# baaivision/Painter

Hardware: AMD Instinct MI355X
Metric: images/sec (896x448 pairs) ViT-L fwd+bwd (higher is better)
Workload: dtype bf16; 1 GPU; painter_vit_large_patch16_input896x448 bf16 batch=8/GPU fwd+bwd on 1xMI355X (BASELINE configs[1]); global_batch=8, image=896x448x3 stitched pair, mode=train (DropPath 0.1), parallelism=dp1, rccl_ranks=0, backend=n/a, grad_allreduce=n/a

## Files before the change

### include/painter_hip.h

```cpp
#ifndef PAINTER_HIP_H
#define PAINTER_HIP_H

#include <stdint.h>

#ifdef __cplusplus
extern "C" {
#endif

#ifndef __HIP__
typedef struct ihipStream_t* hipStream_t;
#endif

enum { PA_F32 = 0, PA_BF16 = 1 };
enum {
    PA_EPI_BIAS = 0,
    PA_EPI_BIAS_F32 = 1,
    PA_EPI_BIAS_GELU = 2,
    PA_EPI_BIAS_RESID = 3
};

#define PA_ABI_VERSION 6
int pa_abi_version(void);
int pa_debug_set(int which, int value);
int pa_debug_get(int which);

int pa_linear_fwd(int dtype, int epilogue, const void* x , int64_t ldx, const void* w ,
                  const float* bias , void* out, void* out2, int64_t ldo, const float* resid ,
                  const float* rowscale , int rows_per_sample, int M, int N, int K,
                  hipStream_t stream);
int pa_linear_pixshuf(int dtype, const void* x, int64_t ldx, const void* w , const float* bias,
                      void* out_nhwc, int batch, int Hp, int Wp, int P, int C, int K, hipStream_t stream);
int64_t pa_linear_dgrad_workspace_bytes(int M, int K);
int pa_linear_dgrad(int dtype, const void* dy , int64_t lddy, const void* w ,
                    const void* gelu_aux , void* dx , int64_t lddx, float* dx_colsum,
                    void* workspace, int M, int N, int K, hipStream_t stream);
int64_t pa_linear_wgrad_workspace_bytes(int dtype, int M, int N, int K);
int pa_linear_wgrad(int dtype, const void* dy , int64_t lddy, const void* x , int64_t ldx,
                    float* dw , void* workspace, int M, int N, int K, hipStream_t stream);
int64_t pa_colsum_workspace_bytes(int M, int N);
int pa_colsum(int dtype, const void* x , int64_t ld, int M, int N, float* out , void* workspace,
              hipStream_t stream);
int pa_slab_reduce(const float* in, float* out, int64_t n, int nz, int64_t stride, int accumulate, hipStream_t stream);

int pa_layernorm_fwd(int dtype, const float* x, int64_t ldx, const float* gamma, const float* beta, float eps,
                     void* y , int64_t ldy, float* mean, float* rstd,
                     int R, int D, hipStream_t stream);
int64_t pa_layernorm_bwd_workspace_bytes(int R, int D);
int pa_layernorm_bwd(int dtype, const void* dy, int64_t lddy, const float* x, int64_t ldx, const float* mean,
                     const float* rstd, const float* gamma, const float* dres, float* dx, int64_t lddx, void* dxT,
                     int64_t lddxT, const float* rowscale, int rows_per_sample, float* dgamma_dbeta, float* dxT_colsum,
                     void* workspace, int R, int D, hipStream_t stream);
int pa_layernorm_bwd_reduce(const void* workspace, float* dgamma_dbeta, float* dxT_colsum, int with_colsum, int R, int D,
                            hipStream_t stream);

int pa_relpos_rows_padded(int Hp, int Wp);
int pa_relpos_pack(int dtype, const float* rel_pos_h, const float* rel_pos_w, void* rcat, int Hp, int Wp, int head_dim,
                   hipStream_t stream);
int pa_relpos_pack_batch(int dtype, const void* tabs, void* rcat, void* rcatT, int nblocks, int Hp, int Wp, int head_dim, hipStream_t stream);
int64_t pa_attn_tables_bytes(int dtype, int batch, int L, int heads, int Hp, int Wp, int head_dim);
int pa_attn_set_generation(int generation);
int pa_attn_launch_counts(long long* out6);
int pa_attn_trace(int enable, unsigned long long* host_out);
int pa_attn_fwd(int dtype, const void* qkv, int64_t ldq, const void* rcat, void* out, int64_t ldo, float* lse,
                void* tables, int batch, int L, int heads, int Hp, int Wp, int head_dim, float scale, hipStream_t stream);

int pa_relpos_pack_t(int dtype, const float* rel_pos_h, const float* rel_pos_w, void* rcatT, int Hp, int Wp, int head_dim,
                     hipStream_t stream);
int pa_attn_bwd_delta(int dtype, const void* out, int64_t ldo, const void* dout, int64_t lddo, float* delta, int batch,
                      int L, int heads, int head_dim, hipStream_t stream);
int pa_attn_bwd_prep_ok(int dtype, int L, int Hp, int Wp, int head_dim);
int pa_attn_bwd_prep(int dtype, const void* out, int64_t ldo, const void* dout, int64_t lddo, const float* lse, void* tables,
                     int batch, int L, int heads, int Hp, int Wp, int head_dim, float scale, hipStream_t stream);
int64_t pa_attn_bwd_aux_bytes(int batch, int L, int heads, int Hp, int Wp);
int64_t pa_attn_bwd_relpos_partials_bytes(int dtype, int batch, int L, int heads, int Hp, int Wp, int head_dim);
int pa_attn_bwd(int dtype, const void* qkv, int64_t ldq, const void* rcat, const void* rcatT, const void* dout,
                int64_t lddo, const float* lse, const float* delta, void* dqkv, void* dG, void* relpos_part, void* aux,
                void* tables, const void* out, int64_t ldo, int batch, int L, int heads, int Hp, int Wp, int head_dim, float scale,
                hipStream_t stream);
int64_t pa_attn_bwd_relpos_workspace_bytes(int dtype, int batch, int L, int heads, int Hp, int Wp, int head_dim);
int pa_attn_bwd_relpos_reduce(const void* relpos_part, float* drcat, void* workspace, int batch, int L, int heads, int Hp, int Wp,
                              int head_dim, hipStream_t stream);
int pa_attn_bwd_relpos(int dtype, const void* dG, const void* qkv, int64_t ldq, float* drcat, void* workspace,
                       int batch, int L, int heads, int Hp, int Wp, int head_dim, hipStream_t stream);

int pa_patch_weight_pack(int dtype, const float* w , void* out , int D, int P, hipStream_t stream);
int pa_patch_embed_fwd(int dtype, const float* imgs, const float* tgts, const void* w, int64_t ldw, const float* bias,
                       const float* mask_token, const float* seg_x, const float* seg_y, const float* pos,
                       const unsigned char* mask, int mask_batch_stride, const float* type_cls, const float* type_ins,
                       const float* seg_type, float* tokens, int batch, int Hp, int Wp, int P, int D, hipStream_t stream);
int pa_patch_cols_ok(int batch, int L, int P, int D);
int pa_patch_im2col(const float* imgs, const float* tgts, void* cols, int batch, int Hp, int Wp, int P, hipStream_t stream);
int pa_patch_embed_fwd_cols(const void* cols, const void* w , int64_t ldw, const float* bias, const float* mask_token,
                            const float* seg_x, const float* seg_y, const float* pos, const unsigned char* mask, int mask_batch_stride,
                            const float* type_cls, const float* type_ins, const float* seg_type, float* tokens, int batch, int L, int K,
                            int D, hipStream_t stream);
int64_t pa_patch_embed_wgrad_workspace_bytes(int D, int P);
int pa_patch_embed_wgrad(int dtype, const void* dpe , const float* imgs, const float* tgts,
                         float* dw , void* workspace, int batch, int Hp, int Wp, int P, int D,
                         hipStream_t stream);
int pa_patch_embed_dgrad(int dtype, const void* dpe, const void* w, int64_t ldw, float* dimgs, float* dtgts, const float* addend,
                         float alpha, int batch, int Hp, int Wp, int P, int D, hipStream_t stream);
int pa_pos_fwd(const int* idx , const float* val , int K, const float* pe , float* pos , int L, int D,
               hipStream_t stream);
int pa_pos_bwd(const int* idxT , const float* valT , int KT, const float* gx , const float* gy ,
               float* dpe , int S, int D, hipStream_t stream);
int pa_tokens_bwd(int dtype, const float* dx0, const unsigned char* mask, int mask_batch_stride, void* dpe, float* sums,
                  int batch, int L, int D, hipStream_t stream);

int pa_merge_fwd(const float* x, float* out, int64_t n_out, hipStream_t stream);
int pa_merge_bwd(int dtype, const float* dmerged, float* dx, void* dxT, const float* rowscale, int rows_per_sample,
                 int64_t rows_half, int D, hipStream_t stream);
int pa_scale_cast(int dtype, const float* in, void* out, const float* rowscale, int rows_per_sample, int64_t rows, int D,
                  hipStream_t stream);
int pa_cast_bf16(const float* in, void* out, int64_t n, hipStream_t stream);
int pa_debug_rmw(const float* src, float* scratch, int64_t n, int passes, int nblocks, hipStream_t stream);
int pa_ensemble_resid(const float* x0, const float* a, float* x1, int batch, int group, int L, int D, hipStream_t stream);

int pa_conv3x3_pack(int dtype, const float* w3 , void* w3r , void* wf ,
                    hipStream_t stream);
int pa_decoder_tail_fwd(int dtype, const void* x_nhwc, const void* w3r, const float* b3, const float* ln_gamma,
                        const float* ln_beta, const float* w1 , const float* b1, void* y3 ,
                        float* pred , int batch, int Hi, int Wi, float eps, hipStream_t stream);
int64_t pa_decoder_tail_bwd_workspace_bytes(int batch, int Hi, int Wi);
int pa_decoder_tail_bwd_pointwise(int dtype, const float* dpred, const void* y3, const float* ln_gamma,
                                  const float* ln_beta, const float* w1, void* dy3, float* grads, void* workspace,
                                  int batch, int Hi, int Wi, float eps, hipStream_t stream);
int pa_conv3x3_dgrad_unshuffle(int dtype, const void* dy3, const void* wf, void* dE, int batch, int Hp, int Wp, int P,
                               hipStream_t stream);
int64_t pa_conv3x3_wgrad_workspace_bytes(int batch, int Hi, int Wi);
int pa_conv3x3_wgrad(int dtype, const void* dy3, const void* x_nhwc, float* dw , void* workspace,
                     int batch, int Hi, int Wi, hipStream_t stream);
// ... 78 lines not shown
```

### painter_amd/csrc/attn3.h

```cpp
#pragma once
#include "common.h"
bool attn3_ok(int L, int Hp, int Wp);
int64_t attn3_table_bytes(int Bn, int L, int H, int Hp, int Wp);
int attn3_fwd(const bf16* qkv, int64_t ldq, const bf16* rcat, bf16* out, int64_t ldo, float* lse, void* tables, int Bn, int L, int H,
              int Hp, int Wp, float scale, hipStream_t st);
int attn3_bwd(const bf16* qkv, int64_t ldq, const bf16* rcatT, const bf16* dout, int64_t lddo, const float* lse, const float* delta,
              void* tables, bf16* dqkv, bf16* dG, float* part, int Bn, int L, int H, int Hp, int Wp, float scale, const bf16* out, int64_t ldo,
              hipStream_t st);
int attn3_bwd_prep(const bf16* out, int64_t ldo, const bf16* dout, int64_t lddo, const float* lse, void* tables, int Bn, int L, int H, int Hp,
                   float scale, hipStream_t st);
int64_t attn3_relpos_partials_bytes(int Bn, int L, int H, int Hp, int Wp);
int attn3_relpos_reduce(const float* part, float* drcat, float* tmp, int Bn, int L, int H, int Hp, int Wp, hipStream_t st);
```

### painter_amd/csrc/attn3.hip

```cpp
#include "attn3_common.h"
#include "../../include/painter_hip.h"
#include "attn3.h"
#include <cstdlib>

#ifndef A3_PRIO
#define A3_PRIO 0
#endif
#ifndef A3_HOIST
#define A3_HOIST 1
#endif
#ifndef A3_NDL
#define A3_NDL true
#endif
#define A3_PRIO_UP() do { if (A3_PRIO) __builtin_amdgcn_s_setprio(1); } while (0)
#define A3_PRIO_DOWN() do { if (A3_PRIO) __builtin_amdgcn_s_setprio(0); } while (0)

namespace a3 {

template <int STAGES>
__global__ __launch_bounds__(NT, STAGES == 1 ? 4 : 2) void fwd_kernel(const bf16* __restrict__ qkv, size_t ldq, const bf16* __restrict__ rcat,
                                                                      bf16* __restrict__ out, size_t ldo, float* __restrict__ lse,
                                                                      unsigned char* __restrict__ tables, int L, int H, int Hp, int NRP,
                                                                      float scale, int nblk, int xcd_map, int abl) {
    extern __shared__ __attribute__((aligned(16))) unsigned char smem[];
    const int tid = threadIdx.x, lane = tid & 63, wave = tid >> 6, g = lane >> 5, ql = lane & 31;
    int blk, bh;
    wg_coords(nblk, xcd_map, blk, bh, (L / 32) / NW);
    const int b = bh / H, h = bh % H, D = H * ATT_HD;
    const bf16* base = qkv + (size_t)b * L * ldq + h * ATT_HD;
    const bf16* kbase = base + D;
    const bf16* vbase = base + 2 * D;
    const int qt = blk * NW + wave;
    const bool valid = qt * 32 < L;
    const int q = qt * 32 + ql;
    unsigned char* thT = smem + STAGES * STAGE_QK + wave * Hp * 64;
    unsigned char* eimg = smem + STAGES * STAGE_QK + NW * Hp * 64;
    unsigned char* twimg = eimg + wave * 2048;
    LaneAddr la;
    la.init(lane);
    EAddr ea;
    ea.init(lane);
    const int ntile = L / 32;
    Stager ks, vs;
    ks.load(kbase, ldq, tid);
    vs.load(vbase, ldq, tid);

    bf16x8 qf[4];
    uint4 T0 = zero4(), T1 = zero4();
    if (valid) {
#pragma unroll
        for (int s = 0; s < 4; ++s) qf[s] = gfrag(base + (size_t)q * ldq, s, g);
        if (!(abl & 32)) build_tables3(twimg, thT, rcat, NRP, qf, q / WP, q % WP, Hp, 1.f / scale, lane, smem + tid * 2);
        T0 = *reinterpret_cast<const uint4*>(twimg + ql * 64 + 16 * g);
        T1 = *reinterpret_cast<const uint4*>(twimg + ql * 64 + 32 + 16 * g);
        if (tables != nullptr) {
            unsigned char* tt = tables + ((size_t)bh * ntile + qt) * ttile_bytes(Hp);
#pragma unroll
            for (int i = 0; i < 2; ++i) *reinterpret_cast<uint4*>(tt + (lane + 64 * i) * 16) = *reinterpret_cast<const uint4*>(twimg + (lane + 64 * i) * 16);
            for (int c = lane; c < Hp * 4; c += 64) *reinterpret_cast<uint4*>(tt + 2048 + c * 16) = *reinterpret_cast<const uint4*>(thT + c * 16);
        }
    }
    __syncthreads();
    build_eimg(eimg, tid);
    ks.store(smem, tid);
    vs.store(smem + IMG, tid);
    __syncthreads();

    f32x16 oacc[2];
    oacc[0] = zero16();
    oacc[1] = zero16();
    float m = 0.f, l = 0.f;
    const float sl = scale * LOG2E_F;
    const unsigned char* thw = thT + ql * 2;

    auto body = [&](auto pc, int a) {
        constexpr int P = decltype(pc)::value;
        const int j = a * PH + P;
        {
            const int jn = min(j + 1, ntile - 1);
            ks.load(kbase + (size_t)jn * 32 * ldq, ldq, tid);
            vs.load(vbase + (size_t)jn * 32 * ldq, ldq, tid);
        }
        const unsigned char* kimg = smem + (STAGES == 2 ? (j & 1) * STAGE_QK : 0);
        const unsigned char* vimg = kimg + IMG;
        if (valid) {
            const unsigned char* thr = thw + a * (RPP * 64);
            if constexpr (P == 0) win_set<0>(T1.w, thr);
            win_set<(P + 1) & 1>(T1.w, thr + (P + 1) * 64);
            const unsigned char* ei = eimg + P * EIMG;
            const bf16x8 ef0 = efrag(ei, ea, 0), ef1 = efrag(ei, ea, 1);
            bf16x8 kfr[4];
#pragma unroll
            for (int s = 0; s < 4; ++s) kfr[s] = rowfrag(kimg, la, s);
            __builtin_amdgcn_sched_barrier(0);
            f32x16 sacc = zero16();
            A3_PRIO_UP();
            sacc = mfma(ef0, as_frag(T0), sacc);
            sacc = mfma(ef1, as_frag(T1), sacc);
#pragma unroll
            for (int s = 0; s < 4; ++s) sacc = mfma(kfr[s], qf[s], sacc);
            A3_PRIO_DOWN();
            bf16x8 vtr[2][2];
            vtr[0][0] = trfrag(vimg, la, 0, 0);
            vtr[0][1] = trfrag(vimg, la, 0, 1);
            if constexpr (STAGES == 2) { vtr[1][0] = trfrag(vimg, la, 1, 0); vtr[1][1] = trfrag(vimg, la, 1, 1); }
            __builtin_amdgcn_sched_barrier(0);
            float p[16];
            const float nm = -m;
#pragma unroll
            for (int r = 0; r < 16; ++r) p[r] = fmaf(sacc[r], sl, nm);
            float tmax = max16(p);
            tmax = fmaxf(tmax, xor32(tmax));
            if (j == 0 || __any(tmax > THR)) {
                const float delta = (j == 0) ? tmax : fmaxf(tmax, 0.f);
                const float alpha = __builtin_amdgcn_exp2f(-delta);
                m += delta;
                l *= alpha;
#pragma unroll
                for (int r = 0; r < 16; ++r) { oacc[0][r] *= alpha; oacc[1][r] *= alpha; p[r] -= delta; }
            }
#pragma unroll
            for (int r = 0; r < 16; ++r) p[r] = __builtin_amdgcn_exp2f(p[r]);
            l += sum16(p);
            const bf16x8 pf0 = packfrag(p), pf1 = packfrag(p + 8);
            if constexpr (STAGES == 1) { vtr[1][0] = trfrag(vimg, la, 1, 0); vtr[1][1] = trfrag(vimg, la, 1, 1); }
            A3_PRIO_UP();
#pragma unroll
            for (int db = 0; db < 2; ++db) {
                oacc[db] = mfma(vtr[db][0], pf0, oacc[db]);
                oacc[db] = mfma(vtr[db][1], pf1, oacc[db]);
            }
            A3_PRIO_DOWN();
        }
        if constexpr (STAGES == 1) __syncthreads();
        if (j + 1 < ntile) {
            ks.store(smem + (STAGES == 2 ? ((j + 1) & 1) * STAGE_QK : 0), tid);
            vs.store(smem + (STAGES == 2 ? ((j + 1) & 1) * STAGE_QK : 0) + IMG, tid);
        }
        __syncthreads();
    };
    for (int a = 0; a < ((abl & 16) ? 0 : Hp / RPP); ++a) {
        body(std::integral_constant<int, 0>{}, a);
        body(std::integral_constant<int, 1>{}, a);
        body(std::integral_constant<int, 2>{}, a);
        body(std::integral_constant<int, 3>{}, a);
        body(std::integral_constant<int, 4>{}, a);
        body(std::integral_constant<int, 5>{}, a);
        body(std::integral_constant<int, 6>{}, a);
    }
    unsigned char* stg = smem + wave * IMG;
    if constexpr (STAGES == 1) { if (wave >= 2) stg = eimg + (wave - 2) * IMG; }
    if (valid) {
        const float lt = l + xor32(l);
        if (g == 0) {
            const float lse_q = (m + __builtin_amdgcn_logf(lt)) * LN2_F;
            lse[(size_t)bh * L + q] = lse_q;
            if (tables != nullptr) {
                unsigned char* tt = tables + ((size_t)bh * ntile + qt) * ttile_bytes(Hp);
                const float x = -lse_q * (1.f / scale);
                const bf16 hi = (bf16)x;
                *reinterpret_cast<bf16*>(tt + 2048 + Hp * 64 + ql * 2) = hi;
                *reinterpret_cast<bf16*>(tt + 2048 + (Hp + 1) * 64 + ql * 2) = (bf16)(x - (float)hi);
            }
        }
        stage_rows(stg, oacc, 1.f / lt, lane);
        write_rows(stg, out + (size_t)(b * L + qt * 32) * ldo + h * ATT_HD, ldo, lane);
    }
}

__device__ unsigned long long g_trace[2 * 2 * 64 * 8];
constexpr int NSMAX = 12;
template <int MINW, bool NDL, bool TR = false, bool FUSE = false>
__global__ __launch_bounds__(NT, MINW) void bwd_dq_kernel(const bf16* __restrict__ qkv, size_t ldq, const bf16* __restrict__ rcatT,
                                                          const bf16* __restrict__ dout, size_t lddo, const float* __restrict__ lse,
                                                          unsigned char* __restrict__ tables, bf16* __restrict__ dqkv,
                                                          bf16* __restrict__ dG, float* __restrict__ part, int L, int H, int Hp, int NRP,
                                                          float scale, int nblk, int xcd_map, int abl, int tile0, int pslot0,
                                                          const bf16* __restrict__ oatt, size_t ldo) {
    extern __shared__ __attribute__((aligned(16))) unsigned char smem[];
    const int tid = threadIdx.x, lane = tid & 63, wave = tid >> 6, g = lane >> 5, ql = lane & 31;
    const int trwg = blockIdx.x == 0 ? 0 : (blockIdx.x == gridDim.x / 2 ? 1 : -1);
    auto coarse = [&](int pt) {
        if constexpr (TR) {
            if constexpr (MINW < 3 && A3_HOIST) __builtin_amdgcn_sched_barrier(0);
            const unsigned long long t = __builtin_amdgcn_s_memtime();
            if (trwg >= 0 && wave < 2 && lane == 0) g_trace[((trwg * 2 + wave) * 64 + pt) * 8] = t;
            if constexpr (MINW < 3 && A3_HOIST) __builtin_amdgcn_sched_barrier(0);
        }
    };
    coarse(60);
    int blk, bh;
    wg_coords(nblk, xcd_map, blk, bh, (L / 32 - tile0) / NW);
    const int b = bh / H, h = bh % H, D = H * ATT_HD;
    const bf16* base = qkv + (size_t)b * L * ldq + h * ATT_HD;
    const bf16* kbase = base + D;
    const bf16* vbase = base + 2 * D;
    const int qt = tile0 + blk * NW + wave;
    const bool valid = qt * 32 < L;
    const int q = qt * 32 + ql;
    const int qh = q / WP, qw = q % WP;
    unsigned char* thT = smem + 2 * STAGE_QK + wave * Hp * 64;
    unsigned char* eimg = smem + 2 * STAGE_QK + NW * Hp * 64;
    unsigned char* rimg = eimg + PH * EIMG;
    const int rpitch = NRP * 2 + 16;
    LaneAddr la;
    la.init(lane);
    EAddr ea;
    ea.init(lane);
    const int ntile = L / 32;
    const float sl = scale * LOG2E_F;
    Stager ks, vs;
    ks.load(kbase, ldq, tid);
    vs.load(vbase, ldq, tid);
    const int rchunks = ATT_HD * (NRP / 8);

    bf16x8 qf[4], dof[4];
    uint4 T0 = zero4(), T1 = zero4();
    uint4 tch[4] = {zero4(), zero4(), zero4(), zero4()};
    float nlse2 = 0.f, ndlt = 0.f;
    unsigned char* tt = tables + ((size_t)bh * ntile + qt) * ttile_bytes(Hp);
    if (valid) {
#pragma unroll
        for (int s = 0; s < 4; ++s) {
            qf[s] = gfrag(base + (size_t)q * ldq, s, g);
            dof[s] = gfrag(dout + (size_t)(b * L + q) * lddo + h * ATT_HD, s, g);
        }
        if (oatt != nullptr) {
            float dl = 0.f;
#pragma unroll
            for (int s = 0; s < 4; ++s) {
                const bf16x8 of = gfrag(oatt + (size_t)(b * L + q) * ldo + h * ATT_HD, s, g);
#pragma unroll
                for (int t = 0; t < 8; ++t) dl = fmaf((float)of[t], (float)dof[s][t], dl);
            }
            dl += xor32(dl);
            ndlt = -dl;
            if (g == 0) *reinterpret_cast<float*>(tt + 2048 + (Hp + 2) * 64 + ql * 4) = ndlt;
        }
        T0 = *reinterpret_cast<const uint4*>(tt + ql * 64 + 16 * g);
        T1 = *reinterpret_cast<const uint4*>(tt + ql * 64 + 32 + 16 * g);
#pragma unroll
        for (int i = 0; i < 4; ++i)
            if (lane + 64 * i < Hp * 4) tch[i] = *reinterpret_cast<const uint4*>(tt + 2048 + (lane + 64 * i) * 16);
        nlse2 = -lse[(size_t)bh * L + q] * LOG2E_F;
        if (oatt == nullptr) ndlt = *reinterpret_cast<const float*>(tt + 2048 + (Hp + 2) * 64 + ql * 4);
    }
    build_eimg(eimg, tid);
    {
        const int per_row = NRP / 8;
        for (int c = tid; c < rchunks; c += 2 * NT) {
            const int c2 = c + NT;
            const uint4 v0 = *reinterpret_cast<const uint4*>(rcatT + (size_t)c * 8);
            const uint4 v1 = c2 < rchunks ? *reinterpret_cast<const uint4*>(rcatT + (size_t)c2 * 8) : zero4();
// ... 165 lines not shown
        };
        const int nstep = NRP / 16;
        const unsigned char* r0 = rimg + ql * rpitch + 16 * g, *r1 = r0 + 32 * rpitch;
        auto rfrag = [&](const unsigned char* rp, int s) { return __builtin_bit_cast(bf16x8, *reinterpret_cast<const uint4*>(rp + 32 * s)); };
        bf16x8 rf[2] = {rfrag(r0, 0), rfrag(r1, 0)};
        float gcur[8];
        gather(0, gcur);
        auto rstep = [&](int s, uint4& keep) {
            const int sn = min(s + 1, nstep - 1);
            const bf16x8 rn[2] = {rfrag(r0, sn), rfrag(r1, sn)};
            float gnext[8];
            if (abl & 32) {
#pragma unroll
                for (int t = 0; t < 8; ++t) gnext[t] = gcur[t] + 1.f;
            } else {
                gather(sn, gnext);
            }
            const bf16x8 gf = packfrag(gcur);
            if constexpr (FUSE) keep = __builtin_bit_cast(uint4, gf);
            else if (!(abl & 2)) *reinterpret_cast<uint4*>(dgrow + 16 * s + 8 * g) = __builtin_bit_cast(uint4, gf);
#pragma unroll
            for (int db = 0; db < 2; ++db) {
                if (!(abl & 64)) dq[db] = mfma(rf[db], gf, dq[db]);
                rf[db] = rn[db];
            }
#pragma unroll
            for (int t = 0; t < 8; ++t) gcur[t] = gnext[t];
        };
        if constexpr (FUSE) {
#pragma unroll
            for (int s = 0; s < NSMAX; ++s)
                if (s < ((abl & 1) ? 0 : nstep)) rstep(s, gfs[s]);
        } else {
            uint4 none;
            for (int s = 0; s < ((abl & 1) ? 0 : nstep); ++s) rstep(s, none);
        }
        stage_rows(stg, dq, 1.f, lane);
        if (!(abl & 4)) write_rows(stg, dqkv + (size_t)(b * L + qt * 32) * ldq + h * ATT_HD, ldq, lane);
    }
    if constexpr (FUSE) {
        __syncthreads();
        const int nimg = (NRP + 63) >> 6;
        unsigned char* wimg = smem + wave * (nimg + 1) * IMG;
        if (valid) {
            const int rsw = vsw(ql);
#pragma unroll
            for (int s = 0; s < NSMAX; ++s)
                if (s < NRP / 16) *reinterpret_cast<uint4*>(wimg + (s >> 2) * IMG + ql * 128 + ((((2 * s + g) & 7) ^ rsw) << 4)) = gfs[s];
#pragma unroll
            for (int s = 0; s < 4; ++s)
                *reinterpret_cast<uint4*>(wimg + nimg * IMG + ql * 128 + (((2 * s + g) ^ rsw) << 4)) = __builtin_bit_cast(uint4, qf[s]);
        }
        __syncthreads();
        float* pw = part + (size_t)(pslot0 + blockIdx.x) * NRP * ATT_HD;
        for (int u = wave; u < 2 * (NRP / 32); u += NW) {
            const int rb = u >> 1, db = u & 1;
            f32x16 acc = zero16();
            for (int w2 = 0; w2 < NW; ++w2) {
                if ((tile0 + blk * NW + w2) * 32 >= L) break;
                const unsigned char* im = smem + w2 * (nimg + 1) * IMG;
#pragma unroll
                for (int ks = 0; ks < 2; ++ks)
                    acc = mfma(trfrag(im + (rb >> 1) * IMG, la, rb & 1, ks), trfrag(im + nimg * IMG, la, db, ks), acc);
            }
            float* pcol = pw + (size_t)(rb * 32 + 4 * g) * ATT_HD + db * 32 + ql;
#pragma unroll
            for (int reg = 0; reg < 16; ++reg) pcol[((reg & 3) + 8 * (reg >> 2)) * ATT_HD] = acc[reg];
        }
    }
    if constexpr (TR) { asm volatile("s_waitcnt vmcnt(0)" ::: "memory"); }
    coarse(63);
}

constexpr int DKV_TW = 2 * IMG, DKV_TH = DKV_TW + 2048, DKV_ND = DKV_TH + 512, DKV_STAGE = DKV_ND + 128;
template <int MINW>
__global__ __launch_bounds__(NT, MINW) void bwd_dkv_kernel(const bf16* __restrict__ qkv, size_t ldq, const bf16* __restrict__ dout,
                                                           size_t lddo, const unsigned char* __restrict__ tables, bf16* __restrict__ dqkv,
                                                           int L, int H, int Hp, float scale, int nblk, int xcd_map, int abl, int tile0) {
    extern __shared__ __attribute__((aligned(16))) unsigned char smem[];
    const int tid = threadIdx.x, lane = tid & 63, wave = tid >> 6, g = lane >> 5, ql = lane & 31;
    int blk, bh;
    wg_coords(nblk, xcd_map, blk, bh, (L / 32 - tile0) / NW);
    const int b = bh / H, h = bh % H, D = H * ATT_HD;
    const bf16* qbase = qkv + (size_t)b * L * ldq + h * ATT_HD;
    const bf16* dobase = dout + (size_t)b * L * lddo + h * ATT_HD;
    const int kt = tile0 + blk * NW + wave;
    const bool valid = kt * 32 < L;
    const int key = kt * 32 + ql;
    const int kh = key / WP, kw = key % WP;
    const int khlo = ((tile0 + blk * NW) * 32) / WP;
    const int kha = (kt * 32) / WP;
    const int ntile = L / 32;
    const int TB = ttile_bytes(Hp);
    const unsigned char* tbase = tables + (size_t)bh * ntile * TB;
    LaneAddr la;
    la.init(lane);
    EAddr ea;
    ea.init(lane);
    const float sl = scale * LOG2E_F;
    const int sa = kha & 3, sb = (kha + 1) & 3;

    bf16x8 kf[4], vf[4], eb0, eb1;
    int woff[2];
    {
        uint32_t e0[4] = {0, 0, 0, 0}, e1[4] = {0, 0, 0, 0};
#pragma unroll
        for (int t = 0; t < 8; ++t) {
            const uint32_t bit = 0x3F80u << (16 * (t & 1));
            if (kw == 8 * g + t) e0[t >> 1] |= bit;
            if (t < 6) {
                if (kw == 16 + 6 * g + t) e1[t >> 1] |= bit;
            } else {
                const int slot = 2 * g + (t - 6);
                if (slot == (kh & 3) || (slot != sa && slot != sb)) e1[t >> 1] |= bit;
            }
        }
        eb0 = __builtin_bit_cast(bf16x8, make_uint4(e0[0], e0[1], e0[2], e0[3]));
        eb1 = __builtin_bit_cast(bf16x8, make_uint4(e1[0], e1[1], e1[2], e1[3]));
#pragma unroll
        for (int hs = 0; hs < 2; ++hs) {
            const int slot = 2 * g + hs;
            int row;
            if (slot == sa) row = kha - khlo;
            else if (slot == sb) row = kha + 1 - khlo;
            else {
                int rank = 0;
                for (int s2 = 0; s2 < slot; ++s2) rank += (s2 != sa && s2 != sb) ? 1 : 0;
                row = 6 + rank;
            }
            woff[hs] = DKV_TH + row * 64 + ql * 2;
        }
    }
    if (valid) {
#pragma unroll
        for (int s = 0; s < 4; ++s) {
            kf[s] = gfrag(qbase + D + (size_t)key * ldq, s, g);
            vf[s] = gfrag(qbase + 2 * D + (size_t)key * ldq, s, g);
        }
    }
    Stager qs, dos;
// ... 135 lines not shown
            unsigned char* tt = tables + ((size_t)bh * (L / 32) + qt) * TB;
            const float x = -lse[(size_t)bh * L + l] * inv_scale;
            const bf16 hi = (bf16)x;
            const bf16 lo = (bf16)(x - (float)hi);
            *reinterpret_cast<bf16*>(tt + 2048 + Hp * 64 + qi * 2) = hi;
            *reinterpret_cast<bf16*>(tt + 2048 + (Hp + 1) * 64 + qi * 2) = lo;
            *reinterpret_cast<float*>(tt + 2048 + (Hp + 2) * 64 + qi * 4) = -s;
        }
    }
}

}

int attn3_bwd_prep(const bf16* out, int64_t ldo, const bf16* dout, int64_t lddo, const float* lse, void* tables, int Bn, int L, int H, int Hp,
                   float scale, hipStream_t st) {
    const int R = Bn * L;
    PA_LAUNCH(a3::prep_delta_kernel, dim3((R + 3) / 4), dim3(256), 0, st, out, (size_t)ldo, dout, (size_t)lddo, lse,
              reinterpret_cast<unsigned char*>(tables), R, L, H, Hp, 1.f / scale);
    return (int)hipGetLastError();
}

static int g_attn_generation = 0;
extern "C" int pa_attn_set_generation(int generation) {
    if (generation != 0 && generation != 2 && generation != 3) return (int)hipErrorInvalidValue;
    g_attn_generation = generation;
    return 0;
}
static int g_attn_trace = 0;
extern "C" int pa_attn_trace(int enable, unsigned long long* host_out) {
    g_attn_trace = enable;
    if (host_out != nullptr) return (int)hipMemcpyFromSymbol(host_out, HIP_SYMBOL(a3::g_trace), sizeof(a3::g_trace));
    return 0;
}
bool attn3_ok(int L, int Hp, int Wp) {
    static const int on = [] { const char* e = getenv("PA_ATTN3"); return e ? atoi(e) : 1; }();
    return on && g_attn_generation != 2 && Wp == a3::WP && Hp % a3::RPP == 0 && Hp >= a3::RPP && L == Hp * Wp;
}
int64_t attn3_table_bytes(int Bn, int L, int H, int Hp, int Wp) {
    if (!attn3_ok(L, Hp, Wp)) return 0;
    return (int64_t)Bn * H * (L / 32) * a3::ttile_bytes(Hp);
}
static int a3_xcd_map_on() {
    static const int v = [] {
        const char* e = getenv("PA_ATTN_XCD");
        const char* l = getenv("PA_ATTN_LIGHT_LAST");
        return ((e ? atoi(e) : 1) ? 1 : 0) | ((l ? atoi(l) : 0) ? 2 : 0);
    }();
    if (g_attn_light_last == 1) return v & 1;
    if (g_attn_light_last == 2) return v | 2;
    return v;
}

int attn3_fwd(const bf16* qkv, int64_t ldq, const bf16* rcat, bf16* out, int64_t ldo, float* lse, void* tables, int Bn, int L, int H,
              int Hp, int Wp, float scale, hipStream_t st) {
    using namespace a3;
    const int NRP = pa_relpos_rows_padded(Hp, Wp);
    static const int stages = [] { const char* v = getenv("PA_ATTN3_FWD_STAGES"); return v ? atoi(v) : 1; }();
    const size_t smem = (size_t)(stages == 2 ? 2 : 1) * STAGE_QK + (size_t)NW * Hp * 64 + PH * EIMG;
    static bool done1 = false, done2 = false;
    auto kern = stages == 2 ? fwd_kernel<2> : fwd_kernel<1>;
    if (int e = set_smem(reinterpret_cast<const void*>(kern), stages == 2 ? done2 : done1)) return e;
    const int nblk = (L / 32 + NW - 1) / NW;
    PA_LAUNCH(kern, dim3(nblk * Bn * H), dim3(NT), smem, st, qkv, (size_t)ldq, rcat, out, (size_t)ldo, lse,
              reinterpret_cast<unsigned char*>(tables), L, H, Hp, NRP, scale, nblk, a3_xcd_map_on(), [] { const char* v = getenv("PA_ATTN3_FWD_ABL"); return v ? atoi(v) : 0; }());
    return (int)hipGetLastError();
}

namespace a3 {
constexpr int RED_ZC = 32;
__global__ __launch_bounds__(256) void relpos_part_reduce_kernel(const float4* __restrict__ part, float4* __restrict__ tmp, int n4, int nz) {
    __shared__ float4 sh[4][64];
    const int c = blockIdx.x * 64 + (threadIdx.x & 63), zl = threadIdx.x >> 6;
    const int z0 = (int)((int64_t)nz * blockIdx.y / gridDim.y), z1 = (int)((int64_t)nz * (blockIdx.y + 1) / gridDim.y);
    float4 s = make_float4(0, 0, 0, 0);
    if (c < n4) {
#pragma unroll 4
        for (int z = z0 + zl; z < z1; z += 4) {
            const float4 v = part[(size_t)z * n4 + c];
            s.x += v.x; s.y += v.y; s.z += v.z; s.w += v.w;
        }
    }
    sh[zl][threadIdx.x & 63] = s;
    __syncthreads();
    if (zl == 0 && c < n4) {
        float4 t = sh[0][threadIdx.x];
#pragma unroll
        for (int k = 1; k < 4; ++k) { const float4 v = sh[k][threadIdx.x]; t.x += v.x; t.y += v.y; t.z += v.z; t.w += v.w; }
        tmp[(size_t)blockIdx.y * n4 + c] = t;
    }
}
}
extern "C" int pa_slab_reduce(const float* in, float* out, int64_t n, int nz, int64_t stride, int accumulate, hipStream_t st);
static int a3_fuse_on() {
    static const int v = [] { const char* e = getenv("PA_ATTN3_FUSE_RELPOS"); return e ? atoi(e) : 1; }();
    return g_attn3_fuse == 1 ? 0 : (g_attn3_fuse == 2 ? 1 : v);
}
static int a3_blocks(int L) { return (L / 32 + a3::NW - 1) / a3::NW; }
static int64_t a3_num_partials(int Bn, int L, int H, int, int) { return (int64_t)a3_blocks(L) * Bn * H; }
int64_t attn3_relpos_partials_bytes(int Bn, int L, int H, int Hp, int Wp) {
    if (!a3_fuse_on() || !attn3_ok(L, Hp, Wp)) return 0;
    const int NRP = pa_relpos_rows_padded(Hp, Wp);
    if (NRP > 16 * a3::NSMAX) return 0;
    return a3_num_partials(Bn, L, H, Hp, Wp) * NRP * ATT_HD * sizeof(float);
}
int attn3_relpos_reduce(const float* part, float* drcat, float* tmp, int Bn, int L, int H, int Hp, int Wp, hipStream_t st) {
    using namespace a3;
    const int NRP = pa_relpos_rows_padded(Hp, Wp);
    const int nz = (int)a3_num_partials(Bn, L, H, Hp, Wp), n4 = NRP * ATT_HD / 4;
    const int zc = nz < RED_ZC ? nz : RED_ZC;
    PA_LAUNCH(relpos_part_reduce_kernel, dim3((n4 + 63) / 64, zc), dim3(256), 0, st, reinterpret_cast<const float4*>(part),
              reinterpret_cast<float4*>(tmp), n4, nz);
    if (int e = (int)hipGetLastError()) return e;
    return pa_slab_reduce(tmp, drcat, (int64_t)n4 * 4, zc, (int64_t)n4 * 4, 0, st);
}

int attn3_bwd(const bf16* qkv, int64_t ldq, const bf16* rcatT, const bf16* dout, int64_t lddo, const float* lse, const float* delta,
              void* tables, bf16* dqkv, bf16* dG, float* part, int Bn, int L, int H, int Hp, int Wp, float scale, const bf16* out, int64_t ldo,
              hipStream_t st) {
    using namespace a3;
    const int NRP = pa_relpos_rows_padded(Hp, Wp);
    if (part != nullptr && NRP > 16 * NSMAX) return (int)hipErrorInvalidValue;
    if (part == nullptr && dG == nullptr) return (int)hipErrorInvalidValue;
    unsigned char* tb = reinterpret_cast<unsigned char*>(tables);
    int e;
    if (delta != nullptr) {
        const int total = Bn * H * L;
        PA_LAUNCH(prep_kernel, dim3((total + 255) / 256), dim3(256), 0, st, lse, delta, tb, L, Hp, 1.f / scale, total);
        if ((e = (int)hipGetLastError())) return e;
    }
    const int tile0 = 0;
    const int nblk = a3_blocks(L);
    static const int dq_w = [] { const char* v = getenv("PA_ATTN3_DQ_WAVES"); return v ? atoi(v) : 2; }();
    static const int dkv_w = [] { const char* v = getenv("PA_ATTN3_DKV_WAVES"); return v ? atoi(v) : 2; }();
    if (nblk > 0) {
        static const size_t pad = [] { const char* v = getenv("PA_ATTN3_LDS_PAD"); return v ? (size_t)atoi(v) : (size_t)0; }();
        size_t smem = 2 * (size_t)STAGE_QK + (size_t)NW * Hp * 64 + PH * EIMG + (size_t)ATT_HD * (NRP * 2 + 16) + pad;
        const bool fuse = part != nullptr;
        if (fuse) {
            const size_t need = (size_t)NW * ((NRP + 63) / 64 + 1) * IMG;
            if (smem < need) smem = need;
        }
        auto kern = fuse ? bwd_dq_kernel<2, A3_NDL, false, true>
                         : (g_attn_trace ? bwd_dq_kernel<2, true, true> : (dq_w == 3 ? bwd_dq_kernel<3, false> : bwd_dq_kernel<2, A3_NDL>));
        static bool done2 = false, done3 = false, donet = false, donef = false;
        if ((e = set_smem(reinterpret_cast<const void*>(kern), fuse ? donef : (g_attn_trace ? donet : (dq_w == 3 ? done3 : done2))))) return e;
        const char* ablv = getenv("PA_ATTN3_DQ_ABL");
        PA_LAUNCH(kern, dim3(nblk * Bn * H), dim3(NT), smem, st, qkv, (size_t)ldq, rcatT, dout, (size_t)lddo, lse, tb, dqkv, dG, part, L, H,
                  Hp, NRP, scale, nblk, a3_xcd_map_on(), ablv ? atoi(ablv) : 0, tile0, 0, delta == nullptr ? out : nullptr, (size_t)ldo);
        if ((e = (int)hipGetLastError())) return e;
    }
    const int tile0_kv = 0, nblk_kv = a3_blocks(L);
    if (nblk_kv > 0) {
        size_t smem = 2 * (size_t)DKV_STAGE;
        if (smem < (size_t)NW * 2 * IMG) smem = (size_t)NW * 2 * IMG;
        static const size_t pad = [] { const char* v = getenv("PA_ATTN3_LDS_PAD"); return v ? (size_t)atoi(v) : (size_t)0; }();
        smem += pad;
        auto kern = dkv_w == 3 ? bwd_dkv_kernel<3> : bwd_dkv_kernel<2>;
        static bool done2 = false, done3 = false;
        if ((e = set_smem(reinterpret_cast<const void*>(kern), dkv_w == 3 ? done3 : done2))) return e;
        PA_LAUNCH(kern, dim3(nblk_kv * Bn * H), dim3(NT), smem, st, qkv, (size_t)ldq, dout, (size_t)lddo, tb, dqkv, L, H, Hp, scale, nblk_kv,
                  a3_xcd_map_on(), [] { const char* v = getenv("PA_ATTN3_DKV_ABL"); return v ? atoi(v) : 0; }(), tile0_kv);
        if ((e = (int)hipGetLastError())) return e;
    }
    return 0;
}
```

### painter_amd/csrc/attn_bwd.hip

```cpp
#include "attn_common.h"
#include <cstdlib>
#include "gemm_engine.h"
#include "../../include/painter_hip.h"
#include "attn2.h"
#include "attn3.h"

template <typename T> DEVI void load16(const T* p, float* v);
template <> DEVI void load16<bf16>(const bf16* p, float* v) {
    const uint4 a = *reinterpret_cast<const uint4*>(p), b = *reinterpret_cast<const uint4*>(p + 8);
    v[0] = bf16_lo(a.x); v[1] = bf16_hi(a.x); v[2] = bf16_lo(a.y); v[3] = bf16_hi(a.y);
    v[4] = bf16_lo(a.z); v[5] = bf16_hi(a.z); v[6] = bf16_lo(a.w); v[7] = bf16_hi(a.w);
    v[8] = bf16_lo(b.x); v[9] = bf16_hi(b.x); v[10] = bf16_lo(b.y); v[11] = bf16_hi(b.y);
    v[12] = bf16_lo(b.z); v[13] = bf16_hi(b.z); v[14] = bf16_lo(b.w); v[15] = bf16_hi(b.w);
}
template <> DEVI void load16<float>(const float* p, float* v) {
#pragma unroll
    for (int i = 0; i < 4; ++i) {
        const float4 a = *reinterpret_cast<const float4*>(p + 4 * i);
        v[4 * i] = a.x; v[4 * i + 1] = a.y; v[4 * i + 2] = a.z; v[4 * i + 3] = a.w;
    }
}
template <typename T, bool VEC>
__global__ __launch_bounds__(256) void attn_delta_kernel(const T* o, size_t ldo, const T* d_o, size_t lddo, float* delta, int R, int L, int H, int hd) {
    __shared__ float part[4][128];
// ... 471 lines not shown
template <typename T, int HD>
static int attn_bwd_t(const T* qkv, int64_t ldq, const T* rcat, const T* rcatT, const T* dout, int64_t lddo, const float* lse,
                      const float* delta, T* dqkv, T* dG, float* aux, int Bn, int L, int H, int Hp, int Wp, float scale, hipStream_t st) {
    typedef KvTile<T, HD> KV;
    const int TS = Hp + Wp;
    const int qtiles = L / 32;
    {
        int ts = 2 * 32 * TS * 4;
        const int stg = 32 * HD * (int)sizeof(T);
        if (ts < stg) ts = stg;
        ts = (ts + 15) / 16 * 16;
        const size_t stages = 2 * (size_t)(2 * KV::KB + KV::VB);
        int e = (int)hipErrorInvalidValue;
        if (stages + 4 * (size_t)ts <= 160 * 1024) {
            e = attn_bwd_dq_launch<T, 4, HD>(qkv, ldq, rcat, rcatT, dout, lddo, lse, delta, dqkv, dG, aux, Bn, L, H, Hp, Wp, scale, stages + 4 * (size_t)ts, ts, st);
        } else if constexpr (HD != 64) {
            if (stages + 3 * (size_t)ts <= 160 * 1024)
                e = attn_bwd_dq_launch<T, 3, HD>(qkv, ldq, rcat, rcatT, dout, lddo, lse, delta, dqkv, dG, aux, Bn, L, H, Hp, Wp, scale, stages + 3 * (size_t)ts, ts, st);
        }
        if (e) return e;
    }
    {
        constexpr int NW = 4;
        const int AUXB = (TS + 2) * AUX_LD * 4;
        size_t smem = 2 * (size_t)(2 * KV::KB + 2 * KV::VB + AUXB);
        const size_t stg = (size_t)NW * 2 * 32 * HD * sizeof(T);
        if (smem < stg) smem = stg;
        if (smem > 160 * 1024 || (TS + 2) * 8 > (HD == 64 ? 3 : 4) * NW * 64) return (int)hipErrorInvalidValue;
        auto kern = attn_bwd_dkv_kernel<T, NW, HD>;
        static bool done = false;
        if (!done) {
            hipError_t e = hipFuncSetAttribute(reinterpret_cast<const void*>(kern), hipFuncAttributeMaxDynamicSharedMemorySize, 160 * 1024);
            if (e != hipSuccess) return (int)e;
            done = true;
        }
        PA_LAUNCH(kern, dim3((qtiles + NW - 1) / NW, Bn * H), dim3(NW * 64), smem, st, qkv, (size_t)ldq, dout, (size_t)lddo,
                           aux, dqkv, L, H, Hp, Wp, scale);
        return (int)hipGetLastError();
    }
}

extern "C" int pa_attn_bwd_prep_ok(int dtype, int L, int Hp, int Wp, int head_dim) {
    return (dtype == PA_BF16 && head_dim == ATT_HD && L == Hp * Wp && attn3_ok(L, Hp, Wp)) ? 1 : 0;
}
extern "C" int pa_attn_bwd_prep(int dtype, const void* out, int64_t ldo, const void* dout, int64_t lddo, const float* lse, void* tables,
                                int batch, int L, int heads, int Hp, int Wp, int head_dim, float scale, hipStream_t st) {
    if (!pa_attn_bwd_prep_ok(dtype, L, Hp, Wp, head_dim) || tables == nullptr || ldo % 8 || lddo % 8) return (int)hipErrorInvalidValue;
    return attn3_bwd_prep((const bf16*)out, ldo, (const bf16*)dout, lddo, lse, tables, batch, L, heads, Hp, scale, st);
}
extern "C" int64_t pa_attn_bwd_relpos_partials_bytes(int dtype, int batch, int L, int heads, int Hp, int Wp, int head_dim) {
    if (dtype != PA_BF16 || head_dim != ATT_HD || L != Hp * Wp) return 0;
    return attn3_relpos_partials_bytes(batch, L, heads, Hp, Wp);
}
extern "C" int pa_attn_bwd(int dtype, const void* qkv, int64_t ldq, const void* rcat, const void* rcatT, const void* dout, int64_t lddo,
                           const float* lse, const float* delta, void* dqkv, void* dG, void* relpos_part, void* aux, void* tables,
                           const void* out, int64_t ldo, int batch, int L, int heads, int Hp, int Wp, int head_dim, float scale, hipStream_t st) {
    if (L != Hp * Wp || L % 32 || Hp % 4 || Wp % 4 || (head_dim != 64 && head_dim != 80)) return (int)hipErrorInvalidValue;
    if (dtype == PA_BF16 && head_dim == ATT_HD && tables != nullptr && attn3_ok(L, Hp, Wp)) {
        if (relpos_part != nullptr && attn3_relpos_partials_bytes(batch, L, heads, Hp, Wp) == 0) return (int)hipErrorInvalidValue;
        ++g_attn_counts[5];
        if (out != nullptr && ldo % 8) return (int)hipErrorInvalidValue;
        return attn3_bwd((const bf16*)qkv, ldq, (const bf16*)rcatT, (const bf16*)dout, lddo, lse, delta, tables, (bf16*)dqkv, (bf16*)dG,
                         (float*)relpos_part, batch, L, heads, Hp, Wp, scale, (const bf16*)out, ldo, st);
    }
    if (relpos_part != nullptr || dG == nullptr || delta == nullptr) return (int)hipErrorInvalidValue;
    if (dtype == PA_BF16 && attn2_ok(L, Hp, Wp, head_dim)) {
        ++g_attn_counts[4];
        return attn2_bwd((const bf16*)qkv, ldq, (const bf16*)rcat, (const bf16*)rcatT, (const bf16*)dout, lddo, lse, delta, (bf16*)dqkv,
                         (bf16*)dG, aux, batch, L, heads, Hp, Wp, head_dim, scale, st);
    }
    ++g_attn_counts[3];
#define PA_ATTN_BWD(TT_, HD_) attn_bwd_t<TT_, HD_>((const TT_*)qkv, ldq, (const TT_*)rcat, (const TT_*)rcatT, (const TT_*)dout, lddo, lse, delta, \
                                                   (TT_*)dqkv, (TT_*)dG, (float*)aux, batch, L, heads, Hp, Wp, scale, st)
    if (dtype == PA_BF16) return head_dim == 80 ? PA_ATTN_BWD(bf16, 80) : PA_ATTN_BWD(bf16, 64);
    return head_dim == 80 ? PA_ATTN_BWD(float, 80) : PA_ATTN_BWD(float, 64);
#undef PA_ATTN_BWD
}

extern "C" int64_t pa_attn_bwd_relpos_workspace_bytes(int dtype, int batch, int L, int heads, int Hp, int Wp, int head_dim) {
    const int NRP = pa_relpos_rows_padded(Hp, Wp);
    return (int64_t)heads * 32 * NRP * head_dim * sizeof(float);
}
template <typename T>
static int relpos_grad_t(const T* dG, const T* qkv, int64_t ldq, float* drcat, float* ws, int Bn, int L, int H, int NRP, int hd, hipStream_t st) {
    const int R = Bn * L;
    OpT<T> A{dG, (size_t)H * NRP, NRP, (size_t)NRP};
    OpT<T> B{qkv, (size_t)ldq, hd, (size_t)hd};
    const int nku = (R + TT<T>::BK - 1) / TT<T>::BK;
    static const int want = [] { const char* v = getenv("PA_RELPOS_SPLITS"); return v ? atoi(v) : 16; }();
    static const bool from_env = getenv("PA_RELPOS_SPLITS") != nullptr;
    int splits = (!from_env && g_relpos_splits > 0) ? g_relpos_splits : want;
    if (splits > 32) splits = 32;
    if (splits < 1) splits = 1;
    if (splits > nku) splits = nku;
    struct Epi {
        float* out; size_t slab; int M, N;
        DEVI void operator()(const f32x16 (&acc)[2][2], int ib, int jb, int lane, int z) const {
            float* o = out + (size_t)z * slab;
            foreach_acc(acc, ib, jb, lane, [&](int i, int j, float v) {
                if (i < M && j < N) o[(size_t)i * N + j] = v;
            });
        }
    };
    int e = launch_gemm<T, 2, 2>(A, B, Epi{ws, (size_t)NRP * hd, NRP, hd}, NRP, hd, R, splits, H, st);
    if (e) return e;
    return pa_slab_reduce(ws, drcat, (int64_t)NRP * hd, splits * H, (int64_t)NRP * hd, 0, st);
}
extern "C" int pa_attn_bwd_relpos_reduce(const void* relpos_part, float* drcat, void* workspace, int batch, int L, int heads, int Hp, int Wp,
                                         int head_dim, hipStream_t st) {
    if (head_dim != ATT_HD || relpos_part == nullptr || attn3_relpos_partials_bytes(batch, L, heads, Hp, Wp) == 0) return (int)hipErrorInvalidValue;
    return attn3_relpos_reduce((const float*)relpos_part, drcat, (float*)workspace, batch, L, heads, Hp, Wp, st);
}
extern "C" int pa_attn_bwd_relpos(int dtype, const void* dG, const void* qkv, int64_t ldq, float* drcat, void* workspace, int batch, int L,
                                  int heads, int Hp, int Wp, int head_dim, hipStream_t st) {
    if (head_dim <= 0 || head_dim % 16) return (int)hipErrorInvalidValue;
    const int NRP = pa_relpos_rows_padded(Hp, Wp);
    if (dtype == PA_BF16) return relpos_grad_t<bf16>((const bf16*)dG, (const bf16*)qkv, ldq, drcat, (float*)workspace, batch, L, heads, NRP, head_dim, st);
    return relpos_grad_t<float>((const float*)dG, (const float*)qkv, ldq, drcat, (float*)workspace, batch, L, heads, NRP, head_dim, st);
}
```

### painter_amd/csrc/attn_fwd.hip

```cpp
#include "attn_common.h"
#include "../../include/painter_hip.h"
#include "attn2.h"
#include "attn3.h"

template <typename T, int NW, int HD>
__global__ __launch_bounds__(NW * 64) void attn_fwd_kernel(const T* __restrict__ qkv, size_t ldq, const T* __restrict__ rcat,
                                                           T* __restrict__ out, size_t ldo, float* __restrict__ lse, int L, int H,
                                                           int Hp, int Wp, int NRP, float scale, int tab_stride) {
    typedef KvTile<T, HD> KV;
    constexpr int NT = NW * 64;
    constexpr int KB = KV::KB, VB = KV::VB, KS = KV::KS, DB = KV::DB;
    extern __shared__ __attribute__((aligned(16))) unsigned char smem[];
    const int tid = threadIdx.x, lane = tid & 63, wave = tid >> 6, g = lane >> 5;
    const int bh = blockIdx.y, b = bh / H, h = bh % H;
    const int D = H * HD, TS = Hp + Wp;
    const T* base = qkv + (size_t)b * L * ldq + h * HD;
    const T* kbase = base + D;
    const T* vbase = base + 2 * D;
    const int qt = blockIdx.x * NW + wave;
    const bool valid = qt * 32 < L;
    const int q = qt * 32 + (lane & 31);
    unsigned char* const kimg = smem;
    unsigned char* const vimg = smem + 2 * KB;
    unsigned char* const wreg = smem + 2 * KB + 2 * VB + (size_t)wave * tab_stride;
// ... 169 lines not shown
    if (r < nh) v = rh[r * hd + d];
    else if (r - nh < nw) v = rw[(r - nh) * hd + d];
    (tr ? rcatT : rcat)[(size_t)blk * NRP * hd + i] = from_f<T>(v);
}
extern "C" int pa_relpos_pack_batch(int dtype, const void* tabs, void* rcat, void* rcatT, int nblocks, int Hp, int Wp, int head_dim, hipStream_t st) {
    if (head_dim <= 0 || head_dim % 16 || nblocks <= 0 || nblocks > 65535) return (int)hipErrorInvalidValue;
    const int NRP = pa_relpos_rows_padded(Hp, Wp);
    const int n = NRP * head_dim;
    const float* const* t = reinterpret_cast<const float* const*>(tabs);
    if (dtype == PA_BF16)
        PA_LAUNCH(relpos_pack_batch_kernel<bf16>, dim3((n + 255) / 256, nblocks, 2), dim3(256), 0, st, t, nblocks, 2 * Hp - 1, 2 * Wp - 1, (bf16*)rcat, (bf16*)rcatT, NRP, head_dim);
    else
        PA_LAUNCH(relpos_pack_batch_kernel<float>, dim3((n + 255) / 256, nblocks, 2), dim3(256), 0, st, t, nblocks, 2 * Hp - 1, 2 * Wp - 1, (float*)rcat, (float*)rcatT, NRP, head_dim);
    LAUNCH_CHECK();
}

static int attn_tab_stride(int Hp, int Wp, int hd, int elem) {
    int a = 32 * (Hp + Wp) * 4, b = 32 * hd * elem;
    int s = a > b ? a : b;
    return (s + 15) / 16 * 16;
}
template <typename T, int NW, int HD>
static int attn_fwd_launch(const T* qkv, int64_t ldq, const T* rcat, T* out, int64_t ldo, float* lse, int Bn, int L, int H, int Hp,
                           int Wp, float scale, hipStream_t st) {
    const int NRP = pa_relpos_rows_padded(Hp, Wp);
    const int ts = attn_tab_stride(Hp, Wp, HD, sizeof(T));
    const size_t smem = 2 * KvTile<T, HD>::KB + 2 * KvTile<T, HD>::VB + (size_t)NW * ts;
    auto kern = attn_fwd_kernel<T, NW, HD>;
    static bool done = false;
    if (!done) {
        hipError_t e = hipFuncSetAttribute(reinterpret_cast<const void*>(kern), hipFuncAttributeMaxDynamicSharedMemorySize, 160 * 1024);
        if (e != hipSuccess) return (int)e;
        done = true;
    }
    if (smem > 160 * 1024) return (int)hipErrorInvalidValue;
    const int qtiles = L / 32;
    dim3 grid((qtiles + NW - 1) / NW, Bn * H);
    PA_LAUNCH(kern, grid, dim3(NW * 64), smem, st, qkv, (size_t)ldq, rcat, out, (size_t)ldo, lse, L, H, Hp, Wp, NRP, scale, ts);
    return (int)hipGetLastError();
}
template <typename T>
static int attn_fwd_t(const void* qkv, int64_t ldq, const void* rcat, void* out, int64_t ldo, float* lse, int Bn, int L, int H, int Hp,
                      int Wp, int hd, float scale, hipStream_t st) {
    const T *q = (const T*)qkv, *r = (const T*)rcat;
    T* o = (T*)out;
    if (hd == 80) return attn_fwd_launch<T, 4, 80>(q, ldq, r, o, ldo, lse, Bn, L, H, Hp, Wp, scale, st);
    if ((L / 32) % 7 == 0) return attn_fwd_launch<T, 7, 64>(q, ldq, r, o, ldo, lse, Bn, L, H, Hp, Wp, scale, st);
    return attn_fwd_launch<T, 4, 64>(q, ldq, r, o, ldo, lse, Bn, L, H, Hp, Wp, scale, st);
}

extern "C" int64_t pa_attn_tables_bytes(int dtype, int batch, int L, int heads, int Hp, int Wp, int head_dim) {
    return dtype == PA_BF16 && head_dim == ATT_HD ? attn3_table_bytes(batch, L, heads, Hp, Wp) : 0;
}
extern "C" int pa_attn_fwd(int dtype, const void* qkv, int64_t ldq, const void* rcat, void* out, int64_t ldo, float* lse, void* tables,
                           int batch, int L, int heads, int Hp, int Wp, int head_dim, float scale, hipStream_t st) {
    if (L != Hp * Wp || L % 32 || Hp % 4 || Wp % 4 || !head_dim_ok(head_dim)) return (int)hipErrorInvalidValue;
    if (dtype == PA_BF16 && head_dim == ATT_HD && attn3_ok(L, Hp, Wp)) {
        ++g_attn_counts[2];
        return attn3_fwd((const bf16*)qkv, ldq, (const bf16*)rcat, (bf16*)out, ldo, lse, tables, batch, L, heads, Hp, Wp, scale, st);
    }
    if (dtype == PA_BF16 && attn2_ok(L, Hp, Wp, head_dim)) {
        ++g_attn_counts[1];
        return attn2_fwd((const bf16*)qkv, ldq, (const bf16*)rcat, (bf16*)out, ldo, lse, batch, L, heads, Hp, Wp, head_dim, scale, st);
    }
    ++g_attn_counts[0];
    if (dtype == PA_BF16) return attn_fwd_t<bf16>(qkv, ldq, rcat, out, ldo, lse, batch, L, heads, Hp, Wp, head_dim, scale, st);
    return attn_fwd_t<float>(qkv, ldq, rcat, out, ldo, lse, batch, L, heads, Hp, Wp, head_dim, scale, st);
}

extern "C" int pa_attn_launch_counts(long long* out6) {
    if (out6 == nullptr) return (int)hipErrorInvalidValue;
    for (int i = 0; i < 6; ++i) out6[i] = g_attn_counts[i];
    return 0;
}
```

### painter_amd/csrc/attn_tile.h

```cpp
#pragma once
#include "attn_common.h"

namespace atile {

constexpr int NW = 4, NT = 256, ROWS = 128, IMG = 4096, STAGE_QK = 2 * IMG;
typedef __attribute__((ext_vector_type(4))) short s16x4;
typedef __attribute__((address_space(3))) s16x4 lds_s16x4;
typedef __attribute__((ext_vector_type(2))) uint32_t u32x2;
typedef __attribute__((ext_vector_type(8))) float f32x8;

DEVI int xcd_run(int n, int total) {
    const int xq = total >> 3, xr = total & 7, xcd = n & 7;
    return (xcd < xr ? xcd * (xq + 1) : xr * (xq + 1) + (xcd - xr) * xq) + (n >> 3);
}
DEVI void wg_coords(int nblk, int xcd_map, int& blk, int& bh, int nfull = 0) {
    const int n = blockIdx.x, total = gridDim.x;
    if ((xcd_map & 2) && nfull > 0 && nfull < nblk) {
        const int nbh = total / nblk, heavy = nfull * nbh;
        if (n < heavy) {
            const int v = (xcd_map & 1) ? xcd_run(n, heavy) : n;
            bh = v / nfull;
            blk = v - bh * nfull;
        } else {
            const int m = n - heavy, per = nblk - nfull, lt = nbh * per;
            const int v = (xcd_map & 1) ? xcd_run(m, lt) : m;
            bh = v / per;
            blk = nfull + (v - bh * per);
        }
        return;
    }
    const int v = (xcd_map & 1) ? xcd_run(n, total) : n;
    bh = v / nblk;
    blk = v - bh * nblk;
}

DEVI int vsw(int row) { return (((row >> 1) & 1) << 2) | (((row >> 2) & 1) << 1) | ((row >> 3) & 1); }

struct Stager {
    uint4 r;
    DEVI void load(const bf16* src, size_t ld, int tid) { r = *reinterpret_cast<const uint4*>(src + (size_t)(tid >> 3) * ld + (tid & 7) * 8); }
    DEVI void store(unsigned char* img, int tid) const {
        const int row = tid >> 3, c = tid & 7;
        *reinterpret_cast<uint4*>(img + row * 128 + ((c ^ vsw(row)) << 4)) = r;
    }
};

struct LaneAddr {
    int rowbase, t;
    int tr[2][2];
    DEVI void init(int lane) {
        const int row = lane & 31, g = lane >> 5;
        rowbase = row * 128;
        t = vsw(row) ^ g;
        const int i = lane & 15, half = (lane >> 4) & 1;
#pragma unroll
        for (int db = 0; db < 2; ++db)
#pragma unroll
            for (int hi = 0; hi < 2; ++hi) {
                const int r = 4 * g + (i >> 2) + 8 * hi;
                const int chunk = 4 * db + 2 * half + ((i & 3) >> 1);
                tr[db][hi] = r * 128 + ((chunk ^ vsw(r)) << 4) + (i & 1) * 8;
            }
    }
};
DEVI bf16x8 rowfrag(const unsigned char* img, const LaneAddr& a, int s) {
    return __builtin_bit_cast(bf16x8, *reinterpret_cast<const uint4*>(img + a.rowbase + (((2 * s) ^ a.t) << 4)));
}
DEVI u32x2 ldtr(const unsigned char* p) {
    return __builtin_bit_cast(u32x2, __builtin_amdgcn_ds_read_tr16_b64_v4i16((lds_s16x4*)p));
}
DEVI bf16x8 trfrag(const unsigned char* img, const LaneAddr& a, int db, int s) {
    const u32x2 l = ldtr(img + a.tr[db][0] + s * 2048), h = ldtr(img + a.tr[db][1] + s * 2048);
    return __builtin_bit_cast(bf16x8, __builtin_shufflevector(l, h, 0, 1, 2, 3));
}
DEVI bf16x8 gfrag(const bf16* p, int s, int g) { return __builtin_bit_cast(bf16x8, *reinterpret_cast<const uint4*>(p + 16 * s + 8 * g)); }
DEVI bf16x8 packfrag(const float* v) {
    const f32x8 f = {v[0], v[1], v[2], v[3], v[4], v[5], v[6], v[7]};
    return __builtin_convertvector(f, bf16x8);
}
DEVI float xor32(float v) {
    const uint32_t u = __builtin_bit_cast(uint32_t, v);
    const auto r = __builtin_amdgcn_permlane32_swap(u, u, false, false);
    return __builtin_bit_cast(float, (threadIdx.x & 32) ? r[0] : r[1]);
}
DEVI float max3f(float a, float b, float c) { return fmaxf(fmaxf(a, b), c); }
DEVI float max16(const float* p) {
    const float a = max3f(p[0], p[1], p[2]), b = max3f(p[3], p[4], p[5]), c = max3f(p[6], p[7], p[8]), d = max3f(p[9], p[10], p[11]),
                e = max3f(p[12], p[13], p[14]);
    return max3f(max3f(a, b, c), max3f(d, e, p[15]), -INFINITY);
}
DEVI float sum16(const float* p) {
    float a = p[0] + p[4], b = p[1] + p[5], c = p[2] + p[6], d = p[3] + p[7];
    a += p[8]; b += p[9]; c += p[10]; d += p[11];
    a += p[12]; b += p[13]; c += p[14]; d += p[15];
    return (a + b) + (c + d);
}
DEVI f32x16 mfma(bf16x8 a, bf16x8 b, f32x16 c) { return __builtin_amdgcn_mfma_f32_32x32x16_bf16(a, b, c, 0, 0, 0); }

DEVI void stage_rows(unsigned char* stg, const f32x16 (&acc)[2], float mul, int lane) {
    const int g = lane >> 5;
#pragma unroll
    for (int db = 0; db < 2; ++db)
#pragma unroll
        for (int rg = 0; rg < 4; ++rg) {
            const int d0 = db * 32 + 8 * rg + 4 * g;
            *reinterpret_cast<uint2*>(stg + (lane & 31) * 128 + d0 * 2) =
                make_uint2(pack_bf16x2(acc[db][rg * 4] * mul, acc[db][rg * 4 + 1] * mul), pack_bf16x2(acc[db][rg * 4 + 2] * mul, acc[db][rg * 4 + 3] * mul));
        }
}
DEVI void write_rows(const unsigned char* stg, bf16* dst, size_t ld, int lane) {
#pragma unroll
    for (int i = 0; i < 4; ++i) {
        const int c = lane + 64 * i, row = c >> 3, ch = c & 7;
        *reinterpret_cast<uint4*>(dst + (size_t)row * ld + ch * 8) = *reinterpret_cast<const uint4*>(stg + row * 128 + ch * 16);
    }
}

static inline int set_smem(const void* kern, bool& done) {
    if (!done) {
        hipError_t e = hipFuncSetAttribute(kern, hipFuncAttributeMaxDynamicSharedMemorySize, 160 * 1024);
        if (e != hipSuccess) return (int)e;
        done = true;
    }
    return 0;
}

}
```

### painter_amd/csrc/common.h

```cpp
#pragma once
#include <hip/hip_runtime.h>
#include <stdint.h>

typedef __bf16 bf16;
typedef __attribute__((ext_vector_type(8))) __bf16 bf16x8;
typedef __attribute__((ext_vector_type(16))) float f32x16;

#define DEVI __device__ __forceinline__

template <typename T> struct TT;
template <> struct TT<float> {
    static constexpr int EPC = 4;
    static constexpr int BK = 32;
    static constexpr int KSTEPS = 2;
    static constexpr int SPF = 2;
    typedef uint4 Vec4;
};
template <> struct TT<bf16> {
    static constexpr int EPC = 8;
    static constexpr int BK = 64;
    static constexpr int KSTEPS = 4;
    static constexpr int SPF = 1;
    typedef uint2 Vec4;
};

DEVI float to_f(float x) { return x; }
DEVI float to_f(bf16 x) { return (float)x; }
template <typename T> DEVI T from_f(float x);
template <> DEVI float from_f<float>(float x) { return x; }
template <> DEVI bf16 from_f<bf16>(float x) { return (bf16)x; }

DEVI uint32_t pack_bf16x2(float lo, float hi) {
    uint16_t a = __builtin_bit_cast(uint16_t, (bf16)lo);
    uint16_t b = __builtin_bit_cast(uint16_t, (bf16)hi);
    return (uint32_t)a | ((uint32_t)b << 16);
}
DEVI float bf16_lo(uint32_t w) { return __builtin_bit_cast(float, w << 16); }
DEVI float bf16_hi(uint32_t w) { return __builtin_bit_cast(float, w & 0xffff0000u); }

template <typename T> struct Frag;
template <> struct Frag<bf16> {
    bf16x8 v;
    DEVI void set(uint4 a) { v = __builtin_bit_cast(bf16x8, a); }
};
template <> struct Frag<float> {
    float v[8];
    DEVI void set(uint4 a, uint4 b) {
        v[0] = __builtin_bit_cast(float, a.x); v[1] = __builtin_bit_cast(float, a.y);
        v[2] = __builtin_bit_cast(float, a.z); v[3] = __builtin_bit_cast(float, a.w);
        v[4] = __builtin_bit_cast(float, b.x); v[5] = __builtin_bit_cast(float, b.y);
        v[6] = __builtin_bit_cast(float, b.z); v[7] = __builtin_bit_cast(float, b.w);
    }
};

DEVI void mma(f32x16& c, const Frag<bf16>& a, const Frag<bf16>& b) {
    c = __builtin_amdgcn_mfma_f32_32x32x16_bf16(a.v, b.v, c, 0, 0, 0);
}
DEVI void mma(f32x16& c, const Frag<float>& a, const Frag<float>& b) {
#pragma unroll
    for (int t = 0; t < 8; ++t) c = __builtin_amdgcn_mfma_f32_32x32x2f32(a.v[t], b.v[t], c, 0, 0, 0);
}
DEVI int acc_row(int reg, int lane) { return (reg & 3) + 8 * (reg >> 2) + 4 * (lane >> 5); }

DEVI int lds128(int row, int slot) { return row * 128 + ((slot ^ ((row >> 1) & 7)) << 4); }
DEVI int lds256(int row, int slot) { return row * 256 + ((slot ^ (row & 15)) << 4); }
DEVI int lds64(int row, int gran) { return row * 64 + ((gran ^ ((row >> 2) & 7)) << 3); }

template <int CTRL> DEVI float lane_dpp(float v) {
    const int i = __builtin_bit_cast(int, v);
    return __builtin_bit_cast(float, __builtin_amdgcn_update_dpp(i, i, CTRL, 0xf, 0xf, false));
}
DEVI float lane_xor1(float v) { return lane_dpp<0xB1>(v); }
DEVI float lane_xor2(float v) { return lane_dpp<0x4E>(v); }
DEVI float lane_xor16(float v) {
    const uint32_t u = __builtin_bit_cast(uint32_t, v);
    const auto r = __builtin_amdgcn_permlane16_swap(u, u, false, false);
    return __builtin_bit_cast(float, (threadIdx.x & 16) ? r[0] : r[1]);
}
DEVI float lane_xor32(float v) {
    const uint32_t u = __builtin_bit_cast(uint32_t, v);
    const auto r = __builtin_amdgcn_permlane32_swap(u, u, false, false);
    return __builtin_bit_cast(float, (threadIdx.x & 32) ? r[0] : r[1]);
}
DEVI float quad_sum(float v) { v += lane_xor1(v); v += lane_xor2(v); return v; }
DEVI float row16_sum(float v) { v = quad_sum(v); v += lane_dpp<0x141>(v); v += lane_dpp<0x140>(v); return v; }
DEVI float wave_sum(float v) { v = row16_sum(v); v += lane_xor16(v); v += lane_xor32(v); return v; }
DEVI float wave_max(float v) {
    v = fmaxf(v, lane_xor1(v)); v = fmaxf(v, lane_xor2(v));
    v = fmaxf(v, lane_dpp<0x141>(v)); v = fmaxf(v, lane_dpp<0x140>(v));
    v = fmaxf(v, lane_xor16(v)); v = fmaxf(v, lane_xor32(v));
    return v;
}

inline int g_relpos_splits = 0;
inline int g_attn3_fuse = 0;
inline int g_attn_light_last = 0;

inline int g_ln_bwd_variant = 0;

inline int g_conv_wgrad_groups = 0;
inline int g_misc_knob[5] = {0, 0, 0, 0, 0};

inline long long g_attn_counts[6] = {0, 0, 0, 0, 0, 0};

DEVI float gelu_f(float x) { return 0.5f * x * (1.0f + erff(x * 0.70710678118654752f)); }
DEVI float gelu_grad_f(float x) {
    const float cdf = 0.5f * (1.0f + erff(x * 0.70710678118654752f));
    const float pdf = 0.39894228040143268f * __expf(-0.5f * x * x);
    return cdf + x * pdf;
}

DEVI void gelu_parts(float x, float& cdf, float& pdf_unnorm) {
    const float z = fabsf(x) * 0.70710678118654752f;
    const float t = __builtin_amdgcn_rcpf(fmaf(0.3275911f, z, 1.0f));
    const float e = __builtin_amdgcn_exp2f(-0.72134752044448170f * x * x);
    float p = fmaf(1.061405429f, t, -1.453152027f);
    p = fmaf(p, t, 1.421413741f);
    p = fmaf(p, t, -0.284496736f);
    p = fmaf(p, t, 0.254829592f);
    const float half_erfc = 0.5f * p * t * e;
    cdf = x >= 0.f ? 1.0f - half_erfc : half_erfc;
    pdf_unnorm = e;
}
DEVI float gelu_fast(float x) {
    float c, e;
    gelu_parts(x, c, e);
    return x * c;
}
typedef __attribute__((ext_vector_type(2))) float f32x2_t;
DEVI void gelu_parts2(f32x2_t x, f32x2_t& cdf, f32x2_t& e) {
    const f32x2_t ax = {fabsf(x[0]), fabsf(x[1])};
    const f32x2_t d = __builtin_elementwise_fma(ax, (f32x2_t){0.23164189f, 0.23164189f}, (f32x2_t){1.0f, 1.0f});
    const f32x2_t t = {__builtin_amdgcn_rcpf(d[0]), __builtin_amdgcn_rcpf(d[1])};
    const f32x2_t xx = x * x * (f32x2_t){-0.72134752044448170f, -0.72134752044448170f};
    e = (f32x2_t){__builtin_amdgcn_exp2f(xx[0]), __builtin_amdgcn_exp2f(xx[1])};
    f32x2_t p = __builtin_elementwise_fma(t, (f32x2_t){0.5307027145f, 0.5307027145f}, (f32x2_t){-0.7265760135f, -0.7265760135f});
    p = __builtin_elementwise_fma(p, t, (f32x2_t){0.7107068705f, 0.7107068705f});
    p = __builtin_elementwise_fma(p, t, (f32x2_t){-0.142248368f, -0.142248368f});
    p = __builtin_elementwise_fma(p, t, (f32x2_t){0.127414796f, 0.127414796f});
    const f32x2_t h = p * t * e;
    const f32x2_t m = (f32x2_t){0.5f, 0.5f} - h;
    cdf = (f32x2_t){__builtin_copysignf(m[0], x[0]), __builtin_copysignf(m[1], x[1])} + (f32x2_t){0.5f, 0.5f};
}
DEVI f32x2_t gelu_fast2(float x0, float x1) {
    const f32x2_t x = {x0, x1};
    f32x2_t c, e;
    gelu_parts2(x, c, e);
    return x * c;
}
DEVI void gelu_both2(float x0, float x1, f32x2_t& y, f32x2_t& dy) {
    const f32x2_t x = {x0, x1};
    f32x2_t c, e;
    gelu_parts2(x, c, e);
    y = x * c;
    dy = __builtin_elementwise_fma(x * (f32x2_t){0.39894228040143268f, 0.39894228040143268f}, e, c);
// ... 27 lines not shown
```

### painter_amd/csrc/gemm.hip

```cpp
#include <cstdlib>
#include "gemm_engine.h"
#include "gemm256.h"
#include "../../include/painter_hip.h"

template <typename OutT> struct EpiBias {
    OutT* out; size_t ldo; const float* bias; int M, N;
    DEVI void operator()(const f32x16 (&acc)[2][2], int ib, int jb, int lane, int) const {
        foreach_acc(acc, ib, jb, lane, [&](int i, int j, float v) {
            if (i < M && j < N) out[(size_t)i * ldo + j] = from_f<OutT>(v + (bias ? bias[j] : 0.f));
        });
    }
};
constexpr float G8_OFF = 0.13f, G8_SCALE = 255.f / 1.26f, G8_STEP = 1.26f / 255.f;
DEVI uint32_t g8_code(float g) { return min((uint32_t)fmaf(g, G8_SCALE, G8_OFF * G8_SCALE + 0.5f), 255u); }
DEVI float g8_value(uint32_t q) { return fmaf((float)q, G8_STEP, -G8_OFF); }
template <typename T> struct GeluAux { typedef T type; };
template <> struct GeluAux<bf16> { typedef unsigned char type; };
template <typename T> struct EpiBiasGelu {
    typename GeluAux<T>::type* aux; T* act; size_t ld; const float* bias; int M, N;
    DEVI void operator()(const f32x16 (&acc)[2][2], int ib, int jb, int lane, int) const {
        foreach_acc(acc, ib, jb, lane, [&](int i, int j, float v) {
            if (i < M && j < N) {
                const T p = from_f<T>(v + bias[j]);
                if constexpr (std::is_same<T, bf16>::value) {
// ... 296 lines not shown
template <typename T> __global__ __launch_bounds__(256) void colsum_kernel(const T* __restrict__ x, size_t ld, int M, int N, int rows_per_chunk, float* __restrict__ part) {
    const int cl = threadIdx.x & 31, rl = threadIdx.x >> 5;
    const int c0 = (blockIdx.x * 32 + cl) * 8;
    const int r0 = blockIdx.y * rows_per_chunk, r1 = min(M, r0 + rows_per_chunk);
    float s[8] = {0, 0, 0, 0, 0, 0, 0, 0};
    if (c0 < N) {
#pragma unroll 4
        for (int r = r0 + rl; r < r1; r += 8) {
            const T* p = x + (size_t)r * ld + c0;
            if constexpr (sizeof(T) == 2) {
                const uint4 w = *reinterpret_cast<const uint4*>(p);
                s[0] += bf16_lo(w.x); s[1] += bf16_hi(w.x); s[2] += bf16_lo(w.y); s[3] += bf16_hi(w.y);
                s[4] += bf16_lo(w.z); s[5] += bf16_hi(w.z); s[6] += bf16_lo(w.w); s[7] += bf16_hi(w.w);
            } else {
                const float4 a = *reinterpret_cast<const float4*>(p), b = *reinterpret_cast<const float4*>(p + 4);
                s[0] += a.x; s[1] += a.y; s[2] += a.z; s[3] += a.w; s[4] += b.x; s[5] += b.y; s[6] += b.z; s[7] += b.w;
            }
        }
    }
    __shared__ float red[8][32 * 8 + 8];
#pragma unroll
    for (int e = 0; e < 8; ++e) red[rl][cl * 8 + e] = s[e];
    __syncthreads();
    const int c = threadIdx.x;
    if (blockIdx.x * 256 + c < N) {
        float t = 0.f;
#pragma unroll
        for (int k = 0; k < 8; ++k) t += red[k][c];
        part[(size_t)blockIdx.y * N + blockIdx.x * 256 + c] = t;
    }
}
static int colsum_rows_per_chunk(int M) { return M >= 4096 ? 128 : 32; }
extern "C" int64_t pa_colsum_workspace_bytes(int M, int N) {
    const int rpc = colsum_rows_per_chunk(M), chunks = (M + rpc - 1) / rpc;
    return (int64_t)chunks * N * sizeof(float);
}
extern "C" int pa_colsum(int dtype, const void* x, int64_t ld, int M, int N, float* out, void* workspace, hipStream_t st) {
    if (N % 8 || ld % 8) return (int)hipErrorInvalidValue;
    const int rpc = colsum_rows_per_chunk(M), chunks = (M + rpc - 1) / rpc;
    float* part = reinterpret_cast<float*>(workspace);
    dim3 grid((N + 255) / 256, chunks);
    if (dtype == PA_BF16)
        PA_LAUNCH(colsum_kernel<bf16>, grid, dim3(256), 0, st, (const bf16*)x, (size_t)ld, M, N, rpc, part);
    else
        PA_LAUNCH(colsum_kernel<float>, grid, dim3(256), 0, st, (const float*)x, (size_t)ld, M, N, rpc, part);
    int e = (int)hipGetLastError();
    if (e) return e;
    return pa_slab_reduce(part, out, N, chunks, N, 0, st);
}

template <typename T>
static int linear_fwd_t(int epi, const T* x, int64_t ldx, const T* w, const float* bias, void* out, void* out2,
                        int64_t ldo, const float* resid, const float* rowscale, int rps, int M, int N, int K,
                        hipStream_t st) {
    if constexpr (std::is_same<T, bf16>::value) {
        if (g256::ok(M, N, K, false, false, ldx, K)) {
            switch (epi) {
            case PA_EPI_BIAS:
                return g256::launch<false, false>(x, ldx, w, K, Epi4Bias<bf16>{(bf16*)out, (size_t)ldo, bias, M, N}, M, N, K, 1, st);
            case PA_EPI_BIAS_F32:
                return g256::launch<false, false>(x, ldx, w, K, Epi4Bias<float>{(float*)out, (size_t)ldo, bias, M, N}, M, N, K, 1, st);
            case PA_EPI_BIAS_GELU:
                return g256::launch<false, false>(x, ldx, w, K, Epi4BiasGelu{(unsigned char*)out2, (bf16*)out, (size_t)ldo, bias, M, N}, M, N, K, 1, st);
            case PA_EPI_BIAS_RESID:
                return g256::launch<false, false>(x, ldx, w, K, Epi4BiasResid{(float*)out, resid, (size_t)ldo, bias, rowscale, rps, M, N}, M, N, K, 1, st);
            }
        }
    }
    OpN<T> A{x, (size_t)ldx, M, 0};
    OpN<T> B{w, (size_t)K, N, 0};
    switch (epi) {
    case PA_EPI_BIAS:
        return launch_gemm<T, 2, 2>(A, B, EpiBias<T>{(T*)out, (size_t)ldo, bias, M, N}, M, N, K, 1, 1, st);
    case PA_EPI_BIAS_F32:
        return launch_gemm<T, 2, 2>(A, B, EpiBias<float>{(float*)out, (size_t)ldo, bias, M, N}, M, N, K, 1, 1, st);
    case PA_EPI_BIAS_GELU:
        return launch_gemm<T, 2, 2>(A, B, EpiBiasGelu<T>{(typename GeluAux<T>::type*)out2, (T*)out, (size_t)ldo, bias, M, N}, M, N, K, 1, 1, st);
    case PA_EPI_BIAS_RESID:
        return launch_gemm<T, 2, 2>(A, B, EpiBiasResid{(float*)out, resid, (size_t)ldo, bias, rowscale, rps, M, N}, M, N, K, 1, 1, st);
    }
    return (int)hipErrorInvalidValue;
}

extern "C" int pa_linear_fwd(int dtype, int epilogue, const void* x, int64_t ldx, const void* w, const float* bias,
                             void* out, void* out2, int64_t ldo, const float* resid, const float* rowscale,
                             int rows_per_sample, int M, int N, int K, hipStream_t st) {
    if (K % (dtype == PA_BF16 ? 8 : 4)) return (int)hipErrorInvalidValue;
    if (dtype == PA_BF16)
        return linear_fwd_t<bf16>(epilogue, (const bf16*)x, ldx, (const bf16*)w, bias, out, out2, ldo, resid, rowscale, rows_per_sample, M, N, K, st);
    return linear_fwd_t<float>(epilogue, (const float*)x, ldx, (const float*)w, bias, out, out2, ldo, resid, rowscale, rows_per_sample, M, N, K, st);
}

template <typename T>
static int linear_pixshuf_t(const T* x, int64_t ldx, const T* w, const float* bias, T* out, int Bn, int Hp, int Wp,
                            int P, int C, int K, hipStream_t st) {
    const int M = Bn * Hp * Wp, N = P * P * C;
    if constexpr (std::is_same<T, bf16>::value) {
        if (g256::ok(M, N, K, false, false, ldx, K) && C % 8 == 0)
            return g256::launch<false, false>(x, ldx, w, K, Epi4PixShuf{out, bias, Hp, Wp, P, C, M, N}, M, N, K, 1, st);
    }
    OpN<T> A{x, (size_t)ldx, M, 0};
    OpN<T> B{w, (size_t)K, N, 0};
    return launch_gemm<T, 2, 2>(A, B, EpiPixShuf<T>{out, bias, Hp, Wp, P, C, M, N}, M, N, K, 1, 1, st);
}
extern "C" int pa_linear_pixshuf(int dtype, const void* x, int64_t ldx, const void* w, const float* bias, void* out_nhwc,
                                 int batch, int Hp, int Wp, int P, int C, int K, hipStream_t st) {
    if (K % 8) return (int)hipErrorInvalidValue;
    if (dtype == PA_BF16) return linear_pixshuf_t<bf16>((const bf16*)x, ldx, (const bf16*)w, bias, (bf16*)out_nhwc, batch, Hp, Wp, P, C, K, st);
    return linear_pixshuf_t<float>((const float*)x, ldx, (const float*)w, bias, (float*)out_nhwc, batch, Hp, Wp, P, C, K, st);
}

extern "C" int64_t pa_linear_dgrad_workspace_bytes(int M, int K) {
    const int64_t fast = (int64_t)2 * ((M + g256::BM_HALF - 1) / g256::BM_HALF) * K * sizeof(float);
    const int64_t slow = pa_colsum_workspace_bytes(M, K);
    return fast > slow ? fast : slow;
}
template <typename T>
static int linear_dgrad_t(const T* dy, int64_t lddy, const T* w, const typename GeluAux<T>::type* pre , T* dx, int64_t lddx, float* dx_colsum, float* ws, int M,
                          int N, int K, hipStream_t st) {
    if constexpr (std::is_same<T, bf16>::value) {
        if (g256::ok(M, K, N, false, true, lddy, K)) {
            if (pre && dx_colsum) {
                Epi4DGeluCS ep;
                ep.out = dx; ep.aux = pre; ep.ld = (size_t)lddx; ep.M = M; ep.N = K; ep.part = ws;
                int e = g256::launch<false, true>(dy, lddy, w, K, ep, M, K, N, 1, st);
                if (e) return e;
                return pa_slab_reduce(ws, dx_colsum, K, 2 * g256::row_tiles_used(M, K, 1), K, 0, st);
            }
            if (pre) return g256::launch<false, true>(dy, lddy, w, K, Epi4DGelu{dx, pre, (size_t)lddx, M, K}, M, K, N, 1, st);
            int e = g256::launch<false, true>(dy, lddy, w, K, Epi4Bias<bf16>{dx, (size_t)lddx, nullptr, M, K}, M, K, N, 1, st);
            if (e || dx_colsum == nullptr) return e;
            return pa_colsum(PA_BF16, dx, lddx, M, K, dx_colsum, ws, st);
        }
    }
    OpN<T> A{dy, (size_t)lddy, M, 0};
    OpT<T> B{w, (size_t)K, K, 0};
    int e;
    if (pre) e = launch_gemm<T, 2, 2>(A, B, EpiDGelu<T>{dx, pre, (size_t)lddx, M, K}, M, K, N, 1, 1, st);
    else e = launch_gemm<T, 2, 2>(A, B, EpiBias<T>{dx, (size_t)lddx, nullptr, M, K}, M, K, N, 1, 1, st);
    if (e || dx_colsum == nullptr) return e;
    return pa_colsum(std::is_same<T, bf16>::value ? PA_BF16 : PA_F32, dx, lddx, M, K, dx_colsum, ws, st);
}
extern "C" int pa_linear_dgrad(int dtype, const void* dy, int64_t lddy, const void* w, const void* gelu_aux,
                               void* dx, int64_t lddx, float* dx_colsum, void* workspace, int M, int N, int K, hipStream_t st) {
    if (N % 8 || K % 4) return (int)hipErrorInvalidValue;
    if (dx_colsum != nullptr && (workspace == nullptr || K % 8 || lddx % 8)) return (int)hipErrorInvalidValue;
    if (dtype == PA_BF16) return linear_dgrad_t<bf16>((const bf16*)dy, lddy, (const bf16*)w, (const unsigned char*)gelu_aux, (bf16*)dx, lddx, dx_colsum, (float*)workspace, M, N, K, st);
    return linear_dgrad_t<float>((const float*)dy, lddy, (const float*)w, (const float*)gelu_aux, (float*)dx, lddx, dx_colsum, (float*)workspace, M, N, K, st);
}

static bool wgrad_fast(int dtype, int M, int N, int K) {
    return dtype == PA_BF16 && g256::ok(N, K, M, true, true, N, K) && K % 4 == 0 && N % 256 == 0 && K % 256 == 0;
}
static int wgrad_fast_splits(int M, int N, int K) {
    const int tiles = (N / 256) * (K / 256);
    static const int env_target = [] { const char* v = getenv("PA_WGRAD_WGS"); return v ? atoi(v) : 0; }();
    int target = env_target > 0 ? env_target : (g256::g_dbg[3] > 0 ? g256::g_dbg[3] : 256);
    if (target < 16) target = 16;
    int s = (target + 3 * tiles / 4) / tiles;
    if (s < 1) s = 1;
    const int ktiles = M / 64;
    if (s > ktiles / 4) s = ktiles / 4 > 0 ? ktiles / 4 : 1;
    return g256::splits_used(M, s);
}
static int wgrad_splits(int M, int N, int K, int bk) {
    const int tiles = ((N + 127) / 128) * ((K + 127) / 128);
    const int nku = (M + bk - 1) / bk;
    int s = (640 + tiles - 1) / tiles;
    if (s > nku) s = nku;
    if (s > 64) s = 64;
    if (s < 1) s = 1;
    return s;
}
extern "C" int64_t pa_linear_wgrad_workspace_bytes(int dtype, int M, int N, int K) {
    if (wgrad_fast(dtype, M, N, K)) {
        const int s = wgrad_fast_splits(M, N, K);
        return s > 1 ? (int64_t)s * N * K * sizeof(float) : 0;
    }
    const int s = wgrad_splits(M, N, K, dtype == PA_BF16 ? 64 : 32);
    return s > 1 ? (int64_t)s * N * K * sizeof(float) : 0;
}
template <typename T>
static int linear_wgrad_t(const T* dy, int64_t lddy, const T* x, int64_t ldx, float* dw, float* ws, int M, int N, int K,
                          hipStream_t st) {
    if constexpr (std::is_same<T, bf16>::value) {
        if (wgrad_fast(PA_BF16, M, N, K) && g256::ok(N, K, M, true, true, lddy, ldx)) {
            const int s = wgrad_fast_splits(M, N, K);
            if (s == 1) return g256::launch<true, true>(dy, lddy, x, ldx, Epi4Slab{dw, (size_t)K, 0, N, K}, N, K, M, 1, st);
            int e = g256::launch<true, true>(dy, lddy, x, ldx, Epi4Slab{ws, (size_t)K, (size_t)N * K, N, K}, N, K, M, s, st);
            if (e) return e;
            return pa_slab_reduce(ws, dw, (int64_t)N * K, s, (int64_t)N * K, 0, st);
        }
    }
    OpT<T> A{dy, (size_t)lddy, N, 0};
    OpT<T> B{x, (size_t)ldx, K, 0};
    const int s = wgrad_splits(M, N, K, TT<T>::BK);
    if (s == 1) return launch_gemm<T, 2, 2>(A, B, EpiSlab{dw, (size_t)K, 0, N, K}, N, K, M, 1, 1, st);
    int e = launch_gemm<T, 2, 2>(A, B, EpiSlab{ws, (size_t)K, (size_t)N * K, N, K}, N, K, M, s, 1, st);
    if (e) return e;
    return pa_slab_reduce(ws, dw, (int64_t)N * K, s, (int64_t)N * K, 0, st);
}
extern "C" int pa_linear_wgrad(int dtype, const void* dy, int64_t lddy, const void* x, int64_t ldx, float* dw,
                               void* workspace, int M, int N, int K, hipStream_t st) {
    if (N % 4 || K % 4) return (int)hipErrorInvalidValue;
    if (dtype == PA_BF16) return linear_wgrad_t<bf16>((const bf16*)dy, lddy, (const bf16*)x, ldx, dw, (float*)workspace, M, N, K, st);
    return linear_wgrad_t<float>((const float*)dy, lddy, (const float*)x, ldx, dw, (float*)workspace, M, N, K, st);
}

extern "C" int pa_abi_version(void) { return PA_ABI_VERSION; }
extern "C" int pa_debug_get(int which) {
    if (which < 0 || which > 15) return -1;
    if (which == 9) return g_conv_wgrad_groups;
    if (which == 10) return g_ln_bwd_variant;
    if (which > 10) return g_misc_knob[which - 11];
    if (which == 6) return g_relpos_splits;
    if (which == 7) return g_attn3_fuse;
    if (which == 8) return g_attn_light_last;
    return g256::g_dbg[which];
}
extern "C" int pa_debug_set(int which, int value) {
    if (which < 0 || which > 15) return (int)hipErrorInvalidValue;
    if (which < 8) g256::g_dbg[which] = value;
    if (which == 9) g_conv_wgrad_groups = value;
    if (which == 10) g_ln_bwd_variant = value;
    if (which > 10) g_misc_knob[which - 11] = value;
    if (which == 6) g_relpos_splits = value;
    if (which == 7) g_attn3_fuse = value;
    if (which == 8) g_attn_light_last = value;
    return 0;
}
```

### painter_amd/csrc/gemm256.h

```cpp
#pragma once
#include "common.h"
#include <cstdlib>
#include <type_traits>

namespace g256 {

constexpr int BM = 256, BN = 256, BK = 64, NT = 512;
constexpr int LDS_BYTES = 131072;
inline int g_dbg[8] = {0, 0, 0, 0, 0, 0, 0, 0};
typedef __attribute__((address_space(3))) void lds_void;
typedef __attribute__((address_space(1))) const void gbl_cvoid;

DEVI constexpr int unit_off(bool isB, int sub, int stage) { return (isB ? 65536 : 0) + sub * 32768 + stage * 16384; }

template <int N> DEVI void wait_vm() { asm volatile("s_waitcnt vmcnt(%0)" ::"n"(N) : "memory"); }
DEVI void wait_lgkm0() { asm volatile("s_waitcnt lgkmcnt(0)" ::: "memory"); }

template <bool MM, bool IS_A>
DEVI uint32_t src_off(int tid, int j, int sub, int tile0, int rows, uint32_t ld) {
    const int cidx = j * NT + tid;
    if constexpr (!MM) {
        const int u = cidx >> 3, p = cidx & 7;
        const int kc = p ^ ((u >> 1) & 7);
        int row = IS_A ? ((u >> 6) * 128 + sub * 64 + (u & 63)) : ((u >> 5) * 64 + sub * 32 + (u & 31));
// ... 14 lines not shown
}
DEVI void dma16(const unsigned char* g, unsigned char* l) {
    __builtin_amdgcn_global_load_lds((gbl_cvoid*)g, (lds_void*)l, 16, 0, 0);
}

template <int OFF> DEVI void lds_read128(uint4& d, uint32_t addr) {
    asm volatile("ds_read_b128 %0, %1 offset:%2" : "=v"(d) : "v"(addr), "n"(OFF) : "memory");
}
template <int OFF> DEVI void lds_read64_tr(uint2& d, uint32_t addr) {
    asm volatile("ds_read_b64_tr_b16 %0, %1 offset:%2" : "=v"(d) : "v"(addr), "n"(OFF) : "memory");
}

template <bool MM> struct Frag4;
template <> struct Frag4<false> {
    uint4 q0, q1, q2, q3;
    template <int IMM> DEVI void read(const uint32_t (&base)[4], int) {
        lds_read128<IMM>(q0, base[0]);
        lds_read128<IMM>(q1, base[1]);
        lds_read128<IMM>(q2, base[2]);
        lds_read128<IMM>(q3, base[3]);
    }
    template <int KS> DEVI bf16x8 k() const {
        return __builtin_bit_cast(bf16x8, KS == 0 ? q0 : KS == 1 ? q1 : KS == 2 ? q2 : q3);
    }
};
template <> struct Frag4<true> {
    uint2 l0, h0, l1, h1, l2, h2, l3, h3;
    template <int IMM> DEVI void read(const uint32_t (&base)[4], int which_mb) {
        const uint32_t b = base[which_mb];
        lds_read64_tr<IMM + 0 * 4096>(l0, b);
        lds_read64_tr<IMM + 0 * 4096 + 1024>(h0, b);
        lds_read64_tr<IMM + 1 * 4096>(l1, b);
        lds_read64_tr<IMM + 1 * 4096 + 1024>(h1, b);
        lds_read64_tr<IMM + 2 * 4096>(l2, b);
        lds_read64_tr<IMM + 2 * 4096 + 1024>(h2, b);
        lds_read64_tr<IMM + 3 * 4096>(l3, b);
        lds_read64_tr<IMM + 3 * 4096 + 1024>(h3, b);
    }
    template <int KS> DEVI bf16x8 k() const {
        typedef __attribute__((ext_vector_type(2))) uint32_t u2;
        typedef __attribute__((ext_vector_type(4))) uint32_t u4;
        const uint2 l = KS == 0 ? l0 : KS == 1 ? l1 : KS == 2 ? l2 : l3;
        const uint2 h = KS == 0 ? h0 : KS == 1 ? h1 : KS == 2 ? h2 : h3;
        u2 lv = {l.x, l.y}, hv = {h.x, h.y};
        return __builtin_bit_cast(bf16x8, __builtin_shufflevector(lv, hv, 0, 1, 2, 3));
    }
};

template <class Epi> struct epi_colsum { static constexpr bool value = false; };
template <class Epi, class = void> struct epi_hi_off { static constexpr int value = 4; };
template <class Epi> struct epi_hi_off<Epi, std::void_t<decltype(Epi::HI_OFF)>> { static constexpr int value = Epi::HI_OFF; };
constexpr int BM_SHORT = 224;
constexpr int BM_HALF = 128;
template <bool AMM, bool BMM, int ILV, class Epi, bool SHORT = false, bool MIXED = false>
__global__ __launch_bounds__(NT) void gemm256_kernel(const bf16* __restrict__ Ag, uint32_t lda, const bf16* __restrict__ Bg,
                                                      uint32_t ldb, Epi epi, int M, int N, int ktiles, int ktiles_per_split,
                                                      int tiles_n, int stagger, int order, int nfull, int patch) {
    static_assert(!(SHORT && AMM), "the 224-row tile is built for a K-major A operand");
    static_assert(!(MIXED && (AMM || SHORT)), "half tiles are built for a K-major A operand and 256-row full tiles");
    constexpr int BMR = SHORT ? BM_SHORT : BM;
    extern __shared__ __attribute__((aligned(1024))) unsigned char smem[];
    const int tid = threadIdx.x, lane = tid & 63;
    if (stagger > 0 && blockIdx.x < 256 && blockIdx.y == 0) {
        const int64_t wait = ((int64_t)stagger * (((blockIdx.x >> 3) * 5) & 15)) >> 4;
        const uint64_t t0 = __builtin_amdgcn_s_memtime();
        while ((int64_t)(__builtin_amdgcn_s_memtime() - t0) < wait) __builtin_amdgcn_s_sleep(16);
    }
    const int wv = __builtin_amdgcn_readfirstlane(tid >> 6);
    const int wr = wv >> 2, wc = wv & 3;

    const bool htile = MIXED && (int)blockIdx.x >= nfull * tiles_n;
    const int nwg = MIXED ? (htile ? (int)gridDim.x - nfull * tiles_n : nfull * tiles_n) : (int)gridDim.x;
    const int bid = htile ? (int)blockIdx.x - nfull * tiles_n : (int)blockIdx.x;
    const int xq = nwg >> 3, xr = nwg & 7, xcd = bid & 7;
    int tile = (xcd < xr ? xcd * (xq + 1) : xr * (xq + 1) + (xcd - xr) * xq) + (bid >> 3);
    int split = blockIdx.y;
    if (gridDim.y > 1 && order == 0 && ((nwg * gridDim.y) & 7) == 0) {
        const int lin = blockIdx.y * nwg + bid;
        const int w = (lin & 7) * ((nwg * (int)gridDim.y) >> 3) + (lin >> 3);
        split = w / nwg;
        tile = w - split * nwg;
    }
    int tm, tn;
    if (order != 1) {
        const int TR = patch > 0 ? patch / 100 : 4, TC = patch > 0 ? patch % 100 : 8;
        const int tiles_m = MIXED ? (htile ? (M - nfull * BMR + BM_HALF - 1) / BM_HALF : nfull) : (M + BMR - 1) / BMR;
        const int per_group = TR * tiles_n;
        const int gm = tile / per_group, rem = tile - gm * per_group;
        const int rg = min(TR, tiles_m - gm * TR);
        const int full = tiles_n / TC;
        int cb = rem / (rg * TC), r2 = rem - cb * (rg * TC), cw = TC;
        if (cb >= full) {
            cb = full;
            r2 = rem - full * (rg * TC);
            cw = tiles_n - full * TC;
        }
        const int dm = r2 / cw;
        tm = gm * TR + dm;
        tn = cb * TC + (r2 - dm * cw);
    } else {
        tm = tile / tiles_n;
        tn = tile - tm * tiles_n;
    }
    const int i0 = htile ? nfull * BMR + tm * BM_HALF : tm * BMR, j0 = tn * BN;
    const bool blk3 = !(SHORT && wr == 1);
    const int kt0 = split * ktiles_per_split;
    const int nt = min(ktiles - kt0, ktiles_per_split);

    uint32_t oa[2][2], ob[2][2];
#pragma unroll
    for (int sub = 0; sub < 2; ++sub)
#pragma unroll
        for (int j = 0; j < 2; ++j) {
            oa[sub][j] = src_off<AMM, true>(tid, j, sub, i0, M, lda);
            ob[sub][j] = src_off<BMM, false>(tid, j, sub, j0, N, ldb);
        }
    const size_t a_step = AMM ? (size_t)BK * lda * 2 : (size_t)BK * 2;
    const size_t b_step = BMM ? (size_t)BK * ldb * 2 : (size_t)BK * 2;
    const unsigned char* abase = reinterpret_cast<const unsigned char*>(Ag) + (size_t)kt0 * a_step;
    const unsigned char* bbase = reinterpret_cast<const unsigned char*>(Bg) + (size_t)kt0 * b_step;
    unsigned char* const dma_dst = smem + wv * 1024;

    auto piece_a = [&](int sub, int stage, int kt, int j) {
        const unsigned char* s = sgpr_ptr(abase + (size_t)kt * a_step);
        dma16(s + oa[sub][j], dma_dst + unit_off(false, sub, stage) + j * 8192);
    };
    auto piece_b = [&](int sub, int stage, int kt, int j) {
        const unsigned char* s = sgpr_ptr(bbase + (size_t)kt * b_step);
        dma16(s + ob[sub][j], dma_dst + unit_off(true, sub, stage) + j * 8192);
    };
    auto stage_a = [&](int sub, int stage, int kt) { piece_a(sub, stage, kt, 0); piece_a(sub, stage, kt, 1); };
    auto stage_b = [&](int sub, int stage, int kt) { piece_b(sub, stage, kt, 0); piece_b(sub, stage, kt, 1); };

    uint32_t ra[4], rb[4];
    {
        const int lr = lane & 31, g = lane >> 5;
        const int t = ((lr >> 1) & 7) ^ g;
        const int i = lane & 15, half = (lane >> 4) & 1;
#pragma unroll
        for (int ks = 0; ks < 4; ++ks) {
            if constexpr (!AMM) ra[ks] = (uint32_t)((htile ? wr * 32768 + lr * 128 : (wr * 64 + lr) * 128) + ((t << 4) ^ (ks << 5)));
            if constexpr (!BMM) rb[ks] = (uint32_t)(65536 + (wc * 32 + lr) * 128 + ((t << 4) ^ (ks << 5)));
        }
        if constexpr (AMM) {
#pragma unroll
            for (int mb = 0; mb < 2; ++mb) {
                const int c = wr * 8 + mb * 4 + half * 2 + ((i & 3) >> 1);
                ra[mb] = (uint32_t)((g * 8 + (i >> 2)) * 256 + ((c ^ (4 * (i >> 2))) << 4) + (i & 1) * 8);
            }
            ra[2] = ra[3] = 0;
        }
        if constexpr (BMM) {
            const int c = wc * 4 + half * 2 + ((i & 3) >> 1);
            rb[0] = (uint32_t)(65536 + (g * 8 + (i >> 2)) * 256 + ((c ^ (4 * (i >> 2))) << 4) + (i & 1) * 8);
            rb[1] = rb[2] = rb[3] = 0;
        }
    }

    f32x16 acc[4][2];
#pragma unroll
    for (int a = 0; a < 4; ++a)
// ... 65 lines not shown
            pre(d0, d1);
            bar(); lwait();
            mma_quad(1, 1, fb1, d0, d1);
            bar();
        }
        {
            auto d0 = [&] { piece_b(0, S, t2, 0); };
            auto d1 = [&] { piece_b(0, S, t2, 1); };
            pre(d0, d1);
            bar();
            mma_quad(1, 0, fb0, d0, d1);
            bar();
        }
    };
    using I0 = std::integral_constant<int, 0>;
    using I1 = std::integral_constant<int, 1>;

    auto half_body = [&](auto stage_c, int T) {
        constexpr int S = decltype(stage_c)::value;
        const int t1 = min(T + 1, nt - 1);
#define G256_HMMA(KS, NC) \
        acc[0][NC] = __builtin_amdgcn_mfma_f32_32x32x16_bf16((NC ? fb1 : fb0).template k<KS>(), fa0.template k<KS>(), acc[0][NC], 0, 0, 0); \
        acc[1][NC] = __builtin_amdgcn_mfma_f32_32x32x16_bf16((NC ? fb1 : fb0).template k<KS>(), fa1.template k<KS>(), acc[1][NC], 0, 0, 0);
#define G256_HDMA(X) __builtin_amdgcn_sched_barrier(0); X; __builtin_amdgcn_sched_barrier(0);
        fa0.template read<unit_off(false, 0, S)>(ra, 0);
        fa1.template read<unit_off(false, 0, S) + 4096>(ra, 1);
        fb0.template read<unit_off(true, 0, S) - 65536>(rb, 0);
        lwait();
        __builtin_amdgcn_s_setprio(1);
        G256_HMMA(0, 0) G256_HDMA(piece_a(0, S ^ 1, t1, 0))
        G256_HMMA(1, 0) G256_HDMA(piece_a(1, S ^ 1, t1, 0))
        G256_HMMA(2, 0) G256_HDMA(piece_b(0, S ^ 1, t1, 0))
        G256_HMMA(3, 0) G256_HDMA(piece_b(0, S ^ 1, t1, 1))
        __builtin_amdgcn_s_setprio(0);
        wait_vm<4>();
        bar();
        fb1.template read<unit_off(true, 1, S) - 65536>(rb, 0);
        lwait();
        __builtin_amdgcn_s_setprio(1);
        G256_HMMA(0, 1) G256_HDMA(piece_b(1, S ^ 1, t1, 0))
        G256_HMMA(1, 1) G256_HMMA(2, 1) G256_HDMA(piece_b(1, S ^ 1, t1, 1))
        G256_HMMA(3, 1)
        __builtin_amdgcn_s_setprio(0);
        wait_vm<2>();
        bar();
#undef G256_HMMA
#undef G256_HDMA
    };

    bool ran_half = false;
    if constexpr (MIXED) {
        if (htile) {
            ran_half = true;
            piece_a(0, 0, 0, 0); piece_a(1, 0, 0, 0); stage_b(0, 0, 0); stage_b(1, 0, 0);
            wait_vm<0>();
            bar();
            for (int T = 0; T < nt; T += 2) {
                half_body(I0{}, T);
                half_body(I1{}, T + 1);
            }
        }
    }
    if (!ran_half) {
        stage_a(0, 0, 0);
        stage_b(0, 0, 0);
        stage_b(1, 0, 0);
        stage_a(1, 0, 0);
        stage_a(0, 1, 1);
        stage_b(0, 1, 1);
        wait_vm<8>();
        bar();
        if (wr == 1) bar();

        for (int T = 0; T < nt; T += 2) {
            tile_body(I0{}, T);
            tile_body(I1{}, T + 1);
        }
    }
    if (wr == 0 && !ran_half) bar();
    wait_vm<0>();

    bar();
    {
        float* stg = reinterpret_cast<float*>(smem + wv * 8704);
        constexpr int HO = epi_hi_off<Epi>::value;
        static_assert(HO == 4 || (HO == 32 && !epi_colsum<Epi>::value), "epilogue column layouts: 8 consecutive, or 4 + 4 at a distance of 32");
        const int lr = lane & 31, g = lane >> 5, rrow = lane >> 3, c0 = (lane & 7) * (HO == 4 ? 8 : 4);
        const int jcol = j0 + wc * 64 + c0;
        const typename Epi::Col col = epi.col(jcol);
        const int rbase = i0 + wr * (htile ? 64 : 128);
        float cs[8] = {0.f, 0.f, 0.f, 0.f, 0.f, 0.f, 0.f, 0.f};
#pragma unroll
        for (int hf = 0; hf < 2; ++hf) {
            if (MIXED && htile && hf != 0) continue;
            typename Epi::Row rows[2][4];
#pragma unroll
            for (int m2 = 0; m2 < 2; ++m2)
#pragma unroll
                for (int st = 0; st < 4; ++st) {
                    const int mb = hf * 2 + m2;
                    if (SHORT && mb == 3 && !blk3) continue;
                    rows[m2][st] = epi.row(rbase + (mb >> 1) * 64 + (mb & 1) * 32 + st * 8 + rrow, jcol);
                }
#pragma unroll
            for (int m2 = 0; m2 < 2; ++m2) {
                const int mb = hf * 2 + m2;
                if (SHORT && mb == 3 && !blk3) continue;
#pragma unroll
                for (int nb = 0; nb < 2; ++nb)
#pragma unroll
                    for (int q = 0; q < 4; ++q) {
                        const f32x16& c = acc[mb][nb];
                        *reinterpret_cast<float4*>(stg + lr * 68 + nb * 32 + q * 8 + g * 4) =
                            make_float4(c[q * 4 + 0], c[q * 4 + 1], c[q * 4 + 2], c[q * 4 + 3]);
                    }
                const int ib = rbase + (mb >> 1) * 64 + (mb & 1) * 32;
#pragma unroll
                for (int st = 0; st < 4; ++st) {
                    const int r = st * 8 + rrow;
                    const float4 lo = *reinterpret_cast<const float4*>(stg + r * 68 + c0);
                    const float4 hi = *reinterpret_cast<const float4*>(stg + r * 68 + c0 + HO);
                    if constexpr (epi_colsum<Epi>::value) epi.store_cs(ib + r, jcol, lo, hi, col, rows[m2][st], split, cs);
                    else epi.store(ib + r, jcol, lo, hi, col, rows[m2][st], split);
                }
            }
        }
        if constexpr (epi_colsum<Epi>::value) {
#pragma unroll
            for (int e = 0; e < 8; ++e) {
                float v = cs[e];
                v += lane_dpp<0x128>(v);
                v += lane_xor16(v);
                v += lane_xor32(v);
                cs[e] = v;
            }
            if (lane < 8) epi.colsum_out((htile ? nfull + tm : tm) * 2 + wr, jcol, cs);
        }
    }
}

static inline int per_split(int ktiles, int nsplit) {
    int per = (ktiles + nsplit - 1) / nsplit;
    return per + (per & 1);
}
template <bool AMM, bool BMM, int ILV, bool SHORT, class Epi, bool MIXED = false>
static int launch_ilv(const bf16* A, size_t lda, const bf16* B, size_t ldb, Epi epi, int M, int N, int K, int nsplit, hipStream_t st, int nfull = 0);
#ifndef G256_ILV_DEFAULT
#define G256_ILV_DEFAULT 2
#endif
static inline bool use_short(int M, int N, int nsplit, bool amm) {
    if (amm || nsplit != 1 || M < BM) return false;
    if (g_dbg[4] == 1) return false;
    if (g_dbg[4] == 2) return true;
    static const int cost = [] { const char* v = getenv("PA_G256_SHORT_COST"); return v ? atoi(v) : 92; }();
    const int tiles_n = (N + BN - 1) / BN;
    const long t256 = (long)((M + BM - 1) / BM) * tiles_n, t224 = (long)((M + BM_SHORT - 1) / BM_SHORT) * tiles_n;
    const long r256 = (t256 + 255) / 256 * 100, r224 = (t224 + 255) / 256 * cost;
    return r224 < r256;
}
struct TilePlan { bool is_short, mixed; int nfull; };
static inline TilePlan tile_plan(int M, int N, int nsplit, bool amm) {
    TilePlan p{use_short(M, N, nsplit, amm), false, 0};
    if (amm || nsplit != 1 || M < 2 * BM || g_misc_knob[1] == 1 || g_dbg[4] != 0) return p;
    if (g_misc_knob[1] == 2 && g_misc_knob[3] > 0 && (long)g_misc_knob[3] * BM < M) return TilePlan{false, true, g_misc_knob[3]};
    static const int cs = [] { const char* v = getenv("PA_G256_SHORT_COST"); return v ? atoi(v) : 97; }();
    static const int ch = [] { const char* v = getenv("PA_G256_HALF_COST"); return v ? atoi(v) : 75; }();
    const int tn = (N + BN - 1) / BN;
    auto rounds = [](long t) { return (t + 255) / 256; };
    long best = p.is_short ? rounds((long)((M + BM_SHORT - 1) / BM_SHORT) * tn) * cs : rounds((long)((M + BM - 1) / BM) * tn) * 100;
    for (int r = 1; r <= 64; ++r) {
        const int nf = (int)((long)r * 256 / tn);
        if (nf < 1) continue;
        if ((long)nf * BM >= M) break;
        const long nh = (M - (long)nf * BM + BM_HALF - 1) / BM_HALF;
        const long c = (long)r * 100 + rounds(nh * tn) * ch;
        if (c <= best - 5) { best = c + 5; p = TilePlan{false, true, nf}; }
    }
    return p;
}
template <bool AMM, bool BMM, class Epi>
static int launch(const bf16* A, size_t lda, const bf16* B, size_t ldb, Epi epi, int M, int N, int K, int nsplit,
                  hipStream_t st) {
    if constexpr (!AMM) {
        const TilePlan tp = tile_plan(M, N, nsplit, AMM);
        if (tp.mixed) return launch_ilv<AMM, BMM, G256_ILV_DEFAULT, false, Epi, true>(A, lda, B, ldb, epi, M, N, K, nsplit, st, tp.nfull);
        if (tp.is_short) return launch_ilv<AMM, BMM, G256_ILV_DEFAULT, true>(A, lda, B, ldb, epi, M, N, K, nsplit, st);
    }
#ifdef G256_ILV_AB
    static const int env_ilv = [] { const char* v = getenv("PA_G256_ILV"); return v ? atoi(v) : G256_ILV_DEFAULT; }();
    const int ilv = g_dbg[5] > 0 ? g_dbg[5] - 1 : env_ilv;
    if (ilv == 2) return launch_ilv<AMM, BMM, 2, false>(A, lda, B, ldb, epi, M, N, K, nsplit, st);
    if (ilv == 1) return launch_ilv<AMM, BMM, 1, false>(A, lda, B, ldb, epi, M, N, K, nsplit, st);
    return launch_ilv<AMM, BMM, 0, false>(A, lda, B, ldb, epi, M, N, K, nsplit, st);
#else
    return launch_ilv<AMM, BMM, G256_ILV_DEFAULT, false>(A, lda, B, ldb, epi, M, N, K, nsplit, st);
#endif
}
template <bool AMM, bool BMM, int ILV, bool SHORT, class Epi, bool MIXED>
static int launch_ilv(const bf16* A, size_t lda, const bf16* B, size_t ldb, Epi epi, int M, int N, int K, int nsplit, hipStream_t st, int nfull) {
    auto kern = gemm256_kernel<AMM, BMM, ILV, Epi, SHORT, MIXED>;
    static bool attr_done = false;
    if (!attr_done) {
        hipError_t e = hipFuncSetAttribute(reinterpret_cast<const void*>(kern), hipFuncAttributeMaxDynamicSharedMemorySize, LDS_BYTES);
        if (e != hipSuccess) return (int)e;
        attr_done = true;
    }
    constexpr int BMR = SHORT ? BM_SHORT : BM;
    static const int env_patch = [] { const char* v = getenv("PA_G256_PATCH"); return v ? atoi(v) : 0; }();
    const int tiles_n = (N + BN - 1) / BN;
    const int tiles_m = MIXED ? nfull + (M - nfull * BMR + BM_HALF - 1) / BM_HALF : (M + BMR - 1) / BMR;
    const int ktiles = K / BK;
    const int per = per_split(ktiles, nsplit);
    const int splits = (ktiles + per - 1) / per;
    if (g_dbg[1]) epi.M = 0;
    PA_LAUNCH(kern, dim3(tiles_m * tiles_n, splits), dim3(NT), LDS_BYTES, st, A, (uint32_t)lda, B, (uint32_t)ldb, epi, M, N,
              ktiles, per, tiles_n, g_dbg[0], g_dbg[2], nfull, g_misc_knob[0] > 0 ? g_misc_knob[0] : env_patch);
    return (int)hipGetLastError();
}
static inline int row_tiles_used(int M, int N, int nsplit) {
    const TilePlan tp = tile_plan(M, N, nsplit, false);
    const int bm = tp.is_short ? BM_SHORT : BM;
    if (tp.mixed) return tp.nfull + (M - tp.nfull * bm + BM_HALF - 1) / BM_HALF;
    return (M + bm - 1) / bm;
}
static inline bool ok(int M, int N, int K, bool amm, bool bmm, size_t lda, size_t ldb) {
    if (K % (2 * BK) || M < 8 || N < 8 || N % 8) return false;
    if (amm && (M % 8)) return false;
    if (bmm && (N % 8)) return false;
    if ((lda % 8) || (ldb % 8)) return false;
    const size_t abytes = (amm ? (size_t)BK * lda + M : (size_t)M * lda) * 2, bbytes = (bmm ? (size_t)BK * ldb + N : (size_t)N * ldb) * 2;
    return abytes < (1ull << 32) && bbytes < (1ull << 32);
}
static inline int splits_used(int K, int nsplit) {
    const int ktiles = K / BK, per = per_split(ktiles, nsplit);
    return (ktiles + per - 1) / per;
}

}
```

### painter_amd/engine.py

```python
import os

import torch

from . import hostmath, ops
from ._lib import EPI_BIAS, EPI_BIAS_F32, EPI_BIAS_RESID


_DBG_KEEP = os.environ.get("PAINTER_AMD_DEBUG_KEEPALIVE", "0") == "1"
_DBG_SERIAL = os.environ.get("PAINTER_AMD_DEBUG_SERIAL", "0") == "1"
_SIDE_EXTRA = os.environ.get("PAINTER_AMD_SIDE_EXTRA", "1") != "0"
_DBG_TRACE = os.environ.get("PAINTER_AMD_DEBUG_TRACE", "0") == "1"


_ATTN_PREP = os.environ.get("PAINTER_AMD_ATTN_PREP", "fused")
_FC1_COLSUM = os.environ.get("PAINTER_AMD_FC1_COLSUM", "epilogue")
_SIDE_STREAM = os.environ.get("PAINTER_AMD_SIDE_STREAM", "1") != "0"
_SIDE_PRIORITY = int(os.environ.get("PAINTER_AMD_SIDE_PRIORITY", "0"))
_RELPOS_PACK = os.environ.get("PAINTER_AMD_RELPOS_PACK", "batch")
_configured = False
WGRAD_SIDE_TARGET = 96
RELPOS_SIDE_SPLITS = 8


def _configure_library():
# ... 163 lines not shown
            st.clear()
        elif st:
            st["ver"] = [None] * len(st["ver"])

    def invalidate(self):
        self._wcache.clear()
        self._pcache.clear()
        self._rcache.clear()

    def shadow_buffers(self):
        return {key[1]: ent[1] for key, ent in self._wcache.items()}

    def mark_fresh(self, params):
        by_ptr = {p.data_ptr(): p for p in params}
        for key, ent in list(self._wcache.items()):
            p = by_ptr.get(key[1])
            if p is not None:
                self._wcache[key] = (p._version, ent[1])

    def forward(self, P, imgs, tgts, mask_u8, valid, seg_type=None, merge_between_batch=-1, drop_scales=None, need_grad=True, want=None):
        c, T = self.cfg, self.T
        dev = imgs.device
        B = imgs.shape[0]
        L, D = c.L, c.D
        S = _Saved()
        S.B, S.need_grad = B, need_grad
        keep = lambda n: need_grad and (want is None or n in want)
        S.imgs, S.tgts, S.mask, S.valid = imgs, tgts, mask_u8, valid
        S.drop = drop_scales
        S.seg_type = seg_type if c.seggpt else None
        pe = P["pos_embed"][0, c.cls:]
        pos = ops.pos_fwd(self.pos_operator(dev)[0], pe, L, D)
        tok_args = (P["patch_embed.proj.bias"], P["mask_token"], P["segment_token_x"], P["segment_token_y"], pos, mask_u8,
                    P.get("type_token_cls") if c.seggpt else None, P.get("type_token_ins") if c.seggpt else None,
                    seg_type if c.seggpt else None)
        S.cols = None
        if ops.patch_cols_ok(T, B, L, c.P, D):
            cols = ops.patch_im2col(imgs, tgts, B, c.Hp, c.Wp, c.P)
            x = ops.patch_embed_fwd_cols(cols, self.w_patch(P), *tok_args, B, L, D)
            if keep("patch_embed.proj.weight"):
                S.cols = cols
        else:
            x = ops.patch_embed_fwd(T, imgs, tgts, self.w_patch(P), *tok_args, B, c.Hp, c.Wp, c.P, D)
        concat = torch.empty((B * L, 4 * D), dtype=T, device=dev)
        S.blocks, S.taps = [], []
        Bc = 2 * B
        for i in range(c.depth):
            pre = "blocks.%d." % i
            R = Bc * L
            merge = 0
            if c.seggpt and merge_between_batch >= 0 and i >= merge_between_batch:
                merge = 1 if c.merge_idx >= i else 2
            ds_a, ds_m = (None, None) if drop_scales is None else drop_scales[i]
            ln1, mean1, rstd1 = ops.layernorm_fwd(x, P[pre + "norm1.weight"], P[pre + "norm1.bias"], c.ln_eps, T)
            qkv = ops.linear_fwd(ln1, self.w(pre + "attn.qkv.weight", P), P[pre + "attn.qkv.bias"], EPI_BIAS)
            rcat = self.relpos(pre, P, False)
            ao, lse, atab = ops.attn_fwd(qkv, rcat, Bc, L, c.heads, c.Hp, c.Wp, c.scale, need_tables=True) if need_grad else \
                ops.attn_fwd(qkv, rcat, Bc, L, c.heads, c.Hp, c.Wp, c.scale) + (None,)
            group = 0
            if merge > 0:
                a = ops.linear_fwd(ao, self.w(pre + "attn.proj.weight", P), P[pre + "attn.proj.bias"], EPI_BIAS_F32)
                group = Bc // 2 if merge == 1 else Bc
                if ds_a is None:
                    x1 = ops.ensemble_resid(x, a, Bc, group, L, D)
                else:
                    e = ops.ensemble_resid(torch.zeros_like(x), a, Bc, group, L, D)
                    x1 = ops.ensemble_resid(x, ops.scale_cast(torch.float32, e, ds_a, L), Bc, 1, L, D)
                    del e
            else:
                x1 = ops.linear_fwd(ao, self.w(pre + "attn.proj.weight", P), P[pre + "attn.proj.bias"], EPI_BIAS_RESID,
                                    resid=x, rowscale=ds_a, rows_per_sample=L)
            ln2, mean2, rstd2 = ops.layernorm_fwd(x1, P[pre + "norm2.weight"], P[pre + "norm2.bias"], c.ln_eps, T)
            act, gaux = ops.linear_gelu(ln2, self.w(pre + "mlp.fc1.weight", P), P[pre + "mlp.fc1.bias"], need_aux=need_grad)
            x2 = ops.linear_fwd(act, self.w(pre + "mlp.fc2.weight", P), P[pre + "mlp.fc2.bias"], EPI_BIAS_RESID,
                                resid=x1, rowscale=ds_m, rows_per_sample=L)
            if need_grad:
                S.blocks.append((x, mean1, rstd1, ln1, qkv, rcat, ao, lse, x1, mean2, rstd2, ln2, gaux, act, Bc, atab, group))
            x = x2
            if i == c.merge_idx:
                Bc = B
                x = ops.merge_fwd(x, B * L, D)
            if i in c.taps:
                k = c.taps.index(i)
                _, mt, rt = ops.layernorm_fwd(x, P["norm.weight"], P["norm.bias"], c.ln_eps, T, out=concat[:, k * D:(k + 1) * D])
                if need_grad:
                    S.taps.append((x, mt, rt))
        E = ops.linear_pixshuf(concat, self.w("decoder_embed.weight", P), P["decoder_embed.bias"], B, c.Hp, c.Wp, c.P, c.dec)
        w3r, wf = ops.conv3x3_pack(P["decoder_pred.0.weight"], T)
        w1 = P["decoder_pred.3.weight"].reshape(3, c.dec)
        pred, y3 = ops.decoder_tail_fwd(E, w3r, P["decoder_pred.0.bias"], P["decoder_pred.1.weight"], P["decoder_pred.1.bias"],
                                        w1, P["decoder_pred.3.bias"], 1e-6, save_y3=need_grad)
        loss_out = ops.loss_fwd(pred, tgts, valid, mask_u8, c.P, ignore_rule=not c.seggpt,
                                eps_den=0.0 if c.seggpt else 1e-2, kind=c.loss_func)
        pred_patch = ops.patchify(pred, c.Hp, c.Wp, c.P)
        if need_grad:
            S.y3, S.pred, S.loss_out, S.wf = y3, pred, loss_out, wf
            S.concat = concat if keep("decoder_embed.weight") else None
            S.E = E if keep("decoder_pred.0.weight") else None
        return loss_out, pred, pred_patch, S

    def backward(self, P, S, dloss, sync=None, want=None, want_imgs=False, want_tgts=False, dpatch=None):
        c, T = self.cfg, self.T
        B, L, D = S.B, c.L, c.D
        dev = S.imgs.device
        G = {}
        if sync is not None:
            want = None
        need = (lambda n: True) if want is None else (lambda n: n in want)
        main = torch.cuda.current_stream(dev)
        side = self.side_stream(dev) if self.use_side_stream and (want is None or len(want) > 0) else None
        keep = []
        self.trace = []

        def tr(name, t):
            if _DBG_TRACE:
                self.trace.append((name, t.detach().double().abs().sum()))

        filt = getattr(self, "side_filter", None)

        def param_grads(wname, bname, dy, x, bout=None):
            if not need(wname) and (bname in G or not need(bname)):
                return
            if not need(wname) or not need(bname):
                def one():
                    if need(wname):
                        G[wname] = ops.linear_wgrad(dy, x)
                    if bname not in G and need(bname):
                        G[bname] = ops.colsum(dy, out=bout)
# ... 49 lines not shown
        dpred_loss = None
        if dpatch is None:
            dpred = ops.loss_bwd(S.pred, S.tgts, S.valid, S.mask, dloss, S.loss_out, c.P, c.loss_func)
            if want_tgts:
                dpred_loss = dpred
        else:
            dpred, dpred_loss = ops.pred_bwd(S.pred, S.tgts, S.valid, S.mask, dloss, S.loss_out, dpatch, c.P, c.loss_func,
                                             want_loss_term=want_tgts and dloss is not None)
        w1 = P["decoder_pred.3.weight"].reshape(3, c.dec)
        dy3, tg = ops.decoder_tail_bwd_pointwise(dpred, S.y3, P["decoder_pred.1.weight"], P["decoder_pred.1.bias"], w1, 1e-6)
        G["decoder_pred.1.weight"] = tg[0:64]
        G["decoder_pred.1.bias"] = tg[64:128]
        G["decoder_pred.3.weight"] = tg[128:320].reshape(3, c.dec, 1, 1)
        G["decoder_pred.3.bias"] = tg[320:323]
        npix = B * c.H * c.W
        if want is None:
            G["decoder_pred.0.weight"], G["decoder_pred.0.bias"] = on_side(
                lambda: (ops.conv3x3_wgrad(dy3, S.E), ops.colsum(dy3.view(npix, c.dec))), dy3, S.E)
        elif need("decoder_pred.0.weight") or need("decoder_pred.0.bias"):
            G["decoder_pred.0.weight"], G["decoder_pred.0.bias"] = on_side(
                lambda: (ops.conv3x3_wgrad(dy3, S.E) if need("decoder_pred.0.weight") else None,
                         ops.colsum(dy3.view(npix, c.dec)) if need("decoder_pred.0.bias") else None),
                *[t for t in (dy3, S.E) if t is not None])
        dE = ops.conv3x3_dgrad_unshuffle(dy3, S.wf, B, c.Hp, c.Wp, c.P)
        del dy3
        param_grads("decoder_embed.weight", "decoder_embed.bias", dE, S.concat)
        dconcat = ops.linear_dgrad(dE, self.w("decoder_embed.weight", P))
        tr("dE", dE); tr("dconcat", dconcat)
        del dE
        ready(["decoder_embed.weight", "decoder_embed.bias"])
        ready([n for n in G if n.startswith("decoder_pred.")])
        dnorm = None
        dx = None
        dyT_next = None
        flats = {}

        def block_flat(i_):
            if i_ not in flats:
                nrp_, hd_ = rc_shape
                sizes = [2 * D, 2 * D, 3 * D, D, c.hidden, D, nrp_ * hd_]
                fb = torch.empty((sum(sizes),), dtype=torch.float32, device=dev)
                if side is not None:
                    fb.record_stream(side)
                flats[i_] = (fb, dict(zip(("n1", "n2", "qkv", "proj", "fc1", "fc2", "rel"), torch.split(fb, sizes))))
            return flats[i_]

        rc_shape = tuple(S.blocks[-1][5].shape)
        for i in reversed(range(c.depth)):
            pre = "blocks.%d." % i
            x0, mean1, rstd1, ln1, qkv, rcat, ao, lse, x1, mean2, rstd2, ln2, gaux, act, Bc, atab, ens_group = S.blocks[i]
            S.blocks[i] = None
            R = Bc * L
            ds_a, ds_m = (None, None) if S.drop is None else S.drop[i]
            nrp, hd = rcat.shape
            flat, fl = block_flat(i)
            del flats[i]
            if i in c.taps:
                k = c.taps.index(i)
                xt, mt, rt = S.taps[k]
                dyT = torch.empty((R, D), dtype=T, device=dev)
                dx, gb = ops.layernorm_bwd(dconcat[:, k * D:(k + 1) * D], xt, mt, rt, P["norm.weight"], dres=dx, dx=dx, dxT=dyT,
                                           rowscale=ds_m, rows_per_sample=L, dxT_colsum=fl["fc2"])
                G[pre + "mlp.fc2.bias"] = fl["fc2"]
                if need("norm.weight") or need("norm.bias"):
                    dnorm = gb if dnorm is None else _add_(dnorm, gb)
            elif i == c.merge_idx:
                dx, dyT = ops.merge_bwd(T, dx, ds_m, L, B * L, D)
            else:
                dyT = dyT_next
            param_grads(pre + "mlp.fc2.weight", pre + "mlp.fc2.bias", dyT, act, fl["fc2"])
            tr("%d.dyT" % i, dyT)
            if _FC1_COLSUM == "epilogue":
                dpre = ops.linear_dgrad(dyT, self.w(pre + "mlp.fc2.weight", P), gelu_aux=gaux, colsum_out=fl["fc1"])
                G[pre + "mlp.fc1.bias"] = fl["fc1"]
            else:
                dpre = ops.linear_dgrad(dyT, self.w(pre + "mlp.fc2.weight", P), gelu_aux=gaux)
            tr("%d.dpre" % i, dpre)
            param_grads(pre + "mlp.fc1.weight", pre + "mlp.fc1.bias", dpre, ln2, fl["fc1"])
            dln2 = ops.linear_dgrad(dpre, self.w(pre + "mlp.fc1.weight", P))
            tr("%d.dln2" % i, dln2)
            del dpre
            dyA = torch.empty_like(dyT) if side is not None else dyT
            lnws, lndone = self.ln_workspace(dev, ops.layernorm_bwd_workspace_bytes(R, D), main, side if _SIDE_EXTRA else None)
            dx, fin = ops.layernorm_bwd(dln2, x1, mean2, rstd2, P[pre + "norm2.weight"], dres=dx, dx=dx, dxT=dyA,
                                        rowscale=ds_a, rows_per_sample=L, gb=fl["n2"].view(2, D), dxT_colsum=fl["proj"], defer=True, ws=lnws)
            gb = None
            if need(pre + "norm2.weight") or need(pre + "norm2.bias") or need(pre + "attn.proj.bias"):
                gb = on_side(fin)
                lndone()
                G[pre + "norm2.weight"], G[pre + "norm2.bias"] = gb[0], gb[1]
            G[pre + "attn.proj.bias"] = fl["proj"]
            del dyT
            tr("%d.dx_ln2" % i, dx); tr("%d.dyA" % i, dyA)
            if gb is not None:
                tr("%d.gb2" % i, gb)
            if ens_group > 0:
                da = ops.ensemble_resid(torch.zeros_like(dx), dx if ds_a is None else ops.scale_cast(torch.float32, dx, ds_a, L), Bc, ens_group, L, D)
                dyA = da if T == torch.float32 else ops.cast_bf16(da, out=dyA)
                del da
            param_grads(pre + "attn.proj.weight", pre + "attn.proj.bias", dyA, ao, fl["proj"])
            dao = ops.linear_dgrad(dyA, self.w(pre + "attn.proj.weight", P), out=dln2)
            tr("%d.dao" % i, dao)
            del dyA
            rcatT = self.relpos(pre, P, True)
            dqkv, dG = ops.attn_bwd_core(qkv, rcat, rcatT, ao, dao, lse, Bc, L, c.heads, c.Hp, c.Wp, c.scale, tables=atab, prep=_ATTN_PREP)
            if need(pre + "attn.rel_pos_h") or need(pre + "attn.rel_pos_w"):
                drcat = on_side(lambda: ops.attn_bwd_relpos(dG, qkv, nrp, Bc, L, c.heads, c.Hp, c.Wp, out=fl["rel"].view(nrp, hd)), dG, qkv)
                nh, nw = 2 * c.Hp - 1, 2 * c.Wp - 1
                G[pre + "attn.rel_pos_h"] = drcat[:nh]
                G[pre + "attn.rel_pos_w"] = drcat[nh:nh + nw]
            del dG
            tr("%d.dqkv" % i, dqkv)
            param_grads(pre + "attn.qkv.weight", pre + "attn.qkv.bias", dqkv, ln1, fl["qkv"])
            dln1 = ops.linear_dgrad(dqkv, self.w(pre + "attn.qkv.weight", P), out=dao)
            del dqkv
            nxt = i - 1
            dyT_next = None
            if nxt >= 0 and nxt not in c.taps and nxt != c.merge_idx:
                dyT_next = torch.empty((R, D), dtype=T, device=dev)
            ds_next = None if (S.drop is None or nxt < 0) else S.drop[nxt][1]
            cs_next = None
            if dyT_next is not None:
                cs_next = block_flat(nxt)[1]["fc2"]
                G["blocks.%d.mlp.fc2.bias" % nxt] = cs_next
            lnws, lndone = self.ln_workspace(dev, ops.layernorm_bwd_workspace_bytes(R, D), main, side if _SIDE_EXTRA else None)
            dx, fin = ops.layernorm_bwd(dln1, x0, mean1, rstd1, P[pre + "norm1.weight"], dres=dx, dx=dx, dxT=dyT_next,
                                        rowscale=ds_next if dyT_next is not None else None, rows_per_sample=L, gb=fl["n1"].view(2, D),
                                        dxT_colsum=cs_next, defer=True, ws=lnws)
            if need(pre + "norm1.weight") or need(pre + "norm1.bias") or (cs_next is not None and need("blocks.%d.mlp.fc2.bias" % nxt)):
                gb = on_side(fin)
                lndone()
                G[pre + "norm1.weight"], G[pre + "norm1.bias"] = gb[0], gb[1]
            tr("%d.dx_ln1" % i, dx)
            del x0, ln1, qkv, ao, x1, ln2, gaux, act, atab
            ready([n for n in G if n.startswith(pre)], flat=flat)
        if dnorm is not None:
            G["norm.weight"], G["norm.bias"] = dnorm[0], dnorm[1]
        dpe, sums = ops.tokens_bwd(T, dx, S.mask, B, L, D)
        if need("patch_embed.proj.weight"):
            if S.cols is not None:
                G["patch_embed.proj.weight"] = ops.linear_wgrad(dpe, S.cols).view(D, 3, c.P, c.P)
            else:
                G["patch_embed.proj.weight"] = ops.patch_embed_wgrad(dpe, S.imgs, S.tgts, B, c.Hp, c.Wp, c.P, D).view(D, 3, c.P, c.P)
        if need("patch_embed.proj.bias"):
            G["patch_embed.proj.bias"] = ops.colsum(dpe)
        if need("pos_embed"):
            dposemb = torch.zeros_like(P["pos_embed"])
            ops.pos_bwd(self.pos_operator(dev)[1], sums[0], sums[1], dposemb[0, c.cls:], c.src * c.src, D)
            G["pos_embed"] = dposemb
        for k_, nm in enumerate(("segment_token_x", "segment_token_y", "mask_token")):
            if need(nm):
                G[nm] = ops.colsum(sums[k_]).view(1, 1, 1, D)
        small_tail = []
        if c.seggpt and S.seg_type is not None and (need("type_token_cls") or need("type_token_ins")):
            types_present = set(S.seg_type.reshape(-1).tolist())
            for t_, nm in ((0.0, "type_token_cls"), (1.0, "type_token_ins")):
                if (t_ not in types_present and sync is None) or not need(nm):
                    continue
                w = (S.seg_type.reshape(-1) == t_).to(torch.float32)
                sel = ops.scale_cast(torch.float32, dx, torch.cat((w, w)).contiguous(), L)
                G[nm] = ops.colsum(sel).view(1, 1, 1, D)
                small_tail.append(nm)
        ready(["norm.weight", "norm.bias", "patch_embed.proj.weight", "patch_embed.proj.bias", "pos_embed",
               "segment_token_x", "segment_token_y", "mask_token"] + small_tail)
        dimgs = dtgts = None
        if want_imgs or want_tgts:
            dimgs, dtgts = ops.patch_embed_dgrad(dpe, self.w_patch(P), B, c.Hp, c.Wp, c.P, D, want_imgs, want_tgts,
# ... 24 lines not shown
```

### painter_amd/ops.py

```python
import torch

from ._lib import (EPI_BIAS, EPI_BIAS_F32, EPI_BIAS_GELU, EPI_BIAS_RESID, PA_BF16, PA_F32, check, lib)

_WS = {}


def stream():
    return torch.cuda.current_stream().cuda_stream


def code(dtype):
    if dtype == torch.bfloat16:
        return PA_BF16
    if dtype == torch.float32:
        return PA_F32
    raise TypeError("painter_amd supports float32 / bfloat16 operand types, got %s" % dtype)


def p(t):
    return 0 if t is None else t.data_ptr()


def workspace(nbytes, device, slot=0):
    key = (device, slot, torch.cuda.current_stream(device).cuda_stream)
    buf = _WS.get(key)
    if buf is None or buf.numel() < nbytes:
        buf = torch.empty(max(int(nbytes), 1 << 20), dtype=torch.uint8, device=device)
        _WS[key] = buf
    return buf


def _req(t, dtype=None):
    assert t.is_cuda and t.stride(-1) == 1, "device tensor with unit inner stride required"
    if dtype is not None:
        assert t.dtype == dtype, (t.dtype, dtype)
    return t


def linear_fwd(x, w, bias, epilogue=EPI_BIAS, out=None, out2=None, resid=None, rowscale=None, rows_per_sample=1):
    M, K = x.shape
    N = w.shape[0]
    T = x.dtype
    _req(x); _req(w, T)
    assert w.is_contiguous() and w.shape[1] == K
    if out is None:
        odt = torch.float32 if epilogue in (EPI_BIAS_F32, EPI_BIAS_RESID) else T
        out = torch.empty((M, N), dtype=odt, device=x.device)
    if epilogue == EPI_BIAS_RESID:
        assert resid is not None and resid.dtype == torch.float32 and resid.stride(0) == out.stride(0)
    check(lib.pa_linear_fwd(code(T), epilogue, p(x), x.stride(0), p(w), p(bias), p(out), p(out2), out.stride(0),
                            p(resid), p(rowscale), rows_per_sample, M, N, K, stream()), "pa_linear_fwd")
    return out


def linear_gelu(x, w, bias, need_aux=True):
    M = x.shape[0]
    N = w.shape[0]
    act = torch.empty((M, N), dtype=x.dtype, device=x.device)
    aux = torch.empty((M, N), dtype=gelu_aux_dtype(x.dtype), device=x.device) if need_aux else None
    assert aux is None or aux.stride(0) == act.stride(0)
    linear_fwd(x, w, bias, EPI_BIAS_GELU, out=act, out2=aux)
    return act, aux


G8_OFF, G8_RANGE = 0.13, 1.26


def gelu_aux_dtype(T):
    return torch.float32 if T == torch.float32 else torch.uint8


def gelu_aux_decode(aux):
    return aux.to(torch.float32) * (G8_RANGE / 255.0) - G8_OFF


def gelu_aux_encode(g):
    return torch.clamp(torch.floor((g.double() + G8_OFF) * (255.0 / G8_RANGE) + 0.5), 0, 255).to(torch.uint8)


def linear_pixshuf(x, w, bias, batch, Hp, Wp, P, C):
    T = x.dtype
    out = torch.empty((batch, Hp * P, Wp * P, C), dtype=T, device=x.device)
    check(lib.pa_linear_pixshuf(code(T), p(x), x.stride(0), p(w), p(bias), p(out), batch, Hp, Wp, P, C, x.shape[1],
                                stream()), "pa_linear_pixshuf")
    return out


def linear_dgrad(dy, w, gelu_aux=None, out=None, colsum_out=None):
    M, N = dy.shape
    K = w.shape[1]
    T = dy.dtype
    _req(dy); _req(w, T)
    if out is None:
        out = torch.empty((M, K), dtype=T, device=dy.device)
    if gelu_aux is not None:
        assert gelu_aux.stride(0) == out.stride(0) and gelu_aux.dtype == gelu_aux_dtype(T), (gelu_aux.dtype, gelu_aux.stride(0), out.stride(0))
    ws = None
    if colsum_out is not None:
        assert colsum_out.shape == (K,) and colsum_out.dtype == torch.float32 and colsum_out.is_contiguous()
        ws = workspace(lib.pa_linear_dgrad_workspace_bytes(M, K), dy.device, slot=2)
    check(lib.pa_linear_dgrad(code(T), p(dy), dy.stride(0), p(w), p(gelu_aux), p(out), out.stride(0), p(colsum_out), p(ws), M, N, K, stream()),
          "pa_linear_dgrad")
    return out


def linear_wgrad(dy, x, out=None):
    M, N = dy.shape
    K = x.shape[1]
    T = dy.dtype
    _req(dy); _req(x, T)
    if out is None:
        out = torch.empty((N, K), dtype=torch.float32, device=dy.device)
    ws = workspace(lib.pa_linear_wgrad_workspace_bytes(code(T), M, N, K), dy.device)
    check(lib.pa_linear_wgrad(code(T), p(dy), dy.stride(0), p(x), x.stride(0), p(out), p(ws), M, N, K, stream()),
          "pa_linear_wgrad")
    return out


def colsum(x, out=None):
    M, N = x.shape
    if out is None:
        out = torch.empty((N,), dtype=torch.float32, device=x.device)
    ws = workspace(lib.pa_colsum_workspace_bytes(M, N), x.device)
    check(lib.pa_colsum(code(x.dtype), p(x), x.stride(0), M, N, p(out), p(ws), stream()), "pa_colsum")
    return out


def layernorm_fwd(x, gamma, beta, eps, out_dtype, out=None):
    R, D = x.shape
    _req(x, torch.float32)
    if out is None:
        out = torch.empty((R, D), dtype=out_dtype, device=x.device)
    mean = torch.empty((R,), dtype=torch.float32, device=x.device)
    rstd = torch.empty((R,), dtype=torch.float32, device=x.device)
    check(lib.pa_layernorm_fwd(code(out.dtype), p(x), x.stride(0), p(gamma), p(beta), eps, p(out), out.stride(0),
                               p(mean), p(rstd), R, D, stream()), "pa_layernorm_fwd")
    return out, mean, rstd


def layernorm_bwd_workspace_bytes(R, D):
    return int(lib.pa_layernorm_bwd_workspace_bytes(R, D))


def layernorm_bwd(dy, x, mean, rstd, gamma, dres=None, dx=None, dxT=None, rowscale=None, rows_per_sample=1, gb=None, dxT_colsum=None, defer=False, ws=None):
    R, D = x.shape
    if dx is None:
        dx = torch.empty((R, D), dtype=torch.float32, device=x.device)
    if gb is None:
        gb = torch.empty((2, D), dtype=torch.float32, device=x.device)
    assert gb.shape == (2, D) and gb.is_contiguous() and gb.dtype == torch.float32
    nbytes = lib.pa_layernorm_bwd_workspace_bytes(R, D)
    if defer:
        if ws is None:
            ws = torch.empty((nbytes,), dtype=torch.uint8, device=x.device)
        assert ws.dtype == torch.uint8 and ws.numel() >= nbytes and ws.is_contiguous()
    else:
        ws = workspace(nbytes, x.device)
    if dxT_colsum is not None:
        assert dxT is not None and dxT_colsum.shape == (D,) and dxT_colsum.dtype == torch.float32 and dxT_colsum.is_contiguous()
    check(lib.pa_layernorm_bwd(code(dy.dtype), p(dy), dy.stride(0), p(x), x.stride(0), p(mean), p(rstd), p(gamma),
                               p(dres), p(dx), dx.stride(0), p(dxT), 0 if dxT is None else dxT.stride(0), p(rowscale),
                               rows_per_sample, 0 if defer else p(gb), p(dxT_colsum), p(ws), R, D, stream()), "pa_layernorm_bwd")
    if not defer:
        return dx, gb

    def finish():
        check(lib.pa_layernorm_bwd_reduce(p(ws), p(gb), p(dxT_colsum), int(dxT_colsum is not None), R, D, stream()), "pa_layernorm_bwd_reduce")
        return gb
    finish.buffer = ws
    return dx, finish


def relpos_pack(rel_pos_h, rel_pos_w, Hp, Wp, dtype):
    nrp = lib.pa_relpos_rows_padded(Hp, Wp)
    hd = rel_pos_h.shape[1]
    assert rel_pos_h.shape == (2 * Hp - 1, hd) and rel_pos_w.shape == (2 * Wp - 1, hd)
    rcat = torch.empty((nrp, hd), dtype=dtype, device=rel_pos_h.device)
    check(lib.pa_relpos_pack(code(dtype), p(rel_pos_h), p(rel_pos_w), p(rcat), Hp, Wp, hd, stream()), "pa_relpos_pack")
    return rcat


def relpos_pack_batch(tabs, nblocks, Hp, Wp, hd, dtype, rcat=None, rcatT=None):
    nrp = lib.pa_relpos_rows_padded(Hp, Wp)
    assert tabs.dtype == torch.int64 and tabs.numel() == 2 * nblocks and tabs.is_cuda and tabs.is_contiguous()
    if rcat is None:
        rcat = torch.empty((nblocks, nrp, hd), dtype=dtype, device=tabs.device)
    if rcatT is None:
        rcatT = torch.empty((nblocks, hd, nrp), dtype=dtype, device=tabs.device)
    assert rcat.shape == (nblocks, nrp, hd) and rcatT.shape == (nblocks, hd, nrp) and rcat.is_contiguous() and rcatT.is_contiguous()
    assert rcat.dtype == dtype and rcatT.dtype == dtype
    check(lib.pa_relpos_pack_batch(code(dtype), p(tabs), p(rcat), p(rcatT), nblocks, Hp, Wp, hd, stream()), "pa_relpos_pack_batch")
    return rcat, rcatT


def attn_fwd(qkv, rcat, batch, L, heads, Hp, Wp, scale, need_tables=False):
    T = qkv.dtype
    hd = rcat.shape[1]
    assert qkv.shape[1] == 3 * heads * hd
    out = torch.empty((batch * L, heads * hd), dtype=T, device=qkv.device)
    lse = torch.empty((batch * heads, L), dtype=torch.float32, device=qkv.device)
    tables = None
    if need_tables:
        nb = lib.pa_attn_tables_bytes(code(T), batch, L, heads, Hp, Wp, hd)
        if nb > 0:
            tables = torch.empty((nb,), dtype=torch.uint8, device=qkv.device)
    check(lib.pa_attn_fwd(code(T), p(qkv), qkv.stride(0), p(rcat), p(out), out.stride(0), p(lse), p(tables), batch, L, heads,
                          Hp, Wp, hd, float(scale), stream()), "pa_attn_fwd")
    return (out, lse, tables) if need_tables else (out, lse)


def attn_launch_counts():
    import ctypes
    buf = (ctypes.c_longlong * 6)()
    check(lib.pa_attn_launch_counts(ctypes.addressof(buf)), "pa_attn_launch_counts")
    v = [int(x) for x in buf]
    return {"fwd": tuple(v[:3]), "bwd": tuple(v[3:])}


def relpos_pack_t(rel_pos_h, rel_pos_w, Hp, Wp, dtype):
    nrp = lib.pa_relpos_rows_padded(Hp, Wp)
    hd = rel_pos_h.shape[1]
    rcatT = torch.empty((hd, nrp), dtype=dtype, device=rel_pos_h.device)
    check(lib.pa_relpos_pack_t(code(dtype), p(rel_pos_h), p(rel_pos_w), p(rcatT), Hp, Wp, hd, stream()), "pa_relpos_pack_t")
    return rcatT


def attn_bwd_core(qkv, rcat, rcatT, out, dout, lse, batch, L, heads, Hp, Wp, scale, tables=None, prep="fused"):
    T = qkv.dtype
    dev = qkv.device
    nrp, hd = rcat.shape
    delta = None
    o_arg = None
    if tables is not None and lib.pa_attn_bwd_prep_ok(code(T), L, Hp, Wp, hd):
        if prep == "fused":
            o_arg = out
        else:
            check(lib.pa_attn_bwd_prep(code(T), p(out), out.stride(0), p(dout), dout.stride(0), p(lse), p(tables), batch, L, heads, Hp, Wp, hd,
                                       float(scale), stream()), "pa_attn_bwd_prep")
    else:
        delta = torch.empty((batch * heads, L), dtype=torch.float32, device=dev)
        check(lib.pa_attn_bwd_delta(code(T), p(out), out.stride(0), p(dout), dout.stride(0), p(delta), batch, L, heads, hd,
                                    stream()), "pa_attn_bwd_delta")
    dqkv = torch.empty_like(qkv)
    nb = lib.pa_attn_bwd_relpos_partials_bytes(code(T), batch, L, heads, Hp, Wp, hd) if tables is not None else 0
    dG = part = None
    if nb > 0:
        part = torch.empty((nb,), dtype=torch.uint8, device=dev)
    else:
        dG = torch.empty((batch * L, heads * nrp), dtype=T, device=dev)
    aux = workspace(lib.pa_attn_bwd_aux_bytes(batch, L, heads, Hp, Wp), dev, slot=1)
    check(lib.pa_attn_bwd(code(T), p(qkv), qkv.stride(0), p(rcat), p(rcatT), p(dout), dout.stride(0), p(lse), p(delta),
                          p(dqkv), p(dG), p(part), p(aux), p(tables), p(o_arg), 0 if o_arg is None else o_arg.stride(0), batch, L, heads, Hp, Wp, hd,
                          float(scale), stream()), "pa_attn_bwd")
    return dqkv, (dG if part is None else part)


def attn_bwd_relpos(dG, qkv, nrp, batch, L, heads, Hp, Wp, out=None):
    T = qkv.dtype
    hd = qkv.shape[1] // (3 * heads)
    drcat = out if out is not None else torch.empty((nrp, hd), dtype=torch.float32, device=qkv.device)
    assert drcat.shape == (nrp, hd) and drcat.is_contiguous()
    ws = workspace(lib.pa_attn_bwd_relpos_workspace_bytes(code(T), batch, L, heads, Hp, Wp, hd), qkv.device)
    if dG.dtype == torch.uint8:
        check(lib.pa_attn_bwd_relpos_reduce(p(dG), p(drcat), p(ws), batch, L, heads, Hp, Wp, hd, stream()), "pa_attn_bwd_relpos_reduce")
        return drcat
    check(lib.pa_attn_bwd_relpos(code(T), p(dG), p(qkv), qkv.stride(0), p(drcat), p(ws), batch, L, heads, Hp, Wp, hd,
                                 stream()), "pa_attn_bwd_relpos")
    return drcat


def attn_bwd(qkv, rcat, rcatT, out, dout, lse, batch, L, heads, Hp, Wp, scale, tables=None):
    dqkv, dG = attn_bwd_core(qkv, rcat, rcatT, out, dout, lse, batch, L, heads, Hp, Wp, scale, tables=tables)
    return dqkv, attn_bwd_relpos(dG, qkv, rcat.shape[0], batch, L, heads, Hp, Wp)


def cast_bf16(x, out=None):
    if out is None:
        out = torch.empty(x.shape, dtype=torch.bfloat16, device=x.device)
    check(lib.pa_cast_bf16(p(x), p(out), x.numel(), stream()), "pa_cast_bf16")
    return out


def pos_fwd(op, pe, L, D):
    idx, val = op
    assert idx.dtype == torch.int32 and val.dtype == torch.float32 and idx.shape == val.shape == (L, idx.shape[1])
    pos = torch.empty((L, D), dtype=torch.float32, device=pe.device)
    check(lib.pa_pos_fwd(p(idx), p(val), idx.shape[1], p(pe), p(pos), L, D, stream()), "pa_pos_fwd")
    return pos


def pos_bwd(opT, gx, gy, dpe, S, D):
    idx, val = opT
    assert idx.dtype == torch.int32 and val.dtype == torch.float32 and idx.shape == val.shape == (S, idx.shape[1])
    check(lib.pa_pos_bwd(p(idx), p(val), idx.shape[1], p(gx), p(gy), p(dpe), S, D, stream()), "pa_pos_bwd")


def patch_weight_pack(w, T, P, out=None):
    D = w.shape[0]
    kp = (3 * P * P + 7) // 8 * 8
    if out is None:
        out = torch.empty((D, kp), dtype=T, device=w.device)
    check(lib.pa_patch_weight_pack(code(T), p(w), p(out), D, P, stream()), "pa_patch_weight_pack")
    return out


def patch_embed_fwd(T, imgs, tgts, w, bias, mask_token, seg_x, seg_y, pos, mask_u8, type_cls, type_ins, seg_type,
# ... 168 lines not shown
```

Baseline: 159.0 images/sec.

## Skip attention and linear work for DropPath-dropped samples

Threads a per-sample DropPath keep/drop vector (rowskip) into the attention forward/backward kernels and the linear forward/dgrad GEMMs, so samples whose residual branch is dropped skip compute and only write zeros to outputs, LSE, tables and partials. The aim is to avoid spending FLOPs on branches whose contribution is multiplied by zero in training mode. It adds new skip variants of kernels and ABI entry points, extra zero-fill writes, and a dependency on the drop mask being on the device. The dropped work is mathematically multiplied by zero, so this is legitimate conditional computation rather than an approximation.

```diff
diff --git a/include/painter_hip.h b/include/painter_hip.h
--- a/include/painter_hip.h
+++ b/include/painter_hip.h
@@ -19,7 +19,7 @@
     PA_EPI_BIAS_RESID = 3
 };
 
-#define PA_ABI_VERSION 6
+#define PA_ABI_VERSION 7
 int pa_abi_version(void);
 int pa_debug_set(int which, int value);
 int pa_debug_get(int which);
@@ -28,12 +28,18 @@
                   const float* bias , void* out, void* out2, int64_t ldo, const float* resid ,
                   const float* rowscale , int rows_per_sample, int M, int N, int K,
                   hipStream_t stream);
+int pa_linear_fwd_skip(int dtype, int epilogue, const void* x, int64_t ldx, const void* w, const float* bias, void* out, void* out2,
+                       int64_t ldo, const float* resid, const float* rowscale, int rows_per_sample, int M, int N, int K,
+                       const float* rowskip, int skip_rows_per_sample, hipStream_t stream);
 int pa_linear_pixshuf(int dtype, const void* x, int64_t ldx, const void* w , const float* bias,
                       void* out_nhwc, int batch, int Hp, int Wp, int P, int C, int K, hipStream_t stream);
 int64_t pa_linear_dgrad_workspace_bytes(int M, int K);
 int pa_linear_dgrad(int dtype, const void* dy , int64_t lddy, const void* w ,
                     const void* gelu_aux , void* dx , int64_t lddx, float* dx_colsum,
                     void* workspace, int M, int N, int K, hipStream_t stream);
+int pa_linear_dgrad_skip(int dtype, const void* dy, int64_t lddy, const void* w, const void* gelu_aux, void* dx, int64_t lddx, float* dx_colsum,
+                         void* workspace, int M, int N, int K, const float* rowskip , int skip_rows_per_sample,
+                         hipStream_t stream);
 int64_t pa_linear_wgrad_workspace_bytes(int dtype, int M, int N, int K);
 int pa_linear_wgrad(int dtype, const void* dy , int64_t lddy, const void* x , int64_t ldx,
                     float* dw , void* workspace, int M, int N, int K, hipStream_t stream);
@@ -63,6 +69,9 @@
 int pa_attn_trace(int enable, unsigned long long* host_out);
 int pa_attn_fwd(int dtype, const void* qkv, int64_t ldq, const void* rcat, void* out, int64_t ldo, float* lse,
                 void* tables, int batch, int L, int heads, int Hp, int Wp, int head_dim, float scale, hipStream_t stream);
+int pa_attn_fwd_skip(int dtype, const void* qkv, int64_t ldq, const void* rcat, void* out, int64_t ldo, float* lse,
+                     void* tables, int batch, int L, int heads, int Hp, int Wp, int head_dim, float scale, const float* rowskip ,
+                     hipStream_t stream);
 
 int pa_relpos_pack_t(int dtype, const float* rel_pos_h, const float* rel_pos_w, void* rcatT, int Hp, int Wp, int head_dim,
                      hipStream_t stream);
@@ -77,6 +86,10 @@
                 int64_t lddo, const float* lse, const float* delta, void* dqkv, void* dG, void* relpos_part, void* aux,
                 void* tables, const void* out, int64_t ldo, int batch, int L, int heads, int Hp, int Wp, int head_dim, float scale,
                 hipStream_t stream);
+int pa_attn_bwd_skip(int dtype, const void* qkv, int64_t ldq, const void* rcat, const void* rcatT, const void* dout,
+                     int64_t lddo, const float* lse, const float* delta, void* dqkv, void* dG, void* relpos_part, void* aux,
+                     void* tables, const void* out, int64_t ldo, int batch, int L, int heads, int Hp, int Wp, int head_dim, float scale,
+                     const float* rowskip , hipStream_t stream);
 int64_t pa_attn_bwd_relpos_workspace_bytes(int dtype, int batch, int L, int heads, int Hp, int Wp, int head_dim);
 int pa_attn_bwd_relpos_reduce(const void* relpos_part, float* drcat, void* workspace, int batch, int L, int heads, int Hp, int Wp,
                               int head_dim, hipStream_t stream);
diff --git a/painter_amd/csrc/attn3.h b/painter_amd/csrc/attn3.h
--- a/painter_amd/csrc/attn3.h
+++ b/painter_amd/csrc/attn3.h
@@ -3,10 +3,10 @@
 bool attn3_ok(int L, int Hp, int Wp);
 int64_t attn3_table_bytes(int Bn, int L, int H, int Hp, int Wp);
 int attn3_fwd(const bf16* qkv, int64_t ldq, const bf16* rcat, bf16* out, int64_t ldo, float* lse, void* tables, int Bn, int L, int H,
-              int Hp, int Wp, float scale, hipStream_t st);
+              int Hp, int Wp, float scale, hipStream_t st, const float* rowskip = nullptr);
 int attn3_bwd(const bf16* qkv, int64_t ldq, const bf16* rcatT, const bf16* dout, int64_t lddo, const float* lse, const float* delta,
               void* tables, bf16* dqkv, bf16* dG, float* part, int Bn, int L, int H, int Hp, int Wp, float scale, const bf16* out, int64_t ldo,
-              hipStream_t st);
+              hipStream_t st, const float* rowskip = nullptr);
 int attn3_bwd_prep(const bf16* out, int64_t ldo, const bf16* dout, int64_t lddo, const float* lse, void* tables, int Bn, int L, int H, int Hp,
                    float scale, hipStream_t st);
 int64_t attn3_relpos_partials_bytes(int Bn, int L, int H, int Hp, int Wp);
diff --git a/painter_amd/csrc/attn3.hip b/painter_amd/csrc/attn3.hip
--- a/painter_amd/csrc/attn3.hip
+++ b/painter_amd/csrc/attn3.hip
@@ -17,22 +17,25 @@
 
 namespace a3 {
 
-template <int STAGES>
+template <int STAGES, bool SKIP = false>
 __global__ __launch_bounds__(NT, STAGES == 1 ? 4 : 2) void fwd_kernel(const bf16* __restrict__ qkv, size_t ldq, const bf16* __restrict__ rcat,
                                                                       bf16* __restrict__ out, size_t ldo, float* __restrict__ lse,
                                                                       unsigned char* __restrict__ tables, int L, int H, int Hp, int NRP,
-                                                                      float scale, int nblk, int xcd_map, int abl) {
+                                                                      float scale, int nblk, int xcd_map, int abl, const float* __restrict__ rowskip) {
     extern __shared__ __attribute__((aligned(16))) unsigned char smem[];
     const int tid = threadIdx.x, lane = tid & 63, wave = tid >> 6, g = lane >> 5, ql = lane & 31;
     int blk, bh;
-    wg_coords(nblk, xcd_map, blk, bh, (L / 32) / NW);
+    bool drop = false;
+    if constexpr (SKIP) drop = wg_coords_skip(nblk, xcd_map, blk, bh, rowskip, H);
+    else wg_coords(nblk, xcd_map, blk, bh, (L / 32) / NW);
     const int b = bh / H, h = bh % H, D = H * ATT_HD;
     const bf16* base = qkv + (size_t)b * L * ldq + h * ATT_HD;
     const bf16* kbase = base + D;
     const bf16* vbase = base + 2 * D;
     const int qt = blk * NW + wave;
-    const bool valid = qt * 32 < L;
+    const bool valid = qt * 32 < L && !drop;
     const int q = qt * 32 + ql;
+    const int ntile = L / 32;
     unsigned char* thT = smem + STAGES * STAGE_QK + wave * Hp * 64;
     unsigned char* eimg = smem + STAGES * STAGE_QK + NW * Hp * 64;
     unsigned char* twimg = eimg + wave * 2048;
@@ -40,7 +43,6 @@
     la.init(lane);
     EAddr ea;
     ea.init(lane);
-    const int ntile = L / 32;
     Stager ks, vs;
     ks.load(kbase, ldq, tid);
     vs.load(vbase, ldq, tid);
@@ -139,7 +141,7 @@
         }
         __syncthreads();
     };
-    for (int a = 0; a < ((abl & 16) ? 0 : Hp / RPP); ++a) {
+    for (int a = 0; a < (((abl & 16) || drop) ? 0 : Hp / RPP); ++a) {
         body(std::integral_constant<int, 0>{}, a);
         body(std::integral_constant<int, 1>{}, a);
         body(std::integral_constant<int, 2>{}, a);
@@ -166,6 +168,14 @@
         stage_rows(stg, oacc, 1.f / lt, lane);
         write_rows(stg, out + (size_t)(b * L + qt * 32) * ldo + h * ATT_HD, ldo, lane);
     }
+    if (drop && qt * 32 < L) {
+        zero_rows(out + (size_t)(b * L + qt * 32) * ldo + h * ATT_HD, ldo, lane);
+        if (g == 0) lse[(size_t)bh * L + q] = 0.f;
+        if (tables != nullptr) {
+            unsigned char* tt = tables + ((size_t)bh * ntile + qt) * ttile_bytes(Hp);
+            for (int c = lane; c < ttile_bytes(Hp) / 16; c += 64) *reinterpret_cast<uint4*>(tt + c * 16) = zero4();
+        }
+    }
 }
 
 __device__ unsigned long long g_trace[2 * 2 * 64 * 8];
@@ -176,7 +186,7 @@
                                                           unsigned char* __restrict__ tables, bf16* __restrict__ dqkv,
                                                           bf16* __restrict__ dG, float* __restrict__ part, int L, int H, int Hp, int NRP,
                                                           float scale, int nblk, int xcd_map, int abl, int tile0, int pslot0,
-                                                          const bf16* __restrict__ oatt, size_t ldo) {
+                                                          const bf16* __restrict__ oatt, size_t ldo, const float* __restrict__ rowskip) {
     extern __shared__ __attribute__((aligned(16))) unsigned char smem[];
     const int tid = threadIdx.x, lane = tid & 63, wave = tid >> 6, g = lane >> 5, ql = lane & 31;
     const int trwg = blockIdx.x == 0 ? 0 : (blockIdx.x == gridDim.x / 2 ? 1 : -1);
@@ -189,8 +199,10 @@
         }
     };
     coarse(60);
-    int blk, bh;
-    wg_coords(nblk, xcd_map, blk, bh, (L / 32 - tile0) / NW);
+    int blk, bh, pslot = blockIdx.x;
+    bool drop = false;
+    if (rowskip != nullptr) drop = wg_coords_skip(nblk, xcd_map, blk, bh, rowskip, H, &pslot);
+    else wg_coords(nblk, xcd_map, blk, bh, (L / 32 - tile0) / NW);
     const int b = bh / H, h = bh % H, D = H * ATT_HD;
     const bf16* base = qkv + (size_t)b * L * ldq + h * ATT_HD;
     const bf16* kbase = base + D;
@@ -199,6 +211,22 @@
     const bool valid = qt * 32 < L;
     const int q = qt * 32 + ql;
     const int qh = q / WP, qw = q % WP;
+    if (drop) {
+        if (valid) {
+            zero_rows(dqkv + (size_t)(b * L + qt * 32) * ldq + h * ATT_HD, ldq, lane);
+            if (g == 0) *reinterpret_cast<float*>(tables + ((size_t)bh * (L / 32) + qt) * ttile_bytes(Hp) + 2048 + (Hp + 2) * 64 + ql * 4) = 0.f;
+            if constexpr (!FUSE) {
+                bf16* dgrow = dG + ((size_t)(b * L + qt * 32) * H + h) * NRP;
+                for (int c = lane; c < 32 * (NRP / 8); c += 64)
+                    *reinterpret_cast<uint4*>(dgrow + (size_t)(c / (NRP / 8)) * H * NRP + (c % (NRP / 8)) * 8) = zero4();
+            }
+        }
+        if constexpr (FUSE) {
+            float4* pw = reinterpret_cast<float4*>(part + (size_t)(pslot0 + pslot) * NRP * ATT_HD);
+            for (int c = tid; c < NRP * ATT_HD / 4; c += NT) pw[c] = make_float4(0.f, 0.f, 0.f, 0.f);
+        }
+        return;
+    }
     unsigned char* thT = smem + 2 * STAGE_QK + wave * Hp * 64;
     unsigned char* eimg = smem + 2 * STAGE_QK + NW * Hp * 64;
     unsigned char* rimg = eimg + PH * EIMG;
@@ -470,7 +498,7 @@
                 *reinterpret_cast<uint4*>(wimg + nimg * IMG + ql * 128 + (((2 * s + g) ^ rsw) << 4)) = __builtin_bit_cast(uint4, qf[s]);
         }
         __syncthreads();
-        float* pw = part + (size_t)(pslot0 + blockIdx.x) * NRP * ATT_HD;
+        float* pw = part + (size_t)(pslot0 + pslot) * NRP * ATT_HD;
         for (int u = wave; u < 2 * (NRP / 32); u += NW) {
             const int rb = u >> 1, db = u & 1;
             f32x16 acc = zero16();
@@ -494,16 +522,27 @@
 template <int MINW>
 __global__ __launch_bounds__(NT, MINW) void bwd_dkv_kernel(const bf16* __restrict__ qkv, size_t ldq, const bf16* __restrict__ dout,
                                                            size_t lddo, const unsigned char* __restrict__ tables, bf16* __restrict__ dqkv,
-                                                           int L, int H, int Hp, float scale, int nblk, int xcd_map, int abl, int tile0) {
+                                                           int L, int H, int Hp, float scale, int nblk, int xcd_map, int abl, int tile0,
+                                                           const float* __restrict__ rowskip) {
     extern __shared__ __attribute__((aligned(16))) unsigned char smem[];
     const int tid = threadIdx.x, lane = tid & 63, wave = tid >> 6, g = lane >> 5, ql = lane & 31;
     int blk, bh;
-    wg_coords(nblk, xcd_map, blk, bh, (L / 32 - tile0) / NW);
+    bool drop = false;
+    if (rowskip != nullptr) drop = wg_coords_skip(nblk, xcd_map, blk, bh, rowskip, H);
+    else wg_coords(nblk, xcd_map, blk, bh, (L / 32 - tile0) / NW);
     const int b = bh / H, h = bh % H, D = H * ATT_HD;
     const bf16* qbase = qkv + (size_t)b * L * ldq + h * ATT_HD;
     const bf16* dobase = dout + (size_t)b * L * lddo + h * ATT_HD;
     const int kt = tile0 + blk * NW + wave;
     const bool valid = kt * 32 < L;
+    if (drop) {
+        if (valid) {
+            bf16* orow = dqkv + (size_t)(b * L + kt * 32) * ldq + h * ATT_HD;
+            zero_rows(orow + D, ldq, lane);
+            zero_rows(orow + 2 * D, ldq, lane);
+        }
+        return;
+    }
     const int key = kt * 32 + ql;
     const int kh = key / WP, kw = key % WP;
     const int khlo = ((tile0 + blk * NW) * 32) / WP;
@@ -745,17 +784,19 @@
 }
 
 int attn3_fwd(const bf16* qkv, int64_t ldq, const bf16* rcat, bf16* out, int64_t ldo, float* lse, void* tables, int Bn, int L, int H,
-              int Hp, int Wp, float scale, hipStream_t st) {
+              int Hp, int Wp, float scale, hipStream_t st, const float* rowskip) {
     using namespace a3;
     const int NRP = pa_relpos_rows_padded(Hp, Wp);
+    if (Bn > 63) rowskip = nullptr;
     static const int stages = [] { const char* v = getenv("PA_ATTN3_FWD_STAGES"); return v ? atoi(v) : 1; }();
     const size_t smem = (size_t)(stages == 2 ? 2 : 1) * STAGE_QK + (size_t)NW * Hp * 64 + PH * EIMG;
     static bool done1 = false, done2 = false;
-    auto kern = stages == 2 ? fwd_kernel<2> : fwd_kernel<1>;
-    if (int e = set_smem(reinterpret_cast<const void*>(kern), stages == 2 ? done2 : done1)) return e;
+    static bool done1s = false, done2s = false;
+    auto kern = rowskip != nullptr ? (stages == 2 ? fwd_kernel<2, true> : fwd_kernel<1, true>) : (stages == 2 ? fwd_kernel<2> : fwd_kernel<1>);
+    if (int e = set_smem(reinterpret_cast<const void*>(kern), rowskip != nullptr ? (stages == 2 ? done2s : done1s) : (stages == 2 ? done2 : done1))) return e;
     const int nblk = (L / 32 + NW - 1) / NW;
     PA_LAUNCH(kern, dim3(nblk * Bn * H), dim3(NT), smem, st, qkv, (size_t)ldq, rcat, out, (size_t)ldo, lse,
-              reinterpret_cast<unsigned char*>(tables), L, H, Hp, NRP, scale, nblk, a3_xcd_map_on(), [] { const char* v = getenv("PA_ATTN3_FWD_ABL"); return v ? atoi(v) : 0; }());
+              reinterpret_cast<unsigned char*>(tables), L, H, Hp, NRP, scale, nblk, a3_xcd_map_on(), [] { const char* v = getenv("PA_ATTN3_FWD_ABL"); return v ? atoi(v) : 0; }(), rowskip);
     return (int)hipGetLastError();
 }
 
@@ -809,10 +850,11 @@
 
 int attn3_bwd(const bf16* qkv, int64_t ldq, const bf16* rcatT, const bf16* dout, int64_t lddo, const float* lse, const float* delta,
               void* tables, bf16* dqkv, bf16* dG, float* part, int Bn, int L, int H, int Hp, int Wp, float scale, const bf16* out, int64_t ldo,
-              hipStream_t st) {
+              hipStream_t st, const float* rowskip) {
     using namespace a3;
     const int NRP = pa_relpos_rows_padded(Hp, Wp);
     if (part != nullptr && NRP > 16 * NSMAX) return (int)hipErrorInvalidValue;
+    if (Bn > 63) rowskip = nullptr;
     if (part == nullptr && dG == nullptr) return (int)hipErrorInvalidValue;
     unsigned char* tb = reinterpret_cast<unsigned char*>(tables);
     int e;
@@ -839,7 +881,7 @@
         if ((e = set_smem(reinterpret_cast<const void*>(kern), fuse ? donef : (g_attn_trace ? donet : (dq_w == 3 ? done3 : done2))))) return e;
         const char* ablv = getenv("PA_ATTN3_DQ_ABL");
         PA_LAUNCH(kern, dim3(nblk * Bn * H), dim3(NT), smem, st, qkv, (size_t)ldq, rcatT, dout, (size_t)lddo, lse, tb, dqkv, dG, part, L, H,
-                  Hp, NRP, scale, nblk, a3_xcd_map_on(), ablv ? atoi(ablv) : 0, tile0, 0, delta == nullptr ? out : nullptr, (size_t)ldo);
+                  Hp, NRP, scale, nblk, a3_xcd_map_on(), ablv ? atoi(ablv) : 0, tile0, 0, delta == nullptr ? out : nullptr, (size_t)ldo, rowskip);
         if ((e = (int)hipGetLastError())) return e;
     }
     const int tile0_kv = 0, nblk_kv = a3_blocks(L);
@@ -852,7 +894,7 @@
         static bool done2 = false, done3 = false;
         if ((e = set_smem(reinterpret_cast<const void*>(kern), dkv_w == 3 ? done3 : done2))) return e;
         PA_LAUNCH(kern, dim3(nblk_kv * Bn * H), dim3(NT), smem, st, qkv, (size_t)ldq, dout, (size_t)lddo, tb, dqkv, L, H, Hp, scale, nblk_kv,
-                  a3_xcd_map_on(), [] { const char* v = getenv("PA_ATTN3_DKV_ABL"); return v ? atoi(v) : 0; }(), tile0_kv);
+                  a3_xcd_map_on(), [] { const char* v = getenv("PA_ATTN3_DKV_ABL"); return v ? atoi(v) : 0; }(), tile0_kv, rowskip);
         if ((e = (int)hipGetLastError())) return e;
     }
     return 0;
diff --git a/painter_amd/csrc/attn_bwd.hip b/painter_amd/csrc/attn_bwd.hip
--- a/painter_amd/csrc/attn_bwd.hip
+++ b/painter_amd/csrc/attn_bwd.hip
@@ -547,16 +547,17 @@
     if (dtype != PA_BF16 || head_dim != ATT_HD || L != Hp * Wp) return 0;
     return attn3_relpos_partials_bytes(batch, L, heads, Hp, Wp);
 }
-extern "C" int pa_attn_bwd(int dtype, const void* qkv, int64_t ldq, const void* rcat, const void* rcatT, const void* dout, int64_t lddo,
-                           const float* lse, const float* delta, void* dqkv, void* dG, void* relpos_part, void* aux, void* tables,
-                           const void* out, int64_t ldo, int batch, int L, int heads, int Hp, int Wp, int head_dim, float scale, hipStream_t st) {
+extern "C" int pa_attn_bwd_skip(int dtype, const void* qkv, int64_t ldq, const void* rcat, const void* rcatT, const void* dout, int64_t lddo,
+                                const float* lse, const float* delta, void* dqkv, void* dG, void* relpos_part, void* aux, void* tables,
+                                const void* out, int64_t ldo, int batch, int L, int heads, int Hp, int Wp, int head_dim, float scale,
+                                const float* rowskip, hipStream_t st) {
     if (L != Hp * Wp || L % 32 || Hp % 4 || Wp % 4 || (head_dim != 64 && head_dim != 80)) return (int)hipErrorInvalidValue;
     if (dtype == PA_BF16 && head_dim == ATT_HD && tables != nullptr && attn3_ok(L, Hp, Wp)) {
         if (relpos_part != nullptr && attn3_relpos_partials_bytes(batch, L, heads, Hp, Wp) == 0) return (int)hipErrorInvalidValue;
         ++g_attn_counts[5];
         if (out != nullptr && ldo % 8) return (int)hipErrorInvalidValue;
         return attn3_bwd((const bf16*)qkv, ldq, (const bf16*)rcatT, (const bf16*)dout, lddo, lse, delta, tables, (bf16*)dqkv, (bf16*)dG,
-                         (float*)relpos_part, batch, L, heads, Hp, Wp, scale, (const bf16*)out, ldo, st);
+                         (float*)relpos_part, batch, L, heads, Hp, Wp, scale, (const bf16*)out, ldo, st, drop_skip_on() ? rowskip : nullptr);
     }
     if (relpos_part != nullptr || dG == nullptr || delta == nullptr) return (int)hipErrorInvalidValue;
     if (dtype == PA_BF16 && attn2_ok(L, Hp, Wp, head_dim)) {
@@ -570,6 +571,12 @@
     if (dtype == PA_BF16) return head_dim == 80 ? PA_ATTN_BWD(bf16, 80) : PA_ATTN_BWD(bf16, 64);
     return head_dim == 80 ? PA_ATTN_BWD(float, 80) : PA_ATTN_BWD(float, 64);
 #undef PA_ATTN_BWD
+}
+extern "C" int pa_attn_bwd(int dtype, const void* qkv, int64_t ldq, const void* rcat, const void* rcatT, const void* dout, int64_t lddo,
+                           const float* lse, const float* delta, void* dqkv, void* dG, void* relpos_part, void* aux, void* tables,
+                           const void* out, int64_t ldo, int batch, int L, int heads, int Hp, int Wp, int head_dim, float scale, hipStream_t st) {
+    return pa_attn_bwd_skip(dtype, qkv, ldq, rcat, rcatT, dout, lddo, lse, delta, dqkv, dG, relpos_part, aux, tables, out, ldo, batch, L, heads, Hp, Wp,
+                            head_dim, scale, nullptr, st);
 }
 
 extern "C" int64_t pa_attn_bwd_relpos_workspace_bytes(int dtype, int batch, int L, int heads, int Hp, int Wp, int head_dim) {
diff --git a/painter_amd/csrc/attn_fwd.hip b/painter_amd/csrc/attn_fwd.hip
--- a/painter_amd/csrc/attn_fwd.hip
+++ b/painter_amd/csrc/attn_fwd.hip
@@ -245,12 +245,13 @@
 extern "C" int64_t pa_attn_tables_bytes(int dtype, int batch, int L, int heads, int Hp, int Wp, int head_dim) {
     return dtype == PA_BF16 && head_dim == ATT_HD ? attn3_table_bytes(batch, L, heads, Hp, Wp) : 0;
 }
-extern "C" int pa_attn_fwd(int dtype, const void* qkv, int64_t ldq, const void* rcat, void* out, int64_t ldo, float* lse, void* tables,
-                           int batch, int L, int heads, int Hp, int Wp, int head_dim, float scale, hipStream_t st) {
+extern "C" int pa_attn_fwd_skip(int dtype, const void* qkv, int64_t ldq, const void* rcat, void* out, int64_t ldo, float* lse, void* tables,
+                                int batch, int L, int heads, int Hp, int Wp, int head_dim, float scale, const float* rowskip, hipStream_t st) {
     if (L != Hp * Wp || L % 32 || Hp % 4 || Wp % 4 || !head_dim_ok(head_dim)) return (int)hipErrorInvalidValue;
     if (dtype == PA_BF16 && head_dim == ATT_HD && attn3_ok(L, Hp, Wp)) {
         ++g_attn_counts[2];
-        return attn3_fwd((const bf16*)qkv, ldq, (const bf16*)rcat, (bf16*)out, ldo, lse, tables, batch, L, heads, Hp, Wp, scale, st);
+        return attn3_fwd((const bf16*)qkv, ldq, (const bf16*)rcat, (bf16*)out, ldo, lse, tables, batch, L, heads, Hp, Wp, scale, st,
+                         drop_skip_on() ? rowskip : nullptr);
     }
     if (dtype == PA_BF16 && attn2_ok(L, Hp, Wp, head_dim)) {
         ++g_attn_counts[1];
@@ -259,6 +260,10 @@
     ++g_attn_counts[0];
     if (dtype == PA_BF16) return attn_fwd_t<bf16>(qkv, ldq, rcat, out, ldo, lse, batch, L, heads, Hp, Wp, head_dim, scale, st);
     return attn_fwd_t<float>(qkv, ldq, rcat, out, ldo, lse, batch, L, heads, Hp, Wp, head_dim, scale, st);
+}
+extern "C" int pa_attn_fwd(int dtype, const void* qkv, int64_t ldq, const void* rcat, void* out, int64_t ldo, float* lse, void* tables,
+                           int batch, int L, int heads, int Hp, int Wp, int head_dim, float scale, hipStream_t st) {
+    return pa_attn_fwd_skip(dtype, qkv, ldq, rcat, out, ldo, lse, tables, batch, L, heads, Hp, Wp, head_dim, scale, nullptr, st);
 }
 
 extern "C" int pa_attn_launch_counts(long long* out6) {
diff --git a/painter_amd/csrc/attn_tile.h b/painter_amd/csrc/attn_tile.h
--- a/painter_amd/csrc/attn_tile.h
+++ b/painter_amd/csrc/attn_tile.h
@@ -32,6 +32,37 @@
     const int v = (xcd_map & 1) ? xcd_run(n, total) : n;
     bh = v / nblk;
     blk = v - bh * nblk;
+}
+
+DEVI bool wg_coords_skip(int nblk, int xcd_map, int& blk, int& bh, const float* __restrict__ rowskip, int H, int* slot = nullptr) {
+    const int n = blockIdx.x, total = gridDim.x, per = nblk * H, ns = total / per;
+    const int lane = threadIdx.x & 63;
+    const float fv = lane < ns ? rowskip[lane] : 1.f;
+    const unsigned long long dmask = __ballot(fv == 0.f);
+    const int nk = (ns - __builtin_popcountll(dmask)) * per;
+    const bool drop = n >= nk;
+    const int v = drop ? n - nk : ((xcd_map & 1) ? xcd_run(n, nk) : n);
+    const int rank = v / per, rem = v - rank * per;
+    int b = rank;
+    if (dmask != 0) {
+        unsigned long long m = drop ? dmask : ~dmask;
+        for (int c = 0; c < rank; ++c) m &= m - 1;
+        b = __builtin_ctzll(m);
+    }
+    bh = b * H + rem / nblk;
+    blk = rem % nblk;
+    if (slot != nullptr) {
+        const int u = bh * nblk + blk;
+        if (xcd_map & 1) {
+            const int xq = total >> 3, xr = total & 7, lim = xr * (xq + 1);
+            const int c = u < lim ? u / (xq + 1) : xr + (u - lim) / xq;
+            const int o = u < lim ? u - c * (xq + 1) : (u - lim) - (c - xr) * xq;
+            *slot = o * 8 + c;
+        } else {
+            *slot = u;
+        }
+    }
+    return drop;
 }
 
 DEVI int vsw(int row) { return (((row >> 1) & 1) << 2) | (((row >> 2) & 1) << 1) | ((row >> 3) & 1); }
@@ -116,6 +147,14 @@
     }
 }
 
+DEVI void zero_rows(bf16* dst, size_t ld, int lane) {
+#pragma unroll
+    for (int i = 0; i < 4; ++i) {
+        const int c = lane + 64 * i, row = c >> 3, ch = c & 7;
+        *reinterpret_cast<uint4*>(dst + (size_t)row * ld + ch * 8) = make_uint4(0, 0, 0, 0);
+    }
+}
+
 static inline int set_smem(const void* kern, bool& done) {
     if (!done) {
         hipError_t e = hipFuncSetAttribute(kern, hipFuncAttributeMaxDynamicSharedMemorySize, 160 * 1024);
diff --git a/painter_amd/csrc/common.h b/painter_amd/csrc/common.h
--- a/painter_amd/csrc/common.h
+++ b/painter_amd/csrc/common.h
@@ -1,6 +1,7 @@
 #pragma once
 #include <hip/hip_runtime.h>
 #include <stdint.h>
+#include <cstdlib>
 
 typedef __bf16 bf16;
 typedef __attribute__((ext_vector_type(8))) __bf16 bf16x8;
@@ -101,6 +102,12 @@
 inline int g_conv_wgrad_groups = 0;
 inline int g_misc_knob[5] = {0, 0, 0, 0, 0};
 
+inline int g_drop_skip = 0;
+static inline bool drop_skip_on() {
+    static const int env = [] { const char* v = getenv("PAINTER_AMD_DROP_SKIP"); return v ? atoi(v) : 1; }();
+    return g_drop_skip == 1 ? false : (g_drop_skip == 2 ? true : env != 0);
+}
+
 inline long long g_attn_counts[6] = {0, 0, 0, 0, 0, 0};
 
 DEVI float gelu_f(float x) { return 0.5f * x * (1.0f + erff(x * 0.70710678118654752f)); }
diff --git a/painter_amd/csrc/gemm.hip b/painter_amd/csrc/gemm.hip
--- a/painter_amd/csrc/gemm.hip
+++ b/painter_amd/csrc/gemm.hip
@@ -372,9 +372,19 @@
 template <typename T>
 static int linear_fwd_t(int epi, const T* x, int64_t ldx, const T* w, const float* bias, void* out, void* out2,
                         int64_t ldo, const float* resid, const float* rowscale, int rps, int M, int N, int K,
-                        hipStream_t st) {
+                        hipStream_t st, const float* rowskip = nullptr, int skip_rps = 1) {
     if constexpr (std::is_same<T, bf16>::value) {
         if (g256::ok(M, N, K, false, false, ldx, K)) {
+            if (rowskip != nullptr) {
+                switch (epi) {
+                case PA_EPI_BIAS:
+                    return g256::launch_skip<false>(x, ldx, w, K, Epi4Bias<bf16>{(bf16*)out, (size_t)ldo, bias, M, N}, M, N, K, st, rowskip, skip_rps);
+                case PA_EPI_BIAS_GELU:
+                    return g256::launch_skip<false>(x, ldx, w, K, Epi4BiasGelu{(unsigned char*)out2, (bf16*)out, (size_t)ldo, bias, M, N}, M, N, K, st, rowskip, skip_rps);
+                case PA_EPI_BIAS_RESID:
+                    return g256::launch_skip<false>(x, ldx, w, K, Epi4BiasResid{(float*)out, resid, (size_t)ldo, bias, rowscale, rps, M, N}, M, N, K, st, rowskip, skip_rps);
+                }
+            }
             switch (epi) {
             case PA_EPI_BIAS:
                 return g256::launch<false, false>(x, ldx, w, K, Epi4Bias<bf16>{(bf16*)out, (size_t)ldo, bias, M, N}, M, N, K, 1, st);
@@ -402,13 +412,21 @@
     return (int)hipErrorInvalidValue;
 }
 
+extern "C" int pa_linear_fwd_skip(int dtype, int epilogue, const void* x, int64_t ldx, const void* w, const float* bias,
+                                  void* out, void* out2, int64_t ldo, const float* resid, const float* rowscale,
+                                  int rows_per_sample, int M, int N, int K, const float* rowskip, int skip_rows_per_sample, hipStream_t st) {
+    if (K % (dtype == PA_BF16 ? 8 : 4)) return (int)hipErrorInvalidValue;
+    if (rowskip != nullptr && skip_rows_per_sample < 1) return (int)hipErrorInvalidValue;
+    if (!drop_skip_on()) rowskip = nullptr;
+    if (dtype == PA_BF16)
+        return linear_fwd_t<bf16>(epilogue, (const bf16*)x, ldx, (const bf16*)w, bias, out, out2, ldo, resid, rowscale, rows_per_sample, M, N, K, st,
+                                  rowskip, skip_rows_per_sample);
+    return linear_fwd_t<float>(epilogue, (const float*)x, ldx, (const float*)w, bias, out, out2, ldo, resid, rowscale, rows_per_sample, M, N, K, st);
+}
 extern "C" int pa_linear_fwd(int dtype, int epilogue, const void* x, int64_t ldx, const void* w, const float* bias,
                              void* out, void* out2, int64_t ldo, const float* resid, const float* rowscale,
                              int rows_per_sample, int M, int N, int K, hipStream_t st) {
-    if (K % (dtype == PA_BF16 ? 8 : 4)) return (int)hipErrorInvalidValue;
-    if (dtype == PA_BF16)
-        return linear_fwd_t<bf16>(epilogue, (const bf16*)x, ldx, (const bf16*)w, bias, out, out2, ldo, resid, rowscale, rows_per_sample, M, N, K, st);
-    return linear_fwd_t<float>(epilogue, (const float*)x, ldx, (const float*)w, bias, out, out2, ldo, resid, rowscale, rows_per_sample, M, N, K, st);
+    return pa_linear_fwd_skip(dtype, epilogue, x, ldx, w, bias, out, out2, ldo, resid, rowscale, rows_per_sample, M, N, K, nullptr, 1, st);
 }
 
 template <typename T>
@@ -437,18 +455,19 @@
 }
 template <typename T>
 static int linear_dgrad_t(const T* dy, int64_t lddy, const T* w, const typename GeluAux<T>::type* pre , T* dx, int64_t lddx, float* dx_colsum, float* ws, int M,
-                          int N, int K, hipStream_t st) {
+                          int N, int K, hipStream_t st, const float* rowskip = nullptr, int skip_rps = 1) {
     if constexpr (std::is_same<T, bf16>::value) {
         if (g256::ok(M, K, N, false, true, lddy, K)) {
             if (pre && dx_colsum) {
                 Epi4DGeluCS ep;
                 ep.out = dx; ep.aux = pre; ep.ld = (size_t)lddx; ep.M = M; ep.N = K; ep.part = ws;
-                int e = g256::launch<false, true>(dy, lddy, w, K, ep, M, K, N, 1, st);
+                int e = rowskip ? g256::launch_skip<true>(dy, lddy, w, K, ep, M, K, N, st, rowskip, skip_rps) : g256::launch<false, true>(dy, lddy, w, K, ep, M, K, N, 1, st);
                 if (e) return e;
                 return pa_slab_reduce(ws, dx_colsum, K, 2 * g256::row_tiles_used(M, K, 1), K, 0, st);
             }
             if (pre) return g256::launch<false, true>(dy, lddy, w, K, Epi4DGelu{dx, pre, (size_t)lddx, M, K}, M, K, N, 1, st);
-            int e = g256::launch<false, true>(dy, lddy, w, K, Epi4Bias<bf16>{dx, (size_t)lddx, nullptr, M, K}, M, K, N, 1, st);
+            int e = rowskip ? g256::launch_skip<true>(dy, lddy, w, K, Epi4Bias<bf16>{dx, (size_t)lddx, nullptr, M, K}, M, K, N, st, rowskip, skip_rps)
+                            : g256::launch<false, true>(dy, lddy, w, K, Epi4Bias<bf16>{dx, (size_t)lddx, nullptr, M, K}, M, K, N, 1, st);
             if (e || dx_colsum == nullptr) return e;
             return pa_colsum(PA_BF16, dx, lddx, M, K, dx_colsum, ws, st);
         }
@@ -461,12 +480,21 @@
     if (e || dx_colsum == nullptr) return e;
     return pa_colsum(std::is_same<T, bf16>::value ? PA_BF16 : PA_F32, dx, lddx, M, K, dx_colsum, ws, st);
 }
+extern "C" int pa_linear_dgrad_skip(int dtype, const void* dy, int64_t lddy, const void* w, const void* gelu_aux,
+                                    void* dx, int64_t lddx, float* dx_colsum, void* workspace, int M, int N, int K,
+                                    const float* rowskip, int skip_rows_per_sample, hipStream_t st) {
+    if (N % 8 || K % 4) return (int)hipErrorInvalidValue;
+    if (dx_colsum != nullptr && (workspace == nullptr || K % 8 || lddx % 8)) return (int)hipErrorInvalidValue;
+    if (rowskip != nullptr && skip_rows_per_sample < 1) return (int)hipErrorInvalidValue;
+    if (!drop_skip_on()) rowskip = nullptr;
+    if (dtype == PA_BF16)
+        return linear_dgrad_t<bf16>((const bf16*)dy, lddy, (const bf16*)w, (const unsigned char*)gelu_aux, (bf16*)dx, lddx, dx_colsum, (float*)workspace, M, N, K, st,
+                                    rowskip, skip_rows_per_sample);
+    return linear_dgrad_t<float>((const float*)dy, lddy, (const float*)w, (const float*)gelu_aux, (float*)dx, lddx, dx_colsum, (float*)workspace, M, N, K, st);
+}
 extern "C" int pa_linear_dgrad(int dtype, const void* dy, int64_t lddy, const void* w, const void* gelu_aux,
                                void* dx, int64_t lddx, float* dx_colsum, void* workspace, int M, int N, int K, hipStream_t st) {
-    if (N % 8 || K % 4) return (int)hipErrorInvalidValue;
-    if (dx_colsum != nullptr && (workspace == nullptr || K % 8 || lddx % 8)) return (int)hipErrorInvalidValue;
-    if (dtype == PA_BF16) return linear_dgrad_t<bf16>((const bf16*)dy, lddy, (const bf16*)w, (const unsigned char*)gelu_aux, (bf16*)dx, lddx, dx_colsum, (float*)workspace, M, N, K, st);
-    return linear_dgrad_t<float>((const float*)dy, lddy, (const float*)w, (const float*)gelu_aux, (float*)dx, lddx, dx_colsum, (float*)workspace, M, N, K, st);
+    return pa_linear_dgrad_skip(dtype, dy, lddy, w, gelu_aux, dx, lddx, dx_colsum, workspace, M, N, K, nullptr, 1, st);
 }
 
 static bool wgrad_fast(int dtype, int M, int N, int K) {
@@ -529,6 +557,7 @@
 
 extern "C" int pa_abi_version(void) { return PA_ABI_VERSION; }
 extern "C" int pa_debug_get(int which) {
+    if (which == 16) return g_drop_skip;
     if (which < 0 || which > 15) return -1;
     if (which == 9) return g_conv_wgrad_groups;
     if (which == 10) return g_ln_bwd_variant;
@@ -539,6 +568,7 @@
     return g256::g_dbg[which];
 }
 extern "C" int pa_debug_set(int which, int value) {
+    if (which == 16) { g_drop_skip = value; return 0; }
     if (which < 0 || which > 15) return (int)hipErrorInvalidValue;
     if (which < 8) g256::g_dbg[which] = value;
     if (which == 9) g_conv_wgrad_groups = value;
diff --git a/painter_amd/csrc/gemm256.h b/painter_amd/csrc/gemm256.h
--- a/painter_amd/csrc/gemm256.h
+++ b/painter_amd/csrc/gemm256.h
@@ -90,11 +90,13 @@
 template <class Epi> struct epi_hi_off<Epi, std::void_t<decltype(Epi::HI_OFF)>> { static constexpr int value = Epi::HI_OFF; };
 constexpr int BM_SHORT = 224;
 constexpr int BM_HALF = 128;
-template <bool AMM, bool BMM, int ILV, class Epi, bool SHORT = false, bool MIXED = false>
+template <bool AMM, bool BMM, int ILV, class Epi, bool SHORT = false, bool MIXED = false, bool SKIP = false>
 __global__ __launch_bounds__(NT) void gemm256_kernel(const bf16* __restrict__ Ag, uint32_t lda, const bf16* __restrict__ Bg,
                                                       uint32_t ldb, Epi epi, int M, int N, int ktiles, int ktiles_per_split,
-                                                      int tiles_n, int stagger, int order, int nfull, int patch) {
+                                                      int tiles_n, int stagger, int order, int nfull, int patch,
+                                                      const float* __restrict__ rowskip, int rps) {
     static_assert(!(SHORT && AMM), "the 224-row tile is built for a K-major A operand");
+    static_assert(!(SKIP && AMM), "row tiles are skipped only for a K-major A operand");
     static_assert(!(MIXED && (AMM || SHORT)), "half tiles are built for a K-major A operand and 256-row full tiles");
     constexpr int BMR = SHORT ? BM_SHORT : BM;
     extern __shared__ __attribute__((aligned(1024))) unsigned char smem[];
@@ -108,8 +110,38 @@
     const int wr = wv >> 2, wc = wv & 3;
 
     const bool htile = MIXED && (int)blockIdx.x >= nfull * tiles_n;
-    const int nwg = MIXED ? (htile ? (int)gridDim.x - nfull * tiles_n : nfull * tiles_n) : (int)gridDim.x;
+    int nwg = MIXED ? (htile ? (int)gridDim.x - nfull * tiles_n : nfull * tiles_n) : (int)gridDim.x;
     const int bid = htile ? (int)blockIdx.x - nfull * tiles_n : (int)blockIdx.x;
+    unsigned long long dmask = 0;
+    auto skipped_ranges = [&](auto&& f) {
+        const int r0 = htile ? nfull * BMR : 0, r1 = (MIXED && !htile) ? nfull * BMR : M;
+        const int np = htile ? (r1 - r0 + BM_HALF - 1) / BM_HALF : (r1 - r0 + BMR - 1) / BMR;
+        unsigned long long m = dmask;
+        while (m != 0) {
+            const int s0 = __builtin_ctzll(m), s1 = s0 + __builtin_ctzll(~(m >> s0));
+            m &= ~0ull << s1;
+            const int ra = max(s0 * rps, r0), rb = min(min(s1 * rps, M), r1);
+            if (rb <= ra) continue;
+            const int ua = ra - r0, ub = rb - r0;
+            const int a = htile ? (ua + BM_HALF - 1) / BM_HALF : (ua + BMR - 1) / BMR;
+            const int b = rb >= r1 ? np : (htile ? ub / BM_HALF : ub / BMR);
+            if (b > a) f(a, b);
+        }
+    };
+    bool skipped = false;
+    int kept_panels = 0;
+    if constexpr (SKIP) {
+        {
+            const int ns = (M + rps - 1) / rps;
+            const float fv = lane < ns ? rowskip[lane] : 1.f;
+            dmask = __ballot(fv == 0.f);
+        }
+        const int r0 = htile ? nfull * BMR : 0, r1 = (MIXED && !htile) ? nfull * BMR : M;
+        kept_panels = htile ? (r1 - r0 + BM_HALF - 1) / BM_HALF : (r1 - r0 + BMR - 1) / BMR;
+        skipped_ranges([&](int a, int b) { kept_panels -= b - a; });
+        nwg = kept_panels * tiles_n;
+        skipped = bid >= nwg;
+    }
     const int xq = nwg >> 3, xr = nwg & 7, xcd = bid & 7;
     int tile = (xcd < xr ? xcd * (xq + 1) : xr * (xq + 1) + (xcd - xr) * xq) + (bid >> 3);
     int split = blockIdx.y;
@@ -119,10 +151,11 @@
         split = w / nwg;
         tile = w - split * nwg;
     }
-    int tm, tn;
-    if (order != 1) {
+    int tm = 0, tn = 0;
+    if (skipped) {
+    } else if (order != 1) {
         const int TR = patch > 0 ? patch / 100 : 4, TC = patch > 0 ? patch % 100 : 8;
-        const int tiles_m = MIXED ? (htile ? (M - nfull * BMR + BM_HALF - 1) / BM_HALF : nfull) : (M + BMR - 1) / BMR;
+        const int tiles_m = SKIP ? kept_panels : MIXED ? (htile ? (M - nfull * BMR + BM_HALF - 1) / BM_HALF : nfull) : (M + BMR - 1) / BMR;
         const int per_group = TR * tiles_n;
         const int gm = tile / per_group, rem = tile - gm * per_group;
         const int rg = min(TR, tiles_m - gm * TR);
@@ -140,11 +173,24 @@
         tm = tile / tiles_n;
         tn = tile - tm * tiles_n;
     }
+    if constexpr (SKIP) {
+        if (skipped) {
+            const int d = bid - nwg;
+            int r = d / tiles_n;
+            tn = d - r * tiles_n;
+            bool found = false;
+            skipped_ranges([&](int a, int b) {
+                if (!found && r < b - a) { tm = a + r; found = true; }
+                if (!found) r -= b - a;
+            });
+        } else {
+            skipped_ranges([&](int a, int b) { if (tm >= a) tm += b - a; });
+        }
+    }
     const int i0 = htile ? nfull * BMR + tm * BM_HALF : tm * BMR, j0 = tn * BN;
     const bool blk3 = !(SHORT && wr == 1);
     const int kt0 = split * ktiles_per_split;
     const int nt = min(ktiles - kt0, ktiles_per_split);
-
     uint32_t oa[2][2], ob[2][2];
 #pragma unroll
     for (int sub = 0; sub < 2; ++sub)
@@ -316,16 +362,18 @@
     if constexpr (MIXED) {
         if (htile) {
             ran_half = true;
-            piece_a(0, 0, 0, 0); piece_a(1, 0, 0, 0); stage_b(0, 0, 0); stage_b(1, 0, 0);
-            wait_vm<0>();
-            bar();
-            for (int T = 0; T < nt; T += 2) {
-                half_body(I0{}, T);
-                half_body(I1{}, T + 1);
+            if (!skipped) {
+                piece_a(0, 0, 0, 0); piece_a(1, 0, 0, 0); stage_b(0, 0, 0); stage_b(1, 0, 0);
+                wait_vm<0>();
+                bar();
+                for (int T = 0; T < nt; T += 2) {
+                    half_body(I0{}, T);
+                    half_body(I1{}, T + 1);
+                }
             }
         }
     }
-    if (!ran_half) {
+    if (!ran_half && !skipped) {
         stage_a(0, 0, 0);
         stage_b(0, 0, 0);
         stage_b(1, 0, 0);
@@ -341,7 +389,7 @@
             tile_body(I1{}, T + 1);
         }
     }
-    if (wr == 0 && !ran_half) bar();
+    if (wr == 0 && !ran_half && !skipped) bar();
     wait_vm<0>();
 
     bar();
@@ -407,8 +455,9 @@
     int per = (ktiles + nsplit - 1) / nsplit;
     return per + (per & 1);
 }
-template <bool AMM, bool BMM, int ILV, bool SHORT, class Epi, bool MIXED = false>
-static int launch_ilv(const bf16* A, size_t lda, const bf16* B, size_t ldb, Epi epi, int M, int N, int K, int nsplit, hipStream_t st, int nfull = 0);
+template <bool AMM, bool BMM, int ILV, bool SHORT, class Epi, bool MIXED = false, bool SKIP = false>
+static int launch_ilv(const bf16* A, size_t lda, const bf16* B, size_t ldb, Epi epi, int M, int N, int K, int nsplit, hipStream_t st, int nfull = 0,
+                      const float* rowskip = nullptr, int rps = 1);
 #ifndef G256_ILV_DEFAULT
 #define G256_ILV_DEFAULT 2
 #endif
@@ -460,9 +509,18 @@
     return launch_ilv<AMM, BMM, G256_ILV_DEFAULT, false>(A, lda, B, ldb, epi, M, N, K, nsplit, st);
 #endif
 }
-template <bool AMM, bool BMM, int ILV, bool SHORT, class Epi, bool MIXED>
-static int launch_ilv(const bf16* A, size_t lda, const bf16* B, size_t ldb, Epi epi, int M, int N, int K, int nsplit, hipStream_t st, int nfull) {
-    auto kern = gemm256_kernel<AMM, BMM, ILV, Epi, SHORT, MIXED>;
+template <bool BMM, class Epi>
+static int launch_skip(const bf16* A, size_t lda, const bf16* B, size_t ldb, Epi epi, int M, int N, int K, hipStream_t st, const float* rowskip, int rps) {
+    if ((M + rps - 1) / rps > 63) return launch<false, BMM>(A, lda, B, ldb, epi, M, N, K, 1, st);
+    const TilePlan tp = tile_plan(M, N, 1, false);
+    if (tp.mixed) return launch_ilv<false, BMM, G256_ILV_DEFAULT, false, Epi, true, true>(A, lda, B, ldb, epi, M, N, K, 1, st, tp.nfull, rowskip, rps);
+    if (tp.is_short) return launch_ilv<false, BMM, G256_ILV_DEFAULT, true, Epi, false, true>(A, lda, B, ldb, epi, M, N, K, 1, st, 0, rowskip, rps);
+    return launch_ilv<false, BMM, G256_ILV_DEFAULT, false, Epi, false, true>(A, lda, B, ldb, epi, M, N, K, 1, st, 0, rowskip, rps);
+}
+template <bool AMM, bool BMM, int ILV, bool SHORT, class Epi, bool MIXED, bool SKIP>
+static int launch_ilv(const bf16* A, size_t lda, const bf16* B, size_t ldb, Epi epi, int M, int N, int K, int nsplit, hipStream_t st, int nfull,
+                      const float* rowskip, int rps) {
+    auto kern = gemm256_kernel<AMM, BMM, ILV, Epi, SHORT, MIXED, SKIP>;
     static bool attr_done = false;
     if (!attr_done) {
         hipError_t e = hipFuncSetAttribute(reinterpret_cast<const void*>(kern), hipFuncAttributeMaxDynamicSharedMemorySize, LDS_BYTES);
@@ -478,7 +536,7 @@
     const int splits = (ktiles + per - 1) / per;
     if (g_dbg[1]) epi.M = 0;
     PA_LAUNCH(kern, dim3(tiles_m * tiles_n, splits), dim3(NT), LDS_BYTES, st, A, (uint32_t)lda, B, (uint32_t)ldb, epi, M, N,
-              ktiles, per, tiles_n, g_dbg[0], g_dbg[2], nfull, g_misc_knob[0] > 0 ? g_misc_knob[0] : env_patch);
+              ktiles, per, tiles_n, g_dbg[0], g_dbg[2], nfull, g_misc_knob[0] > 0 ? g_misc_knob[0] : env_patch, rowskip, rps);
     return (int)hipGetLastError();
 }
 static inline int row_tiles_used(int M, int N, int nsplit) {
diff --git a/painter_amd/engine.py b/painter_amd/engine.py
--- a/painter_amd/engine.py
+++ b/painter_amd/engine.py
@@ -239,11 +239,12 @@
             if c.seggpt and merge_between_batch >= 0 and i >= merge_between_batch:
                 merge = 1 if c.merge_idx >= i else 2
             ds_a, ds_m = (None, None) if drop_scales is None else drop_scales[i]
+            sk_a = None if merge > 0 else ds_a
             ln1, mean1, rstd1 = ops.layernorm_fwd(x, P[pre + "norm1.weight"], P[pre + "norm1.bias"], c.ln_eps, T)
-            qkv = ops.linear_fwd(ln1, self.w(pre + "attn.qkv.weight", P), P[pre + "attn.qkv.bias"], EPI_BIAS)
+            qkv = ops.linear_fwd(ln1, self.w(pre + "attn.qkv.weight", P), P[pre + "attn.qkv.bias"], EPI_BIAS, rowskip=sk_a, skip_rows_per_sample=L)
             rcat = self.relpos(pre, P, False)
-            ao, lse, atab = ops.attn_fwd(qkv, rcat, Bc, L, c.heads, c.Hp, c.Wp, c.scale, need_tables=True) if need_grad else \
-                ops.attn_fwd(qkv, rcat, Bc, L, c.heads, c.Hp, c.Wp, c.scale) + (None,)
+            ao, lse, atab = ops.attn_fwd(qkv, rcat, Bc, L, c.heads, c.Hp, c.Wp, c.scale, need_tables=True, rowskip=sk_a) if need_grad else \
+                ops.attn_fwd(qkv, rcat, Bc, L, c.heads, c.Hp, c.Wp, c.scale, rowskip=sk_a) + (None,)
             group = 0
             if merge > 0:
                 a = ops.linear_fwd(ao, self.w(pre + "attn.proj.weight", P), P[pre + "attn.proj.bias"], EPI_BIAS_F32)
@@ -256,11 +257,11 @@
                     del e
             else:
                 x1 = ops.linear_fwd(ao, self.w(pre + "attn.proj.weight", P), P[pre + "attn.proj.bias"], EPI_BIAS_RESID,
-                                    resid=x, rowscale=ds_a, rows_per_sample=L)
+                                    resid=x, rowscale=ds_a, rows_per_sample=L, rowskip=sk_a)
             ln2, mean2, rstd2 = ops.layernorm_fwd(x1, P[pre + "norm2.weight"], P[pre + "norm2.bias"], c.ln_eps, T)
-            act, gaux = ops.linear_gelu(ln2, self.w(pre + "mlp.fc1.weight", P), P[pre + "mlp.fc1.bias"], need_aux=need_grad)
+            act, gaux = ops.linear_gelu(ln2, self.w(pre + "mlp.fc1.weight", P), P[pre + "mlp.fc1.bias"], need_aux=need_grad, rowskip=ds_m, rows_per_sample=L)
             x2 = ops.linear_fwd(act, self.w(pre + "mlp.fc2.weight", P), P[pre + "mlp.fc2.bias"], EPI_BIAS_RESID,
-                                resid=x1, rowscale=ds_m, rows_per_sample=L)
+                                resid=x1, rowscale=ds_m, rows_per_sample=L, rowskip=ds_m)
             if need_grad:
                 S.blocks.append((x, mean1, rstd1, ln1, qkv, rcat, ao, lse, x1, mean2, rstd2, ln2, gaux, act, Bc, atab, group))
             x = x2
@@ -416,6 +417,7 @@
             S.blocks[i] = None
             R = Bc * L
             ds_a, ds_m = (None, None) if S.drop is None else S.drop[i]
+            sk_a = None if ens_group > 0 else ds_a
             nrp, hd = rcat.shape
             flat, fl = block_flat(i)
             del flats[i]
@@ -435,13 +437,13 @@
             param_grads(pre + "mlp.fc2.weight", pre + "mlp.fc2.bias", dyT, act, fl["fc2"])
             tr("%d.dyT" % i, dyT)
             if _FC1_COLSUM == "epilogue":
-                dpre = ops.linear_dgrad(dyT, self.w(pre + "mlp.fc2.weight", P), gelu_aux=gaux, colsum_out=fl["fc1"])
+                dpre = ops.linear_dgrad(dyT, self.w(pre + "mlp.fc2.weight", P), gelu_aux=gaux, colsum_out=fl["fc1"], rowskip=ds_m, rows_per_sample=L)
                 G[pre + "mlp.fc1.bias"] = fl["fc1"]
             else:
                 dpre = ops.linear_dgrad(dyT, self.w(pre + "mlp.fc2.weight", P), gelu_aux=gaux)
             tr("%d.dpre" % i, dpre)
             param_grads(pre + "mlp.fc1.weight", pre + "mlp.fc1.bias", dpre, ln2, fl["fc1"])
-            dln2 = ops.linear_dgrad(dpre, self.w(pre + "mlp.fc1.weight", P))
+            dln2 = ops.linear_dgrad(dpre, self.w(pre + "mlp.fc1.weight", P), rowskip=ds_m, rows_per_sample=L)
             tr("%d.dln2" % i, dln2)
             del dpre
             dyA = torch.empty_like(dyT) if side is not None else dyT
@@ -463,11 +465,11 @@
                 dyA = da if T == torch.float32 else ops.cast_bf16(da, out=dyA)
                 del da
             param_grads(pre + "attn.proj.weight", pre + "attn.proj.bias", dyA, ao, fl["proj"])
-            dao = ops.linear_dgrad(dyA, self.w(pre + "attn.proj.weight", P), out=dln2)
+            dao = ops.linear_dgrad(dyA, self.w(pre + "attn.proj.weight", P), out=dln2, rowskip=sk_a, rows_per_sample=L)
             tr("%d.dao" % i, dao)
             del dyA
             rcatT = self.relpos(pre, P, True)
-            dqkv, dG = ops.attn_bwd_core(qkv, rcat, rcatT, ao, dao, lse, Bc, L, c.heads, c.Hp, c.Wp, c.scale, tables=atab, prep=_ATTN_PREP)
+            dqkv, dG = ops.attn_bwd_core(qkv, rcat, rcatT, ao, dao, lse, Bc, L, c.heads, c.Hp, c.Wp, c.scale, tables=atab, prep=_ATTN_PREP, rowskip=sk_a)
             if need(pre + "attn.rel_pos_h") or need(pre + "attn.rel_pos_w"):
                 drcat = on_side(lambda: ops.attn_bwd_relpos(dG, qkv, nrp, Bc, L, c.heads, c.Hp, c.Wp, out=fl["rel"].view(nrp, hd)), dG, qkv)
                 nh, nw = 2 * c.Hp - 1, 2 * c.Wp - 1
@@ -476,7 +478,7 @@
             del dG
             tr("%d.dqkv" % i, dqkv)
             param_grads(pre + "attn.qkv.weight", pre + "attn.qkv.bias", dqkv, ln1, fl["qkv"])
-            dln1 = ops.linear_dgrad(dqkv, self.w(pre + "attn.qkv.weight", P), out=dao)
+            dln1 = ops.linear_dgrad(dqkv, self.w(pre + "attn.qkv.weight", P), out=dao, rowskip=sk_a, rows_per_sample=L)
             del dqkv
             nxt = i - 1
             dyT_next = None
diff --git a/painter_amd/ops.py b/painter_amd/ops.py
--- a/painter_amd/ops.py
+++ b/painter_amd/ops.py
@@ -37,7 +37,23 @@
     return t
 
 
-def linear_fwd(x, w, bias, epilogue=EPI_BIAS, out=None, out2=None, resid=None, rowscale=None, rows_per_sample=1):
+def _skip_args(rowskip, skip_rows_per_sample, M):
+    if rowskip is None:
+        return 0, 1
+    assert rowskip.dtype == torch.float32 and rowskip.is_cuda and rowskip.is_contiguous() and skip_rows_per_sample >= 1
+    assert rowskip.numel() * skip_rows_per_sample >= M, (rowskip.numel(), skip_rows_per_sample, M)
+    return rowskip.data_ptr(), int(skip_rows_per_sample)
+
+
+def drop_skip(mode=None):
+    old = int(lib.pa_debug_get(16))
+    if mode is not None:
+        check(lib.pa_debug_set(16, int(mode)), "pa_debug_set")
+    return old
+
+
+def linear_fwd(x, w, bias, epilogue=EPI_BIAS, out=None, out2=None, resid=None, rowscale=None, rows_per_sample=1, *, rowskip=None,
+               skip_rows_per_sample=None):
     M, K = x.shape
     N = w.shape[0]
     T = x.dtype
@@ -48,18 +64,23 @@
         out = torch.empty((M, N), dtype=odt, device=x.device)
     if epilogue == EPI_BIAS_RESID:
         assert resid is not None and resid.dtype == torch.float32 and resid.stride(0) == out.stride(0)
-    check(lib.pa_linear_fwd(code(T), epilogue, p(x), x.stride(0), p(w), p(bias), p(out), p(out2), out.stride(0),
-                            p(resid), p(rowscale), rows_per_sample, M, N, K, stream()), "pa_linear_fwd")
-    return out
-
-
-def linear_gelu(x, w, bias, need_aux=True):
+    if rowskip is None:
+        check(lib.pa_linear_fwd(code(T), epilogue, p(x), x.stride(0), p(w), p(bias), p(out), p(out2), out.stride(0),
+                                p(resid), p(rowscale), rows_per_sample, M, N, K, stream()), "pa_linear_fwd")
+    else:
+        sk, srps = _skip_args(rowskip, rows_per_sample if skip_rows_per_sample is None else skip_rows_per_sample, M)
+        check(lib.pa_linear_fwd_skip(code(T), epilogue, p(x), x.stride(0), p(w), p(bias), p(out), p(out2), out.stride(0),
+                                     p(resid), p(rowscale), rows_per_sample, M, N, K, sk, srps, stream()), "pa_linear_fwd_skip")
+    return out
+
+
+def linear_gelu(x, w, bias, need_aux=True, *, rowskip=None, rows_per_sample=1):
     M = x.shape[0]
     N = w.shape[0]
     act = torch.empty((M, N), dtype=x.dtype, device=x.device)
     aux = torch.empty((M, N), dtype=gelu_aux_dtype(x.dtype), device=x.device) if need_aux else None
     assert aux is None or aux.stride(0) == act.stride(0)
-    linear_fwd(x, w, bias, EPI_BIAS_GELU, out=act, out2=aux)
+    linear_fwd(x, w, bias, EPI_BIAS_GELU, out=act, out2=aux, rowskip=rowskip, skip_rows_per_sample=rows_per_sample)
     return act, aux
 
 
@@ -86,7 +107,7 @@
     return out
 
 
-def linear_dgrad(dy, w, gelu_aux=None, out=None, colsum_out=None):
+def linear_dgrad(dy, w, gelu_aux=None, out=None, colsum_out=None, *, rowskip=None, rows_per_sample=1):
     M, N = dy.shape
     K = w.shape[1]
     T = dy.dtype
@@ -99,8 +120,13 @@
     if colsum_out is not None:
         assert colsum_out.shape == (K,) and colsum_out.dtype == torch.float32 and colsum_out.is_contiguous()
         ws = workspace(lib.pa_linear_dgrad_workspace_bytes(M, K), dy.device, slot=2)
-    check(lib.pa_linear_dgrad(code(T), p(dy), dy.stride(0), p(w), p(gelu_aux), p(out), out.stride(0), p(colsum_out), p(ws), M, N, K, stream()),
-          "pa_linear_dgrad")
+    if rowskip is None:
+        check(lib.pa_linear_dgrad(code(T), p(dy), dy.stride(0), p(w), p(gelu_aux), p(out), out.stride(0), p(colsum_out), p(ws), M, N, K, stream()),
+              "pa_linear_dgrad")
+    else:
+        sk, srps = _skip_args(rowskip, rows_per_sample, M)
+        check(lib.pa_linear_dgrad_skip(code(T), p(dy), dy.stride(0), p(w), p(gelu_aux), p(out), out.stride(0), p(colsum_out), p(ws), M, N, K,
+                                       sk, srps, stream()), "pa_linear_dgrad_skip")
     return out
 
 
@@ -193,7 +219,7 @@
     return rcat, rcatT
 
 
-def attn_fwd(qkv, rcat, batch, L, heads, Hp, Wp, scale, need_tables=False):
+def attn_fwd(qkv, rcat, batch, L, heads, Hp, Wp, scale, need_tables=False, *, rowskip=None):
     T = qkv.dtype
     hd = rcat.shape[1]
     assert qkv.shape[1] == 3 * heads * hd
@@ -204,8 +230,12 @@
         nb = lib.pa_attn_tables_bytes(code(T), batch, L, heads, Hp, Wp, hd)
         if nb > 0:
             tables = torch.empty((nb,), dtype=torch.uint8, device=qkv.device)
-    check(lib.pa_attn_fwd(code(T), p(qkv), qkv.stride(0), p(rcat), p(out), out.stride(0), p(lse), p(tables), batch, L, heads,
-                          Hp, Wp, hd, float(scale), stream()), "pa_attn_fwd")
+    if rowskip is None:
+        check(lib.pa_attn_fwd(code(T), p(qkv), qkv.stride(0), p(rcat), p(out), out.stride(0), p(lse), p(tables), batch, L, heads,
+                              Hp, Wp, hd, float(scale), stream()), "pa_attn_fwd")
+    else:
+        check(lib.pa_attn_fwd_skip(code(T), p(qkv), qkv.stride(0), p(rcat), p(out), out.stride(0), p(lse), p(tables), batch, L, heads,
+                                   Hp, Wp, hd, float(scale), _skip_args(rowskip, 1, batch)[0], stream()), "pa_attn_fwd_skip")
     return (out, lse, tables) if need_tables else (out, lse)
 
 
@@ -225,7 +255,7 @@
     return rcatT
 
 
-def attn_bwd_core(qkv, rcat, rcatT, out, dout, lse, batch, L, heads, Hp, Wp, scale, tables=None, prep="fused"):
+def attn_bwd_core(qkv, rcat, rcatT, out, dout, lse, batch, L, heads, Hp, Wp, scale, tables=None, prep="fused", *, rowskip=None):
     T = qkv.dtype
     dev = qkv.device
     nrp, hd = rcat.shape
@@ -249,9 +279,14 @@
     else:
         dG = torch.empty((batch * L, heads * nrp), dtype=T, device=dev)
     aux = workspace(lib.pa_attn_bwd_aux_bytes(batch, L, heads, Hp, Wp), dev, slot=1)
-    check(lib.pa_attn_bwd(code(T), p(qkv), qkv.stride(0), p(rcat), p(rcatT), p(dout), dout.stride(0), p(lse), p(delta),
-                          p(dqkv), p(dG), p(part), p(aux), p(tables), p(o_arg), 0 if o_arg is None else o_arg.stride(0), batch, L, heads, Hp, Wp, hd,
-                          float(scale), stream()), "pa_attn_bwd")
+    if rowskip is None:
+        check(lib.pa_attn_bwd(code(T), p(qkv), qkv.stride(0), p(rcat), p(rcatT), p(dout), dout.stride(0), p(lse), p(delta),
+                              p(dqkv), p(dG), p(part), p(aux), p(tables), p(o_arg), 0 if o_arg is None else o_arg.stride(0), batch, L, heads, Hp, Wp, hd,
+                              float(scale), stream()), "pa_attn_bwd")
+    else:
+        check(lib.pa_attn_bwd_skip(code(T), p(qkv), qkv.stride(0), p(rcat), p(rcatT), p(dout), dout.stride(0), p(lse), p(delta),
+                                   p(dqkv), p(dG), p(part), p(aux), p(tables), p(o_arg), 0 if o_arg is None else o_arg.stride(0), batch, L, heads, Hp, Wp,
+                                   hd, float(scale), _skip_args(rowskip, 1, batch)[0], stream()), "pa_attn_bwd_skip")
     return dqkv, (dG if part is None else part)
 
 
```

New measurement: 161.1 images/sec, median of 6. 1.01x the previous value.
